# tachyon-beep/keisei

Measured on AMD Instinct MI355X. Metric: PPO samples/sec, se_resnet 40x256 on 50x9x9, higher is better.
Workload: dtype bf16; 1 GPU; se_resnet 40x256 KataGo-PPO minibatch step (gather+fwd+loss+bwd+clip+Adam), minibatch 4096/GPU from a 16384-sample device-resident epoch dataset, obs 50x9x9; per_gpu_batch=4096, global_batch=4096, parallelism=dp1

## Files before the change

### include/keisei_amd.h

```cpp
#ifndef KEISEI_AMD_H
#define KEISEI_AMD_H

#ifdef __cplusplus
extern "C" {
#endif

#define KA_OK 0
#define KA_ERR_ARG (-1)
#define KA_ERR_HIP (-2)
#define KA_ERR_UNSUPPORTED (-3)
#define KA_DTYPE_F32 0
#define KA_DTYPE_BF16 1

int ka_version(void);
const char* ka_target_arch(void);
const char* ka_last_error(void);
int ka_options_reload(void);

int ka_conv3x3_fwd(const void* in, const void* wpack, void* out, const float* in_scale, const float* in_shift,
                   const float* in_bias, int relu, float* bsum, float* sqpart, int B, int Cin, int Cout, int dtype,
                   void* stream);
int ka_conv3x3_fwd_keep_supported(int B, int Cin, int Cout, int dtype);
int ka_conv3x3_fwd_keep(const void* in, const void* wpack, void* out, const float* in_scale, const float* in_shift,
                        const float* in_bias, int relu, float* bsum, float* sqpart, void* x_out, int B, int Cin, int Cout, int dtype,
                        void* stream);
int ka_conv3x3_sqpart_rows(int B);
int ka_conv_route_counts(long long* out, int n);
int ka_conv3x3_dgrad_fused(const void* in, const void* in2, const float* k, void* dy_out, const void* wpack, void* out,
                           float* bsum, const void* ep_y, const float* ep_scale, const float* ep_shift,
                           const float* ep_mean, const float* ep_invstd, float* ep_s1, float* ep_s2, int B, int Cin,
                           int Cout, int dtype, void* stream);
int ka_conv3x3_dgrad_gated_supported(int B, int Cin, int Cout, int dtype, int masked);
int ka_conv3x3_dgrad_fused_gated(const void* du, const float* gate_add, const void* in2, const float* k,
                                 void* dy_out, const void* wpack, void* out, float* bsum, const void* ep_y,
                                 const float* ep_scale, const float* ep_shift, const float* ep_mean, const float* ep_invstd,
                                 float* ep_s1, float* ep_s2, int B, int Cin, int Cout, int dtype, void* stream);
int ka_pack_conv3x3(const float* w, void* dst, int Co, int Ci, int Nout, int Kin, int mode, int dtype, void* stream);
int ka_pack_conv3x3_multi(const long long* table, int n, long long max_pieces, int dtype, void* stream);
int ka_conv3x3_wgrad(const void* dy, const void* x, const float* in_scale, const float* in_shift, const float* in_bias,
                     int relu, float* slab, float* dw, int B, int Cin, int Cin_real, int Cout, int accumulate,
                     int target_wgs, int dtype, void* stream);
int ka_wgrad_splits(int B, int Cin, int Cout, int target_wgs);
int ka_debug_conv_stamps(unsigned long long* stamps);

int ka_obs_to_nhwc(const float* obs, const long long* idx, void* out, int B, int Cobs, int Cpad, int dtype, void* stream);
int ka_nhwc_to_nchw(const void* in, float* out, int B, int C, int dtype, void* stream);

int ka_reduce_workspace_doubles(int C);
int ka_bn_reduce(const float* bsum, int B, const float* sqpart, int R, int C, double* sums, double* part, void* stream);
int ka_bn_coeffs(const double* sums, double count, const double* count_dev, const float* gamma, const float* beta,
                 float* running_mean, float* running_var, long long* num_batches_tracked, float momentum, float eps,
                 float* scale, float* shift, float* mean, float* invstd, int C, void* stream);
int ka_bn_eval_coeffs(const float* gamma, const float* beta, const float* running_mean, const float* running_var,
                      float eps, float* scale, float* shift, int C, void* stream);
int ka_bn_eval_coeffs_multi(const long long* table, int n, int max_c, void* stream);
int ka_pair_reduce(const float* p1, const float* p2, int B, int C, double* sums, double* part, void* stream);
int ka_bn_bwd_coeffs(const double* sums_local, const double* sums_global, double count, const double* count_dev,
                     const float* gamma, const float* mean, const float* invstd, float* dgamma, float* dbeta, float* k,
                     int C, int train, void* stream);
int ka_sync_reduce(const float* p1, int rows1, const float* p2, int rows2, int C, double count, double* sums,
                   double* local_copy, double* part, void* stream);
int ka_bn_coeffs_parts(const double* part, double count, const float* gamma, const float* beta, float* running_mean,
                       float* running_var, long long* num_batches_tracked, float momentum, float eps, float* scale,
                       float* shift, float* mean, float* invstd, int C, void* stream);
int ka_bn_bwd_coeffs_parts(const double* part, double count, const float* gamma, const float* mean, const float* invstd,
                           float* dgamma, float* dbeta, float* k, int C, int train, void* stream);
int ka_bn_reduce_coeffs(const float* bsum, int B, const float* sqpart, int R, int C, double* part, int* counters, double count,
                        const float* gamma, const float* beta, float* running_mean, float* running_var,
                        long long* num_batches_tracked, float momentum, float eps, float* scale, float* shift, float* mean,
                        float* invstd, void* stream);
int ka_pair_reduce_bwd_coeffs(const float* p1, const float* p2, int rows, int C, double* part, int* counters, double count,
                              const float* gamma, const float* mean, const float* invstd, float* dgamma, float* dbeta, float* k,
                              int train, void* stream);
int ka_bn_bwd_apply(const void* dz, const void* y, const float* k, void* dy, int B, int C, int dtype, void* stream);
int ka_affine_rows(const float* in, const float* a, const float* s, float mul, float* out, int B, int C, void* stream);

int ka_block_tail_fwd(const void* y, const float* scale, const float* shift, const float* se, const void* res, void* out,
                      float* pool, int B, int C, int dtype, void* stream);
int ka_block_tail_fwd_se_supported(int C, int H, int dtype);
int ka_block_tail_fwd_se(const void* y, const float* scale, const float* shift, const float* bsum, const float* W1, const float* b1,
                         const float* W2, const float* b2, const void* res, void* out, float* pool, float* sqz_out, float* se1_out,
                         float* se_out, int B, int C, int H, int dtype, void* stream);
int ka_pool_fwd(const void* x, float* pool, int B, int C, int dtype, void* stream);
int ka_tail_bwd_reduce(const void* dout, const void* out, const void* y, const float* scale, const float* shift,
                       const float* se, float* dse, int B, int C, int dtype, void* stream);
int ka_tail_bwd_dz(const void* dout, const void* out, const void* y, const float* se, const float* dsq, const float* mean,
                   const float* invstd, void* dz, float* s1p, float* s2p, int B, int C, int dtype, void* stream);
int ka_tail_bwd_fused_supported(int C, int H, int dtype);
int ka_tail_bwd_fused(const void* dout, const void* out, const void* y, const float* scale, const float* shift,
                      const float* se, const float* se1, const float* W2, const float* W1, const float* mean,
                      const float* invstd, void* dz, float* dse, float* dh, float* s1p, float* s2p, int B, int C, int H,
                      int dtype, void* stream);
int ka_relu_bn_bwd_reduce(const void* dh, const void* y, const float* scale, const float* shift, const float* mean,
                          const float* invstd, void* da, float* s1p, float* s2p, int B, int C, int dtype, void* stream);
int ka_block_dx(const void* dxc, const void* dout, const void* out, const void* x, const float* xpool, const float* dpool,
                void* dx, int B, int C, int dtype, void* stream);
int ka_block_dx_tail_bwd_supported(int C, int H, int dtype);
int ka_block_dx_tail_bwd(const void* dxc, const void* dout_up, const void* out_up, const void* x, const float* xpool,
                         const float* dpool, void* dx, const void* y, const float* scale, const float* shift, const float* se,
                         const float* se1, const float* W2, const float* W1, const float* mean, const float* invstd, void* dz,
                         float* dse, float* dh, float* s1p, float* s2p, int B, int C, int H, int dtype, void* stream);
int ka_block_dx_tail_bwd_du(const void* dxc, const void* du_up, const void* x, const float* xpool, const float* dpool,
                            void* du_out, const void* y, const float* scale, const float* shift, const float* se,
                            const float* se1, const float* W2, const float* W1, const float* mean, const float* invstd, void* dz,
                            float* dse, float* dh, float* s1p, float* s2p, int B, int C, int H, int dtype, void* stream);
int ka_block_dx_tail_bwd_du_gate(const void* dxc, const void* du_up, const void* x, const float* xpool, const float* dpool,
                                 void* du_out, const void* y, const float* scale, const float* shift, const float* se,
                                 const float* se1, const float* W2, const float* W1, const float* mean, const float* invstd,
                                 float* gate_out, float* add_out, float* dse, float* dh, float* s1p, float* s2p, int B, int C,
                                 int H, int dtype, void* stream);

int ka_gemm(const void* A, const void* B, void* C, const float* bias, int M, int N, int K, int lda, int ldb, int ldc,
            int transA, int transB, int a_bf16, int b_bf16, int c_bf16, int relu, int accumulate, int nsplit, void* stream);
int ka_gemm_grouped_wgrad(const long long* table, int njobs, int total_wgs, void* stream);
int ka_fc_chain_supported(int K1, int ldx, int H, int N2);
int ka_fc_chain(const float* x, const float* in_scale, const float* in_shift, float in_alpha, const float* W1,
                const float* b1, const float* W2, const float* b2, float* x_out, float* hidden_out, float* y, int M, int K1,
                int ldx, int H, int N2, void* stream);
int ka_fc_chain_bwd(const float* dy, const float* hidden, const float* W2T, const float* W1T, float* dhidden_out, float* dx,
                    int M, int N2, int H, int K1, void* stream);
int ka_transpose_multi(const void* table, int n, int max_tiles, void* stream);
int ka_reduce_slabs(const float* slab, float* out, int nsplit, long long n, int accumulate, void* stream);
int ka_reduce_slabs2(const float* slab_a, float* out_a, long long na, const float* slab_b, float* out_b, long long nb, int nsplit,
                     void* stream);
int ka_colsum(const float* A, const float* Bm, float* part, float* part2, int M, int N, int nsplit, void* stream);
int ka_relu_mask(float* g, const float* h, long long n, void* stream);
int ka_rows_affine_relu(const float* in, const float* scale, const float* shift, float* out, long long M, int N, void* stream);
int ka_rows_sq_sums(const float* A, float* part, float* part2, int M, int N, int nsplit, void* stream);
int ka_rows_bn_sums(const float* da, const float* in, const float* mean, const float* invstd, float* part, float* part2,
                    int M, int N, int nsplit, void* stream);
int ka_rows_bn_bwd(float* dr, const float* in, const float* p0, const float* p1, long long M, int N, int mode, void* stream);

int ka_policy_loss(const float* logits, const void* legal, const long long* actions, const float* old_lp, const float* adv,
                   const long long* idx, float* dlogits, float* new_lp, float* rowloss, float* rowent, int* flags,
                   const float* gscale, float clip_eps, float w_policy, float w_entropy, int B, int A, int legal_words,
                   void* stream);
int ka_masked_softmax(const float* logits, const void* legal, float* probs, int* nlegal, int* flags, int B, int A,
                      int legal_words, void* stream);
int ka_policy_sample(const void* logits, int logits_bf16, const void* legal, int legal_words, long long seed,
                     const float* vlogits, const float* score, float alpha, long long* actions, float* logp, float* values,
                     int* nlegal, int* flags, int B, int A, void* stream);
int ka_policy_sample_play(const void* logits, int logits_bf16, const void* legal, int legal_words, const long long* seed_dev,
                          const int* model_of, int K, long long* actions, float* logp, int* nlegal, int* flags, int B, int A,
                          void* stream);
int ka_policy_ce(const float* logits, const long long* targets, const long long* idx, float* dlogits, float* rowloss,
                 int* flags, const float* gscale, float w_policy, int B, int A, void* stream);
int ka_value_loss(const float* vlogits, const float* score, const long long* cats, const float* targets,
                  const long long* idx, const float* rowloss, const float* rowent, float* dvlogits, float* dscore,
                  float* out, float* acc, const float* gscale, float lambda_policy, float lambda_value, float lambda_score,
                  float entropy_coeff, int combined_value_metric, int B, void* stream);
int ka_scalar_value(const float* vlogits, const float* score, float alpha, float* out, int B, void* stream);

int ka_adam_chunk(void);
int ka_clip_adam_step(const void* tab, const int* blk_tensor, const long long* blk_off, int nblocks, double* partial,
                      float* ctl, float* step_state, float* scaler, const int* guard_flags, float* acc_gnorm,
                      float max_norm, float lr, float beta1, float beta2, float eps, void* stream);

int ka_gae(const void* rewards, const void* values, const float* term, const void* next_value, const void* override_,
           const long long* lengths, void* adv, int T, int N, double gamma, double lam, int f64, void* stream);
int ka_normalize_advantages(const float* x, float* out, long long n, void* stream);

int ka_mask_words(int A);
int ka_rollout_append(const float* obs, const void* legal, const long long* actions, const float* log_probs,
                      const float* values, const float* rewards, const void* dones, const void* terminated,
                      const long long* cats, const float* score, const long long* env_ids, const float* override_,
                      float* d_obs, void* d_bits, long long* d_actions, float* d_log_probs, float* d_values, float* d_rewards,
                      void* d_dones, void* d_terminated, long long* d_cats, float* d_score, long long* d_env_ids,
                      float* d_override, int* flags, int n, int obs_elems, int A, void* stream);
int ka_rollout_append_packed(const float* obs, const void* legal_bits, const long long* actions, const float* log_probs,
                             const float* values, const float* rewards, const void* dones, const void* terminated,
                             const long long* cats, const float* score, const long long* env_ids, const float* override_,
                             float* d_obs, void* d_bits, long long* d_actions, float* d_log_probs, float* d_values, float* d_rewards,
                             void* d_dones, void* d_terminated, long long* d_cats, float* d_score, long long* d_env_ids,
                             float* d_override, int* flags, int n, int obs_elems, int A, void* stream);
int ka_unpack_mask_bits(const void* bits, const long long* idx, void* out, int rows, int A, void* stream);
int ka_pack_mask_bits(const void* legal, void* bits, int rows, int A, void* stream);

int ka_pending_open(float* obs, void* bits, long long* actions, float* log_probs, float* values, float* rewards, float* score,
                    void* valid, const void* env_mask, const float* s_obs, const void* s_legal, const void* s_bits,
                    const long long* s_actions, const float* s_log_probs, const float* s_values, const float* s_rewards,
                    const float* s_score, int* flags, int n, int obs_elems, int A, void* stream);
int ka_pending_accumulate(float* rewards, const void* valid, const float* add_rewards, int n, void* stream);
int ka_pending_settle(float* obs, void* bits, long long* actions, float* log_probs, float* values, float* rewards, float* score,
                      const void* valid, void* valid_out, const void* fin_mask, const void* dones, const void* terminated,
                      int flags_are_f32, const float* add_rewards, float* o_obs, void* o_bits, long long* o_actions,
                      float* o_log_probs, float* o_values, float* o_rewards, float* o_dones, float* o_terminated, float* o_score,
                      long long* o_env_ids, long long* o_cats, int* flags, int n, int obs_elems, int A, void* stream);

int ka_tower_eval_supported(int C, int G, int R, int dtype);
int ka_tower_eval(const void* x_in, const float* pool_in, void* x_out, float* pool_out, const void* blocks, int nblocks, int B,
                  int C, int G, int R, int dtype, void* stream);
int ka_tower_eval_grouped_supported(int C, int G, int R, int dtype);
int ka_stem_eval_grouped(const float* obs, const int* model_of, const void* stems, int K, void* x_out, float* pool_out, int B,
                         int cin, int C, int dtype, void* stream);
int ka_tower_eval_grouped(const void* x_in, const float* pool_in, void* x_out, float* pool_out, const int* model_of,
                          const void* tables, int K, int nblocks, int B, int C, int G, int R, int dtype, void* stream);
int ka_heads_eval_grouped(const void* x, const float* pool, const int* model_of, const void* heads, int K, float* logits,
                          float* value, float* score, int B, int C, int P, int V, int S, int dtype, void* stream);

int ka_shogi_env_state_bytes(void);
int ka_shogi_env_action_space(int action_mode);
int ka_shogi_env_reset(void* state, void* keys, void* checks, int n, int max_ply, int obs_mode, int action_mode, float* obs,
                       void* mask, void* mask_bits, void* current_players, int refresh, void* stream);
int ka_shogi_env_step(void* state, void* keys, void* checks, const long long* actions, int n, int max_ply, int obs_mode,
                      int action_mode, const void* prev_mask, const void* prev_mask_bits, int* err, float* obs, void* mask, void* mask_bits,
                      float* rewards, void* terminated, void* truncated, float* terminal_obs, void* current_players,
                      void* captured, void* term_reason, void* ply_count, int* material, void* stats, void* stream);

int ka_arena_state_words(int slots);
int ka_arena_referee(int* state, int slots, int envs_per_slot, const float* rewards, const void* terminated,
                     const void* truncated, const void* players, const int* nlegal, const long long* refusal, int* model_of,
                     void* pre_player, void* stream);
int ka_arena_assign(int* state, const int* jobs, int njobs, int envs_per_slot, const void* players, int* model_of,
                    void* pre_player, void* stream);
int ka_arena_cursor_words(int slots);
int ka_arena_record_pre(const int* state, const int* side_bits, int slots, int envs_per_slot, const float* obs,
                        const void* mask_bits, const long long* actions, const void* pre_player, const int* nlegal,
                        int* cursors, int* row_of, float* st_obs, void* st_mask_bits, long long* st_actions,
                        void* st_perspective, int cap, int obs_elems, int mask_words, void* stream);
int ka_arena_record_post(int* cursors, const int* row_of, int slots, int envs_per_slot, const float* rewards,
                         const void* terminated, const void* truncated, float* st_rewards, float* st_dones, int cap,
                         void* stream);
int ka_arena_feature_words(int which);
int ka_arena_features_step(const int* state, int slots, int envs_per_slot, const long long* actions, const void* pre_player,
                           const int* nlegal, const void* captured, const void* reason, const void* ply, const float* rewards,
                           const void* terminated, const void* truncated, int* acc, int* records, int* fcursors, int cap,
                           void* stream);
int ka_arena_features_seat(const int* jobs, int njobs, int slots, int envs_per_slot, int* acc, void* stream);
int ka_dynamic_targets(const float* rewards, const float* dones, long long* cats, float* adv, long long n, void* stream);

int ka_league_state_words(int opponents);
int ka_league_layout(int which);
int ka_league_step(int* state, int envs, int opponents, int flush, const float* obs, const void* mask_bits,
                   const long long* actions, const float* logp, const float* vlogits, const float* score_lead, float alpha,
                   const int* nlegal, const void* pre_player, const float* rewards, const void* terminated,
                   const void* truncated, const void* players, const int* material, float score_norm, const float* term_obs,
                   const long long* refusal, void* side, int* opp, int* games, const void* cum, int color_rand,
                   int* model_of, void* stall, float* values, float* p_obs, void* p_bits, int* p_scal, float* t_obs,
                   int* t_list, const long long* desc, int* plan, int obs_elems, int mask_words, void* stream);

int ka_tf_gemm_nt(const void* A, const void* B, void* C, const float* bias, const void* residual, int M, int N, int K,
                  int lda, int ldb, int ldc, int c_bf16, int relu, int nsplit, float drop_p, unsigned long long seed,
                  void* stream);
int ka_tf_gemm_nt_slabs(int K, int nsplit);
int ka_tf_gemm_nt_masked(const void* A, const void* B, void* C, const void* relu_act, int M, int N, int K, int lda, int ldb,
                         int ldc, float drop_p, unsigned long long seed, void* stream);
int ka_tf_gemm_tn(const void* A, const void* B, float* C, int M, int N, int K, int lda, int ldb, int ldc, int nsplit, void* stream);
int ka_tf_gemm_tn_bias(const void* A, const void* B, float* C, float* colsum, int M, int N, int K, int lda, int ldb, int ldc,
                       int nsplit, void* stream);
int ka_tf_gemm_tn_slabs(int M, int nsplit);
int ka_tf_transpose_pad(const void* in, void* out, int M, int N, int ldi, int ldo, int dtype, void* stream);
int ka_tf_cast_pad(const void* in, void* out, long long M, int N, int ldi, int ldo, int dtype, void* stream);
int ka_tf_weights16_multi(const void* table, int n, int total_tiles, void* stream);
int ka_tf_add_pos(void* x, const float* row_embed, const float* col_embed, int B, int d, int dtype, void* stream);
int ka_tf_pos_grad(const void* dx, float* scratch, float* drow, float* dcol, int B, int d, int dtype, void* stream);
int ka_tf_layernorm_fwd(const void* x, const float* gamma, const float* beta, void* y, float* mean, float* rstd, long long M,
                        int d, float eps, int dtype, void* stream);
int ka_tf_layernorm_parts(long long M);
int ka_tf_route_counts(long long* out, int n);
int ka_tf_layernorm_bwd(const void* dy, const void* x, const float* gamma, const float* mean, const float* rstd,
                        const void* dres, void* dx, float* part, float* dgamma, float* dbeta, long long M, int d, int dtype,
                        void* stream);
int ka_tf_layernorm_bwd_drop(const void* dy, const void* x, const float* gamma, const float* mean, const float* rstd,
                             const void* dres, void* dx, void* dx_drop, float drop_p, unsigned long long seed, float* part,
                             float* dgamma, float* dbeta, long long M, int d, int dtype, void* stream);
int ka_tf_drop_apply(const void* g_in, const void* act, const void* res, void* g_out, long long n, float drop_p,
                     unsigned long long seed, int dtype, void* stream);
int ka_tf_colsum(const void* a, float* part, float* out, long long M, int N, int nsplit, int dtype, void* stream);
int ka_tf_mean_pool(const void* x, float* pooled, int B, int d, int dtype, void* stream);
int ka_tf_head_grad(const float* dpooled, const void* dflat, void* dx, int B, int d, int dtype, void* stream);
int ka_tf_tanh(float* v, long long n, void* stream);
int ka_tf_tanh_bwd(const float* dy, const float* y, float* dx, long long n, void* stream);
int ka_tf_attention_fwd(const void* qkv, void* out, float* lse, int B, int H, int dh, float drop_p, unsigned long long seed,
                        int dtype, void* stream);
int ka_tf_attention_bwd(const void* qkv, const void* dout, const float* lse, void* dqkv, int B, int H, int dh, float drop_p,
                        unsigned long long seed, int dtype, void* stream);
int ka_tf_attention_bwd_o(const void* qkv, const void* out, const void* dout, const float* lse, void* dqkv, int B, int H, int dh,
                          float drop_p, unsigned long long seed, int dtype, void* stream);

#ifdef __cplusplus
}
#endif
#endif
```

### keisei_amd/_lib.py

```python
from __future__ import annotations

import ctypes
import os
from pathlib import Path
from typing import Optional

import torch

_LIB_PATH = Path(os.environ.get("KEISEI_AMD_LIB") or Path(__file__).resolve().parent / "libkeisei_amd.so")

_SIGS = {
    "ka_conv3x3_fwd": "pppppp i pp iii i p",
    "ka_conv3x3_fwd_keep_supported": "iiii",
    "ka_conv3x3_fwd_keep": "pppppp i pp p iii i p",
    "ka_conv3x3_dgrad_fused": "ppppp pp ppppp pp iii i p",
    "ka_conv3x3_dgrad_gated_supported": "iiiii",
    "ka_conv3x3_dgrad_fused_gated": "pppppp pp ppppp pp iii i p",
    "ka_conv3x3_sqpart_rows": "i",
    "ka_conv_route_counts": "p i",
    "ka_debug_conv_stamps": "p",
    "ka_pack_conv3x3": "pp iiii i i p",
    "ka_pack_conv3x3_multi": "p i q i p",
    "ka_wgrad_splits": "iiii",
    "ka_conv3x3_wgrad": "ppppp i pp iiii i i i p",
    "ka_obs_to_nhwc": "ppp iii i p",
    "ka_nhwc_to_nchw": "pp ii i p",
    "ka_bn_reduce": "p i p i i pp p",
    "ka_reduce_workspace_doubles": "i",
    "ka_pair_reduce": "pp ii pp p",
    "ka_sync_reduce": "p i p i i d ppp p",
    "ka_bn_coeffs": "p d p pppp p ff pppp i p",
    "ka_bn_coeffs_parts": "p d pppp p ff pppp i p",
    "ka_bn_bwd_coeffs_parts": "p d ppp ppp i i p",
    "ka_bn_reduce_coeffs": "p i p i i pp d pppp p ff pppp p",
    "ka_pair_reduce_bwd_coeffs": "pp i i pp d ppp ppp i p",
    "ka_bn_eval_coeffs": "pppp f pp i p",
    "ka_bn_bwd_coeffs": "pp d p ppp ppp i i p",
    "ka_affine_rows": "ppp f p ii p",
    "ka_bn_bwd_apply": "pppp ii i p",
    "ka_block_tail_fwd": "ppppp pp ii i p",
    "ka_block_tail_fwd_se_supported": "iii",
    "ka_block_tail_fwd_se": "pppppppp ppp ppp iii i p",
    "ka_pool_fwd": "pp ii i p",
    "ka_tail_bwd_reduce": "pppppp p ii i p",
    "ka_tail_bwd_dz": "ppppppp ppp ii i p",
    "ka_tail_bwd_fused_supported": "iii",
    "ka_tail_bwd_fused": "ppppp pppppp p pppp iii i p",
    "ka_relu_bn_bwd_reduce": "pppppp ppp ii i p",
    "ka_block_dx": "pppppp p ii i p",
    "ka_block_dx_tail_bwd_supported": "iii",
    "ka_block_dx_tail_bwd": "pppppp p ppppppppp p pppp iii i p",
    "ka_block_dx_tail_bwd_du": "ppppp p ppppppppp p pppp iii i p",
    "ka_block_dx_tail_bwd_du_gate": "ppppp p ppppppppp pp pppp iii i p",
    "ka_gemm": "pppp iii iii ii iii i i i p",
    "ka_reduce_slabs": "pp i q i p",
    "ka_reduce_slabs2": "pp q pp q i p",
    "ka_colsum": "pppp ii i p",
    "ka_relu_mask": "pp q p",
    "ka_rows_affine_relu": "pppp q i p",
    "ka_rows_bn_bwd": "pppp q i i p",
    "ka_rows_bn_sums": "pppp pp ii i p",
    "ka_rows_sq_sums": "ppp ii i p",
    "ka_policy_loss": "pppppp pppp pp fff iii p",
    "ka_masked_softmax": "ppppp iii p",
    "ka_policy_sample": "pi pi q pp f ppp pp ii p",
    "ka_policy_sample_play": "pi pi pp i pp pp ii p",
    "ka_policy_ce": "ppp ppp p f ii p",
    "ka_value_loss": "ppppp pp pp pp p ffff i i p",
    "ka_scalar_value": "pp f p i p",
    "ka_adam_chunk": "",
    "ka_clip_adam_step": "ppp i ppp ppp fffff p",
    "ka_gae": "ppppp pp ii dd i p",
    "ka_normalize_advantages": "pp q p",
    "ka_bn_eval_coeffs_multi": "p ii p",
    "ka_gemm_grouped_wgrad": "p ii p",
    "ka_fc_chain_supported": "iiii",
    "ka_fc_chain": "ppp f pppp ppp iiiii p",
    "ka_fc_chain_bwd": "pppppp iiii p",
    "ka_transpose_multi": "p ii p",
    "ka_mask_words": "i",
    "ka_rollout_append": "pppppppppppp pppppppppppp p iii p",
    "ka_rollout_append_packed": "pppppppppppp pppppppppppp p iii p",
    "ka_unpack_mask_bits": "ppp ii p",
    "ka_pack_mask_bits": "pp ii p",
    "ka_pending_open": "pppppppp ppppppppp p iii p",
    "ka_pending_accumulate": "ppp i p",
    "ka_pending_settle": "ppppppppp ppp i p ppppppppppp p iii p",
    "ka_tower_eval_supported": "iiii",
    "ka_tower_eval": "ppppp iiiii i p",
    "ka_tower_eval_grouped_supported": "iiii",
    "ka_stem_eval_grouped": "ppp i pp iiii p",
    "ka_tower_eval_grouped": "pppppp iiiiiii p",
    "ka_heads_eval_grouped": "pppp i ppp iiiii i p",
    "ka_shogi_env_state_bytes": "",
    "ka_shogi_env_action_space": "i",
    "ka_shogi_env_reset": "ppp ii ii pppp i p",
    "ka_shogi_env_step": "pppp ii ii ppp ppp ppp pp ppp pp p",
    "ka_arena_state_words": "i",
    "ka_arena_referee": "p ii ppppp p pp p",
    "ka_arena_assign": "pp ii ppp p",
    "ka_arena_cursor_words": "i",
    "ka_arena_record_pre": "pp ii ppppp pp pppp iii p",
    "ka_arena_record_post": "pp ii ppp pp i p",
    "ka_arena_feature_words": "i",
    "ka_arena_features_step": "p ii ppp ppp ppp ppp i p",
    "ka_arena_features_seat": "p iii p p",
    "ka_dynamic_targets": "pppp q p",
    "ka_league_state_words": "i",
    "ka_league_layout": "i",
    "ka_league_step": "p iii pppppp f ppppppp f pp pppp i ppp ppp pp pp ii p",
    "ka_tf_gemm_nt": "ppppp iii iii iii f q p",
    "ka_tf_gemm_nt_slabs": "ii",
    "ka_tf_gemm_nt_masked": "pppp iii iii f q p",
    "ka_tf_gemm_tn": "ppp iii iii i p",
    "ka_tf_gemm_tn_bias": "pppp iii iii i p",
    "ka_tf_gemm_tn_slabs": "ii",
    "ka_tf_transpose_pad": "pp iiii i p",
    "ka_tf_cast_pad": "pp q iii i p",
    "ka_tf_weights16_multi": "p ii p",
    "ka_tf_add_pos": "ppp ii i p",
    "ka_tf_pos_grad": "pppp ii i p",
    "ka_tf_layernorm_fwd": "pppppp q i f i p",
    "ka_tf_layernorm_parts": "q",
    "ka_tf_route_counts": "p i",
    "ka_tf_layernorm_bwd": "pppppp pppp q i i p",
    "ka_tf_layernorm_bwd_drop": "pppppp pp f q ppp q i i p",
    "ka_tf_drop_apply": "pppp q f q i p",
    "ka_tf_colsum": "ppp q ii i p",
    "ka_tf_mean_pool": "pp ii i p",
    "ka_tf_head_grad": "ppp ii i p",
    "ka_tf_tanh": "p q p",
    "ka_tf_tanh_bwd": "ppp q p",
    "ka_tf_attention_fwd": "ppp iii f q i p",
    "ka_tf_attention_bwd": "pppp iii f q i p",
    "ka_tf_attention_bwd_o": "ppppp iii f q i p",
    "ka_version": "",
    "ka_options_reload": "",
}
_CT = {"p": ctypes.c_void_p, "i": ctypes.c_int, "f": ctypes.c_float, "d": ctypes.c_double, "q": ctypes.c_longlong}

_lib: Optional[ctypes.CDLL] = None
_load_error: Optional[str] = None


class KeiseiHipError(RuntimeError):
    """Raised when a libkeisei_amd.so entry point reports failure (or the library is absent)."""


def _load() -> ctypes.CDLL:
    global _lib, _load_error
    if _lib is not None:
        return _lib
    if _load_error is not None:
        raise KeiseiHipError(_load_error)
    if not _LIB_PATH.exists():
        _load_error = (f"{_LIB_PATH} is missing: build it with `python -m keisei_amd.build` "
                       "(hipcc --offload-arch=gfx950). There is no fallback for GPU tensors.")
        raise KeiseiHipError(_load_error)
    try:
        lib = ctypes.CDLL(str(_LIB_PATH))
    except OSError as e:
        _load_error = f"cannot load {_LIB_PATH}: {e}"
        raise KeiseiHipError(_load_error) from e
    for name, sig in _SIGS.items():
        fn = getattr(lib, name)
        fn.argtypes = [_CT[c] for c in sig.replace(" ", "")]
        fn.restype = ctypes.c_int
    lib.ka_last_error.restype = ctypes.c_char_p
    lib.ka_last_error.argtypes = []
    lib.ka_target_arch.restype = ctypes.c_char_p
    lib.ka_target_arch.argtypes = []
    _lib = lib
    return lib


def reload_options() -> int:
    _QUERIES.clear()
    return int(_load().ka_options_reload())


def library_path() -> Path:
    return _LIB_PATH


def exported_symbols() -> list:
    return sorted(list(_SIGS) + ["ka_last_error", "ka_target_arch"])


def available() -> bool:
    try:
        _load()
        return True
    except KeiseiHipError:
        return False


_CHECK = os.environ.get("KA_CHECK_ARGS", "0") == "1"


def _check_tensors(name: str, args) -> None:
    dev = None
    for i, a in enumerate(args):
        if not isinstance(a, torch.Tensor):
            continue
        if not a.is_cuda:
            raise KeiseiHipError(f"{name}: argument {i} is a {a.device} tensor (the C ABI takes device pointers)")
        if not a.is_contiguous():
            raise KeiseiHipError(f"{name}: argument {i} is not contiguous (shape {tuple(a.shape)}, strides {a.stride()})")
        if dev is None:
            dev = a.device
        elif a.device != dev:
            raise KeiseiHipError(f"{name}: tensors on different devices ({dev} and {a.device})")
    if dev is not None and dev.index != torch.cuda.current_device():
        raise KeiseiHipError(f"{name}: tensors live on {dev} but the current device is cuda:{torch.cuda.current_device()} "
                             "(wrap the call in torch.cuda.device(tensor.device))")


def _ptr(x):
    if x is None:
        return None
    if isinstance(x, torch.Tensor):
        return x.data_ptr()
    return int(x)


def stream_ptr(device=None) -> int:
    return torch.cuda.current_stream(device).cuda_stream


_PLANS: dict = {}
_Tensor = torch.Tensor
_cur_dev = torch.cuda.current_device


def _plan(name: str):
    lib = _load()
    sig = _SIGS[name].replace(" ", "")
    ent = (getattr(lib, name), tuple(i for i, c in enumerate(sig) if c == "p"), len(sig))
    _PLANS[name] = ent
    return ent


def call(name: str, *args) -> None:
    ent = _PLANS.get(name)
    if ent is None:
        ent = _plan(name)
    fn, ptr_idx, n = ent
    if len(args) != n:
        raise TypeError(f"{name}: expected {n} arguments, got {len(args)}")
    conv = list(args)
    dev = None
    for i in ptr_idx:
        a = conv[i]
        if a is None:
            continue
        if type(a) is _Tensor or isinstance(a, _Tensor):
            if dev is None and a.is_cuda:
                dev = a.device.index
            conv[i] = a.data_ptr()
        else:
            conv[i] = int(a)
    if dev is not None and dev != _cur_dev():
        with torch.cuda.device(dev):
            if _CHECK:
                _check_tensors(name, args)
            rc = fn(*conv)
    else:
        if _CHECK:
            _check_tensors(name, args)
        rc = fn(*conv)
    if rc != 0:
        raise KeiseiHipError(f"{name} failed ({rc}): {_load().ka_last_error().decode()}")


_QUERIES: dict = {}


def query(name: str, *args) -> int:
    key = (name, args)
    v = _QUERIES.get(key)
    if v is None:
        v = _QUERIES[key] = int(getattr(_load(), name)(*args))
    return v


DTYPE_F32, DTYPE_BF16 = 0, 1


def dtype_code(dt: torch.dtype) -> int:
    if dt == torch.float32:
        return DTYPE_F32
    if dt == torch.bfloat16:
        return DTYPE_BF16
    raise KeiseiHipError(f"unsupported activation dtype {dt} (float32 or bfloat16)")
```

### keisei_amd/csrc/common.h

```cpp
#pragma once
#include <hip/hip_runtime.h>
#include <stdint.h>

#define KA_OK 0
#define KA_ERR_ARG (-1)
#define KA_ERR_HIP (-2)
#define KA_ERR_UNSUPPORTED (-3)

#define KA_DTYPE_F32 0
#define KA_DTYPE_BF16 1

#define KA_BOARD 81
#define KA_PADBOARD 121

typedef __attribute__((ext_vector_type(8))) __bf16 bf16x8;
typedef __attribute__((ext_vector_type(4))) __bf16 bf16x4;
typedef __attribute__((ext_vector_type(4))) float f32x4;
typedef __attribute__((ext_vector_type(2))) float f32x2;

struct bf16_t { uint16_t v; };

void ka_set_error(const char* fmt, ...);
int ka_check_launch(const char* what);
#define KA_REQUIRE(cond, ...) do { if (!(cond)) { ka_set_error(__VA_ARGS__); return KA_ERR_ARG; } } while (0)

#include <atomic>
inline int ka_big_lds_once(const void* func, std::atomic<unsigned long long>& done, const char* what) {
    int dev = 0;
    if (hipGetDevice(&dev) != hipSuccess) { ka_set_error("%s: hipGetDevice failed", what); return KA_ERR_HIP; }
    const unsigned long long bit = 1ull << (dev & 63);
    if (done.load(std::memory_order_acquire) & bit) return KA_OK;
    if (hipFuncSetAttribute(func, hipFuncAttributeMaxDynamicSharedMemorySize, 160 * 1024) != hipSuccess) {
        ka_set_error("%s: hipFuncSetAttribute failed on device %d", what, dev);
        return KA_ERR_HIP;
    }
    done.fetch_or(bit, std::memory_order_release);
    return KA_OK;
}

#include <stdlib.h>
inline const char* ka_diag_env(const char* name) {
#ifdef KA_DIAG
    return getenv(name);
#else
    (void)name;
    return nullptr;
#endif
}

#define KA_OPTIONS(X)                                                                                                      \
    X(CONV_P) X(CONV_MT) X(CONV_PC2) X(CONV_PC2_SKIP) X(CONV_PC2_STAG) X(CONV_CORNER_IN) X(CONV_P_STAG) X(CONV_P_PRIO) X(CONV_P_WGS) X(CONV_P_NPW) X(CONV_WM) X(CONV_KC)       \
    X(CONV_NTW) X(CONV_STAGGER) X(CONV_PRIO) X(WGRAD_TN) X(WGRAD_WGS) X(WGRAD_STAG) X(WGRAD_LEAN) X(BOARD_PAIRS) X(TF_LDS_EPI) X(TF_K256) X(TF_BIG)    \
    X(TF_MAP2D) X(TF_ATTN_LDS) X(TF_ATTN_ONE) X(TAIL_FWD_KB) X(TAIL_GATE_P4)
enum KaOpt {
#define KA_OPT_ENUM(n) KA_OPT_##n,
    KA_OPTIONS(KA_OPT_ENUM)
#undef KA_OPT_ENUM
    KA_OPT_COUNT
};
struct KaOptVal { int set, val; };
const KaOptVal* ka_opts();
inline bool ka_opt_set(KaOpt o) { return ka_opts()[o].set != 0; }
inline int ka_opt(KaOpt o, int dflt) { const KaOptVal v = ka_opts()[o]; return v.set ? v.val : dflt; }

std::atomic<unsigned long long*>& ka_debug_stamps();

enum KaConvRoute {
    KA_RT_CONV,
    KA_RT_PC,
    KA_RT_PC2,
    KA_RT_PC2_CORNER_IN,
    KA_RT_PC2_CORNER_OUT,
    KA_RT_CORNER,
    KA_RT_WGRAD_LEAN,
    KA_RT_WGRAD_TILED,
    KA_RT_COUNT
};
void ka_conv_route(int r);

__device__ __forceinline__ float bf2f(uint16_t h) { return __uint_as_float(((uint32_t)h) << 16); }
__device__ __forceinline__ uint16_t f2bf(float f) {
    __bf16 b = (__bf16)f;
    return __builtin_bit_cast(uint16_t, b);
}

template <typename T> struct Elem;
template <> struct Elem<float> {
    static constexpr int kSize = 4;
    static constexpr int kPer16 = 4;
    static constexpr int kDtype = KA_DTYPE_F32;
    typedef f32x4 vec16;
    static __device__ __forceinline__ float ld(const float* p) { return *p; }
    static __device__ __forceinline__ void st(float* p, float v) { *p = v; }
    static __device__ __forceinline__ void unpack(const vec16& v, float* f) {
        f[0] = v[0]; f[1] = v[1]; f[2] = v[2]; f[3] = v[3];
    }
    static __device__ __forceinline__ vec16 pack(const float* f) { vec16 v = {f[0], f[1], f[2], f[3]}; return v; }
};
template <> struct Elem<bf16_t> {
    static constexpr int kSize = 2;
    static constexpr int kPer16 = 8;
    static constexpr int kDtype = KA_DTYPE_BF16;
    typedef bf16x8 vec16;
    static __device__ __forceinline__ float ld(const bf16_t* p) { return bf2f(p->v); }
    static __device__ __forceinline__ void st(bf16_t* p, float v) { p->v = f2bf(v); }
    static __device__ __forceinline__ void unpack(const vec16& v, float* f) {
#pragma unroll
        for (int i = 0; i < 8; ++i) f[i] = (float)v[i];
    }
    static __device__ __forceinline__ vec16 pack(const float* f) {
        vec16 v;
#pragma unroll
        for (int i = 0; i < 8; ++i) v[i] = (__bf16)f[i];
        return v;
    }
};

template <typename T> __device__ __forceinline__ f32x2 ld2(const T* p);
template <> __device__ __forceinline__ f32x2 ld2<float>(const float* p) { return *reinterpret_cast<const f32x2*>(p); }
template <> __device__ __forceinline__ f32x2 ld2<bf16_t>(const bf16_t* p) {
    uint32_t u = *reinterpret_cast<const uint32_t*>(p);
    f32x2 r = {__uint_as_float(u << 16), __uint_as_float(u & 0xffff0000u)};
    return r;
}
template <typename T> __device__ __forceinline__ void st2(T* p, f32x2 v);
template <> __device__ __forceinline__ void st2<float>(float* p, f32x2 v) { *reinterpret_cast<f32x2*>(p) = v; }
template <> __device__ __forceinline__ void st2<bf16_t>(bf16_t* p, f32x2 v) {
    uint32_t u = (uint32_t)f2bf(v[0]) | ((uint32_t)f2bf(v[1]) << 16);
    *reinterpret_cast<uint32_t*>(p) = u;
}
template <typename T> __device__ __forceinline__ float rnd(float v);
template <> __device__ __forceinline__ float rnd<float>(float v) { return v; }
template <> __device__ __forceinline__ float rnd<bf16_t>(float v) { return bf2f(f2bf(v)); }

__device__ __forceinline__ int pad_index(int p) { return (p / 9 + 1) * 11 + (p % 9) + 1; }

__device__ __forceinline__ float wave_sum(float v) {
#pragma unroll
    for (int o = 32; o > 0; o >>= 1) v += __shfl_xor(v, o);
    return v;
}
__device__ __forceinline__ double wave_sum_d(double v) {
#pragma unroll
    for (int o = 32; o > 0; o >>= 1) v += __shfl_xor(v, o);
    return v;
}
#define KA_LDS_BARRIER() asm volatile("s_waitcnt lgkmcnt(0)\n\ts_barrier" ::: "memory")

__device__ __forceinline__ float sigmoidf_(float x) { return 1.0f / (1.0f + expf(-x)); }

__device__ __forceinline__ int ka_tile_rank(bool want, int running, int* wsum, int* rank) {
    const int lane = threadIdx.x & 63, wave = threadIdx.x >> 6;
    const unsigned long long b = __ballot(want);
    __syncthreads();
    if (lane == 0) wsum[wave] = __popcll(b);
    __syncthreads();
    int off = running, tot = 0;
    for (int w = 0; w < 4; ++w) {
        if (w < wave) off += wsum[w];
        tot += wsum[w];
    }
    *rank = want ? off + __popcll(b & ((1ull << lane) - 1ull)) : -1;
    return tot;
}
```

### keisei_amd/csrc/conv3x3.hip

```cpp
#include <stdlib.h>
#include <utility>
#include "common.h"

static std::atomic<long long> g_conv_routes[KA_RT_COUNT];
void ka_conv_route(int r) { g_conv_routes[r].fetch_add(1, std::memory_order_relaxed); }

namespace {

constexpr int kNB = 2;
constexpr int kPW = 17;
constexpr int kBoardStride = 193;
constexpr int kLdsSquares = kBoardStride + 11 * kPW;
constexpr int kImgSquares1 = 10 * kPW + 11;
constexpr int kZeroSquares = 2 * (kPW + 1) + 1;
__device__ __forceinline__ int lds_square(int b, int p) { return b * kBoardStride + (p / 9 + 1) * kPW + (p % 9) + 1; }
constexpr int kMTW = 6;

__host__ __device__ __forceinline__ int chan_of(int nt, int s, int NT) {
    return ((nt | 1) < NT) ? (nt >> 1) * 32 + (s >> 2) * 8 + (nt & 1) * 4 + (s & 3) : nt * 16 + s;
}

__device__ __forceinline__ float row_sum16(float v) {
    v += __int_as_float(__builtin_amdgcn_update_dpp(0, __float_as_int(v), 0xB1, 0xF, 0xF, true));
    v += __int_as_float(__builtin_amdgcn_update_dpp(0, __float_as_int(v), 0x4E, 0xF, 0xF, true));
// ... 748 lines not shown
#pragma unroll
                for (int e = 0; e < 4; ++e) {
                    esc[e] = a.ep_scale[cbl + 4 * j + e]; esh[e] = a.ep_shift[cbl + 4 * j + e];
                    emu[e] = a.ep_mean[cbl + 4 * j + e]; eis[e] = a.ep_invstd[cbl + 4 * j + e];
                    t1[e] = 0.f; t2[e] = 0.f;
                }
#pragma unroll
                for (int mt = 0; mt < MT; ++mt) {
                    const int p = mt * 16 + rl;
                    const bool in = p < KA_BOARD;
                    bf16x4 yv = bf16x4{};
                    if (in) yv = *reinterpret_cast<const bf16x4*>(smem + kPcLds + p * kPcYStride + (cb0 + 4 * j) * 2);
                    bf16x4 o;
#pragma unroll
                    for (int e = 0; e < 4; ++e) {
                        const float y = (float)yv[e];
                        const __bf16 db = (__bf16)acc[mt][j][e];
                        const float d = (in && y * esc[e] + esh[e] > 0.f) ? (float)db : 0.f;
                        t1[e] += d; t2[e] += d * ((y - emu[e]) * eis[e]);
                        o[e] = (__bf16)d;
                    }
                    if (j == 0) o0[mt] = o;
                    else if (in) {
                        bf16x8 o8;
#pragma unroll
                        for (int e = 0; e < 4; ++e) { o8[e] = o0[mt][e]; o8[4 + e] = o[e]; }
                        *reinterpret_cast<bf16x8*>(static_cast<char*>(a.out) + ((size_t)(bb * KA_BOARD + p) * a.Cout + cb0) * 2) = o8;
                    }
                }
#pragma unroll
                for (int e = 0; e < 4; ++e) { t1[e] = row_sum16(t1[e]); t2[e] = row_sum16(t2[e]); }
                if (rl == 0) {
                    *reinterpret_cast<f32x4*>(a.ep_s1 + (size_t)bb * a.Cout + cb0 + 4 * j) = f32x4{t1[0], t1[1], t1[2], t1[3]};
                    *reinterpret_cast<f32x4*>(a.ep_s2 + (size_t)bb * a.Cout + cb0 + 4 * j) = f32x4{t2[0], t2[1], t2[2], t2[3]};
                }
            }
            wfrag(0, 0, w0); wfrag(0, 1, w1); wfrag(0, 2, w2);
        }
    }
}

template <bool TWO, bool MASKED, int NPW, int MT, bool STAG = false>
static int launch_conv_pc_form(const ConvArgs& a, int grid, size_t lds, hipStream_t st, const char* what) {
    static std::atomic<unsigned long long> done{0};
    if (int rc = ka_big_lds_once(reinterpret_cast<const void*>(&conv3x3_pc_kernel<TWO, MASKED, NPW, MT, STAG>), done, what)) return rc;
    hipLaunchKernelGGL((conv3x3_pc_kernel<TWO, MASKED, NPW, MT, STAG>), dim3(grid), dim3(512 + 64 * NPW), lds, st, a);
    return ka_check_launch(what);
}
static int launch_conv_pc(ConvArgs a, hipStream_t st) {
    a.tune_stagger = 0; a.tune_prio = 0;
    if (const char* e = ka_diag_env("KA_CONV_P_ABL")) a.tune_stagger = atoi(e);
    a.tune_prio = ka_opt(KA_OPT_CONV_P_PRIO, 0);
    ka_conv_route(KA_RT_PC);
    int grid = 256;
    if (const int v = ka_opt(KA_OPT_CONV_P_WGS, 0); v > 0) grid = v;
    if (grid > a.B) grid = a.B;
    const int stag = ka_opt(KA_OPT_CONV_P_STAG, 0);
#define KA_PC_FORM(TWO_, MASKED_, NPW_, LDS_, WHAT_)                                                         \
    (a.mt5 ? ((stag && !MASKED_) ? launch_conv_pc_form<TWO_, false, NPW_, 5, true>(a, grid, LDS_, st, WHAT_ ", 5 row tiles, staggered") \
                                 : launch_conv_pc_form<TWO_, MASKED_, NPW_, 5>(a, grid, LDS_, st, WHAT_ ", 5 row tiles"))            \
           : launch_conv_pc_form<TWO_, MASKED_, NPW_, kMTW>(a, grid, LDS_, st, WHAT_))
    if (a.in2 && a.ep_y) return KA_PC_FORM(true, true, 4, kPcLdsMasked, "conv3x3 (pc, masked)");
    if (a.in2) return KA_PC_FORM(true, false, 4, kPcLds, "conv3x3 (pc, two-tensor)");
    if (ka_opt_set(KA_OPT_CONV_P_NPW) ? ka_opt(KA_OPT_CONV_P_NPW, 4) == 2 : (a.in_scale || a.relu || a.in_bias))
        return KA_PC_FORM(false, false, 2, kPcLds, "conv3x3 (pc, 2 staging waves)");
    return KA_PC_FORM(false, false, 4, kPcLds, "conv3x3 (pc)");
#undef KA_PC_FORM
}

typedef __attribute__((ext_vector_type(2))) unsigned u32x2;
template <int C, int MT>
__device__ __forceinline__ void conv_epilogue_masked_pair(const ConvArgs& a, f32x4 (&acc)[2 * MT][2], int b0, bool has_b1, int nt0, int r, int q) {
    constexpr int ROWB = C * 2, NT = C / 16;
    const int cb[2] = {chan_of(nt0, 4 * q, NT), chan_of(nt0 + 1, 4 * q, NT)};
    const char* yb = static_cast<const char*>(a.ep_y) + (size_t)b0 * (KA_BOARD * ROWB);
    char* ob = static_cast<char*>(a.out) + (size_t)b0 * (KA_BOARD * ROWB);
    const int lo[2] = {r * ROWB + cb[0] * 2, r * ROWB + cb[1] * 2};
    auto live = [&](int mt) { return MT == 5 || mt < 5 || r == 0; };
    u32x2 yA[MT], yB[MT];
    auto yload = [&](int b, int j, u32x2 (&y)[MT]) {
#pragma unroll
        for (int mt = 0; mt < MT; ++mt) y[mt] = live(mt) ? *reinterpret_cast<const u32x2*>(yb + b * (KA_BOARD * ROWB) + lo[j] + mt * 16 * ROWB) : u32x2{0u, 0u};
    };
    f32x4 cA[2], cB[2];
    yload(0, 0, yA);
    cA[0] = *reinterpret_cast<const f32x4*>(a.ep_scale + cb[0]); cA[1] = *reinterpret_cast<const f32x4*>(a.ep_shift + cb[0]);
    if (a.bsum) {
#pragma unroll
        for (int b = 0; b < 2; ++b)
#pragma unroll
            for (int j = 0; j < 2; ++j) {
                float s0[4] = {0.f, 0.f, 0.f, 0.f};
#pragma unroll
                for (int mt = 0; mt < MT; ++mt)
#pragma unroll
                    for (int i = 0; i < 4; ++i) s0[i] += live(mt) ? acc[MT * b + mt][j][i] : 0.f;
#pragma unroll
                for (int i = 0; i < 4; ++i) s0[i] = row_sum16(s0[i]);
                if (r == 0 && (b == 0 || has_b1)) *reinterpret_cast<f32x4*>(a.bsum + (b0 + b) * C + cb[j]) = f32x4{s0[0], s0[1], s0[2], s0[3]};
            }
    }
    yload(0, 1, yB);
    cB[0] = *reinterpret_cast<const f32x4*>(a.ep_scale + cb[1]); cB[1] = *reinterpret_cast<const f32x4*>(a.ep_shift + cb[1]);
    auto process = [&](int b, int j, const u32x2 (&y)[MT], const f32x4 (&c)[2]) {
        const f32x4 emu = *reinterpret_cast<const f32x4*>(a.ep_mean + cb[j]), eis = *reinterpret_cast<const f32x4*>(a.ep_invstd + cb[j]);
        float t1[4] = {0.f, 0.f, 0.f, 0.f}, t2[4] = {0.f, 0.f, 0.f, 0.f};
#pragma unroll
        for (int mt = 0; mt < MT; ++mt) {
            u32x2 o;
#pragma unroll
            for (int h = 0; h < 2; ++h) {
                const unsigned yw = y[mt][h];
                const float y0 = __uint_as_float(yw << 16), y1 = __uint_as_float(yw & 0xffff0000u);
                typedef __attribute__((ext_vector_type(2))) __bf16 bf16x2;
                const bf16x2 dbp = {(__bf16)acc[MT * b + mt][j][2 * h], (__bf16)acc[MT * b + mt][j][2 * h + 1]};
                const unsigned dw = __builtin_bit_cast(unsigned, dbp);
                const float d0 = (live(mt) && y0 * c[0][2 * h] + c[1][2 * h] > 0.f) ? __uint_as_float(dw << 16) : 0.f;
                const float d1 = (live(mt) && y1 * c[0][2 * h + 1] + c[1][2 * h + 1] > 0.f) ? __uint_as_float(dw & 0xffff0000u) : 0.f;
                t1[2 * h] += d0; t1[2 * h + 1] += d1;
                t2[2 * h] = fmaf(d0, y0, t2[2 * h]); t2[2 * h + 1] = fmaf(d1, y1, t2[2 * h + 1]);
                o[h] = (__float_as_uint(d0) >> 16) | __float_as_uint(d1);
            }
            if (live(mt)) *reinterpret_cast<u32x2*>(ob + b * (KA_BOARD * ROWB) + lo[j] + mt * 16 * ROWB) = o;
        }
#pragma unroll
        for (int e = 0; e < 4; ++e) {
            t1[e] = row_sum16(t1[e]);
            t2[e] = (row_sum16(t2[e]) - emu[e] * t1[e]) * eis[e];
        }
        if (r == 0) {
            *reinterpret_cast<f32x4*>(a.ep_s1 + (b0 + b) * C + cb[j]) = f32x4{t1[0], t1[1], t1[2], t1[3]};
            *reinterpret_cast<f32x4*>(a.ep_s2 + (b0 + b) * C + cb[j]) = f32x4{t2[0], t2[1], t2[2], t2[3]};
        }
    };
    process(0, 0, yA, cA);
    if (has_b1) yload(1, 0, yA);
    process(0, 1, yB, cB);
    if (has_b1) {
        yload(1, 1, yB);
        process(1, 0, yA, cA);
        process(1, 1, yB, cB);
    }
}

__device__ __forceinline__ void ld4x8_l2(const float* const (&p)[8], f32x4 (&v)[8]) {
    asm volatile("global_load_dwordx4 %0, %8, off sc1\n\t"
                 "global_load_dwordx4 %1, %9, off sc1\n\t"
                 "global_load_dwordx4 %2, %10, off sc1\n\t"
                 "global_load_dwordx4 %3, %11, off sc1\n\t"
                 "global_load_dwordx4 %4, %12, off sc1\n\t"
                 "global_load_dwordx4 %5, %13, off sc1\n\t"
                 "global_load_dwordx4 %6, %14, off sc1\n\t"
                 "global_load_dwordx4 %7, %15, off sc1\n\t"
                 "s_waitcnt vmcnt(0)"
                 : "=&v"(v[0]), "=&v"(v[1]), "=&v"(v[2]), "=&v"(v[3]), "=&v"(v[4]), "=&v"(v[5]), "=&v"(v[6]), "=&v"(v[7])
                 : "v"(p[0]), "v"(p[1]), "v"(p[2]), "v"(p[3]), "v"(p[4]), "v"(p[5]), "v"(p[6]), "v"(p[7])
                 : "memory");
}
__device__ __forceinline__ void corner_tile_epilogue(const ConvArgs& a, const f32x4 (&acc)[2], int bb, bool live, int nt0, int q) {
    if (!live) return;
    int cb[2];
    f32x4 pbs[2], psq[2], ps1[2], ps2[2];
    {
        const float* any = a.bsum ? a.bsum : reinterpret_cast<const float*>(a.wpack);
        const float* src[8];
#pragma unroll
        for (int j = 0; j < 2; ++j) {
            cb[j] = chan_of(nt0 + j, 4 * q, 16);
            const size_t srow = (size_t)bb * 256 + cb[j];
            src[j] = a.bsum ? a.bsum + srow : any;
            src[2 + j] = a.sqpart ? a.sqpart + srow : any;
            src[4 + j] = a.ep_y ? a.ep_s1 + srow : any;
            src[6 + j] = a.ep_y ? a.ep_s2 + srow : any;
        }
        f32x4 got[8];
        ld4x8_l2(src, got);
#pragma unroll
        for (int j = 0; j < 2; ++j) { pbs[j] = got[j]; psq[j] = got[2 + j]; ps1[j] = got[4 + j]; ps2[j] = got[6 + j]; }
    }
#pragma unroll
    for (int j = 0; j < 2; ++j) {
        const f32x4 v = acc[j];
        const size_t orow = ((size_t)bb * KA_BOARD + 80) * 256 + cb[j], srow = (size_t)bb * 256 + cb[j];
        if (a.bsum) *reinterpret_cast<f32x4*>(a.bsum + srow) = pbs[j] + v;
        if (a.sqpart) *reinterpret_cast<f32x4*>(a.sqpart + srow) = psq[j] + f32x4{v[0] * v[0], v[1] * v[1], v[2] * v[2], v[3] * v[3]};
        bf16x4 o;
        if (!a.ep_y) {
#pragma unroll
            for (int e = 0; e < 4; ++e) o[e] = (__bf16)v[e];
        } else {
            const f32x4 esc = *reinterpret_cast<const f32x4*>(a.ep_scale + cb[j]), esh = *reinterpret_cast<const f32x4*>(a.ep_shift + cb[j]);
            const f32x4 emu = *reinterpret_cast<const f32x4*>(a.ep_mean + cb[j]), eis = *reinterpret_cast<const f32x4*>(a.ep_invstd + cb[j]);
            const bf16x4 yv = *reinterpret_cast<const bf16x4*>(static_cast<const char*>(a.ep_y) + orow * 2);
            f32x4 t1, t2;
#pragma unroll
            for (int e = 0; e < 4; ++e) {
                const float y = (float)yv[e];
                const __bf16 db = (__bf16)v[e];
                const float d = (y * esc[e] + esh[e] > 0.f) ? (float)db : 0.f;
                t1[e] = d; t2[e] = d * ((y - emu[e]) * eis[e]);
                o[e] = (__bf16)d;
            }
            *reinterpret_cast<f32x4*>(a.ep_s1 + srow) = ps1[j] + t1;
            *reinterpret_cast<f32x4*>(a.ep_s2 + srow) = ps2[j] + t2;
        }
        *reinterpret_cast<bf16x4*>(static_cast<char*>(a.out) + orow * 2) = o;
    }
}

constexpr int kP2Stride = 64 * 2 + 32;
constexpr int kP2Img = kImgSquares1 * kP2Stride;
constexpr int kP2Lds = 4 * kP2Img;
constexpr int kP2SideRow = 4 * 512 + 16;
constexpr int kP2SideSlots = 9;
constexpr int kP2Side = kP2Lds, kP2Dump = kP2Side + 2 * kP2SideSlots * kP2SideRow, kP2LdsCorner = kP2Dump + 16;
constexpr int kP2Base = (kPW + 1) * kP2Stride;

struct P2Perm { unsigned char sq[10][16]; };
constexpr P2Perm make_p2perm() {
    P2Perm P{};
    const int E[8] = {0, 1, 2, 3, 12, 13, 14, 15}, O[8] = {4, 5, 6, 7, 8, 9, 10, 11};
    for (int k = 0; k < 8; ++k) {
        const int edge[4] = {k, 9 * k + 8, 9 * (k + 1), k < 7 ? 72 + (k + 1) : 40};
        for (int t = 0; t < 4; ++t) { P.sq[t][E[k]] = (unsigned char)edge[t]; P.sq[t][O[k]] = (unsigned char)edge[t]; }
    }
    int byres[8][6] = {}, cnt[8] = {};
    for (int y = 1; y <= 7; ++y)
        for (int x = 1; x <= 7; ++x) {
            if (y == 4 && x == 4) continue;
            const int rho = (x + y) & 7;
            byres[rho][cnt[rho]++] = 9 * y + x;
        }
    for (int b = 0; b < 2; ++b)
        for (int tt = 0; tt < 3; ++tt)
            for (int k = 0; k < 8; ++k) {
                P.sq[4 + 3 * b + tt][E[k]] = (unsigned char)byres[k][2 * tt];
                P.sq[4 + 3 * b + tt][O[k]] = (unsigned char)byres[k][2 * tt + 1];
            }
    return P;
}
__device__ const P2Perm kP2Perm = make_p2perm();
__host__ __device__ constexpr bool p2_skip(int t, int tap) {
    return (t == 0 && tap / 3 == 0) || (t == 1 && tap % 3 == 2) || (t == 2 && tap % 3 == 0);
}

template <typename F, int... I>
__device__ __forceinline__ void static_for_impl(F&& f, std::integer_sequence<int, I...>) { (f(std::integral_constant<int, I>{}), ...); }
template <int N, typename F>
__device__ __forceinline__ void static_for(F&& f) { static_for_impl(f, std::make_integer_sequence<int, N>{}); }

struct P2Seq { unsigned char s[216], t[216]; int n; };
constexpr P2Seq make_p2seq(bool skip, int ntiles) {
    P2Seq Q{};
    Q.n = 0;
    for (int s = 0; s < 18; ++s)
        for (int t = 0; t < ntiles; ++t)
            if (!(skip && p2_skip(t, s >> 1))) { Q.s[Q.n] = (unsigned char)s; Q.t[Q.n] = (unsigned char)t; ++Q.n; }
    return Q;
}

__device__ __forceinline__ void conv_epilogue_pair(const ConvArgs& a, f32x4 (&acc)[10][2], const unsigned (&sqp)[3], int b0, bool has_b1,
                                                   int nt0, int r, int q) {
    const int cb[2] = {chan_of(nt0, 4 * q, 16), chan_of(nt0 + 1, 4 * q, 16)};
    const bool isO = r >= 4 && r < 12;
    if (a.bsum || a.sqpart) {
#pragma unroll
        for (int j = 0; j < 2; ++j) {
#pragma unroll
            for (int b = 0; b < 2; ++b) {
                float s[4] = {0.f, 0.f, 0.f, 0.f}, ss[4] = {0.f, 0.f, 0.f, 0.f};
#pragma unroll
                for (int t = 0; t < 10; ++t) {
                    if (t >= 4 && (t >= 7) != (b == 1)) continue;
#pragma unroll
                    for (int i = 0; i < 4; ++i) {
                        float v = acc[t][j][i];
                        if (t < 4) v = (isO == (b == 1)) ? v : 0.f;
                        s[i] += v; ss[i] += v * v;
                    }
                }
#pragma unroll
                for (int i = 0; i < 4; ++i) { s[i] = row_sum16(s[i]); ss[i] = row_sum16(ss[i]); }
                if (r == 0 && (b == 0 || has_b1)) {
                    if (a.bsum) *reinterpret_cast<f32x4*>(a.bsum + (size_t)(b0 + b) * 256 + cb[j]) = f32x4{s[0], s[1], s[2], s[3]};
                    if (a.sqpart) *reinterpret_cast<f32x4*>(a.sqpart + (size_t)(b0 + b) * 256 + cb[j]) = f32x4{ss[0], ss[1], ss[2], ss[3]};
                }
                __builtin_amdgcn_sched_barrier(0);
            }
        }
    }
#pragma unroll
    for (int t = 0; t < 10; ++t) {
        const int bd = t < 4 ? (isO ? 1 : 0) : (t < 7 ? 0 : 1);
        if (bd && !has_b1) continue;
        bf16x8 o;
#pragma unroll
        for (int i = 0; i < 4; ++i) { o[i] = (__bf16)acc[t][0][i]; o[4 + i] = (__bf16)acc[t][1][i]; }
        const int sq = (int)((sqp[t >> 2] >> (8 * (t & 3))) & 0xffu);
        *reinterpret_cast<bf16x8*>(static_cast<char*>(a.out) + (size_t)b0 * (KA_BOARD * 512) + ((bd * KA_BOARD + sq) * 256 + cb[0]) * 2) = o;
        __builtin_amdgcn_sched_barrier(0);
    }
}

template <int C, int MT, bool TWO, bool MASKED, int NPW, bool SKIP = false, bool STAG = false, bool GATED = false>
__global__ __launch_bounds__((C / 32 + NPW) * 64) void conv3x3_pc2_kernel(ConvArgs a) {
    static_assert(!GATED || (TWO && MASKED && !SKIP && !STAG), "the gated input is conv2's data gradient: two-tensor, masked");
    static_assert(!(SKIP && MASKED), "the border-tile layout is built for the register-only epilogue");
    static_assert((C == 256 && MT == 5) || (C == 128 && MT == 6 && !SKIP), "shapes this kernel is built for");
    constexpr int NMW = C / 32, NCH = C / 64, NTILE = C / 16, KSG = C / 32, ROWB = C * 2, NTL = 2 * MT;
    constexpr int NT_ = (NMW + NPW) * 64, NP = 64 * NPW;
    constexpr int kHalf = KA_BOARD * 8, kPieces = 2 * kHalf;
    constexpr int KP = (kPieces + NP - 1) / NP;
    extern __shared__ __attribute__((aligned(16))) char smem[];
    const int tid = threadIdx.x, lane = tid & 63, wave = tid >> 6, r = lane & 15, q = lane >> 4;
    const int nwg = gridDim.x, npairs_all = (a.B + 1) >> 1;
    if ((int)blockIdx.x >= npairs_all) return;
    for (int i = tid; i < kP2Lds / 16; i += NT_) reinterpret_cast<uint4*>(smem)[i] = uint4{0, 0, 0, 0};
    const int npairs = (npairs_all - (int)blockIdx.x + nwg - 1) / nwg, nunits = NCH * npairs;
    if (!MASKED) a.ep_y = nullptr;
    __syncthreads();

    if (wave >= NMW) {
        const int pt = tid - NMW * 64, pc = pt & 7, swave = __builtin_amdgcn_readfirstlane(wave) - NMW;
        const bool has_aff = GATED || a.in_scale != nullptr;
        auto pair_rsrc = [&](const void* p, int b0, bool sized) {
            const unsigned nb = sized ? (unsigned)min(2, a.B - b0) * (KA_BOARD * ROWB) : 0u;
            return __builtin_amdgcn_make_buffer_rsrc(const_cast<char*>(static_cast<const char*>(p)) + (size_t)b0 * (KA_BOARD * ROWB), 0, nb,
                                                     0x00020000);
        };
        const int voff0 = (pt >> 3) * ROWB + pc * 16;
        int ldso[KP];
#pragma unroll
        for (int k = 0; k < KP; ++k) {
            const int row = min((pt + NP * k) >> 3, 2 * KA_BOARD - 1), j = row >= KA_BOARD ? 1 : 0;
            ldso[k] = j * kP2Img + lds_square(0, row - j * KA_BOARD) * kP2Stride + pc * 16;
        }
        auto live = [&](int k) { return (swave * 64 + NP * k) < kPieces; };
        const bool corner_in = C == 256 && MT == 5 && !MASKED && a.mt5 == 2;
        int cso[KP];
#pragma unroll
        for (int k = 0; k < KP; ++k) {
            const int row = min((pt + NP * k) >> 3, 2 * KA_BOARD - 1), j = row >= KA_BOARD ? 1 : 0, sq = row - j * KA_BOARD;
            const int ps = sq == 70 ? 0 : sq == 71 ? 1 : sq == 79 ? 2 : sq == 80 ? 3 : -1;
            cso[k] = (corner_in && ps >= 0 && pt + NP * k < kPieces) ? j * kP2SideRow + ps * 512 + pc * 16 : -1;
        }
        int chas = 0;
#pragma unroll
        for (int k = 0; k < KP; ++k) chas |= (__builtin_amdgcn_readfirstlane((int)(__ballot(cso[k] >= 0) != 0ull)) & 1) << k;
        bf16x8 pv[KP], pw[TWO ? KP : 1];
        auto stage_load = [&](int u) {
            const int b0 = __builtin_amdgcn_readfirstlane(2 * ((int)blockIdx.x + (u / NCH) * nwg)), c4 = u % NCH;
            const int soff = __builtin_amdgcn_readfirstlane(c4 * 128);
            const __amdgpu_buffer_rsrc_t r_in = pair_rsrc(a.in, b0, true), r_in2 = pair_rsrc(TWO ? a.in2 : a.in, b0, true);
#pragma unroll
            for (int k = 0; k < KP; ++k) {
                if (!live(k)) continue;
                const int vo = pt + NP * k < kPieces ? voff0 + k * (NP / 8) * ROWB : (int)0x7fffffff;
                pv[k] = __builtin_bit_cast(bf16x8, __builtin_amdgcn_raw_buffer_load_b128(r_in, vo, soff, 2));
                if (TWO) pw[TWO ? k : 0] = __builtin_bit_cast(bf16x8, __builtin_amdgcn_raw_buffer_load_b128(r_in2, vo, soff, 2));
            }
        };
        auto stage_write = [&](int u) __attribute__((always_inline)) {
            const int b0 = __builtin_amdgcn_readfirstlane(2 * ((int)blockIdx.x + (u / NCH) * nwg)), c4 = u % NCH, ch0 = c4 * 64 + pc * 8;
            const int soff = __builtin_amdgcn_readfirstlane(c4 * 128);
            const __amdgpu_buffer_rsrc_t r_out = pair_rsrc(a.in_out ? a.in_out : a.in, b0, a.in_out != nullptr);
            char* img = smem + (u & 1) * (2 * kP2Img);
            float sc[8], sh[8], k3[8], pb[2][8];
            {
                const f32x4 z = {0.f, 0.f, 0.f, 0.f}, o = {1.f, 1.f, 1.f, 1.f};
                const float* shp = GATED ? a.in_scale + C : a.in_shift;
                const float* k3p = GATED ? a.in_scale + 2 * C : a.in_k3;
                const f32x4 s0 = has_aff ? *reinterpret_cast<const f32x4*>(a.in_scale + ch0) : o, s1 = has_aff ? *reinterpret_cast<const f32x4*>(a.in_scale + ch0 + 4) : o;
                const f32x4 t0 = has_aff ? *reinterpret_cast<const f32x4*>(shp + ch0) : z, t1 = has_aff ? *reinterpret_cast<const f32x4*>(shp + ch0 + 4) : z;
                const f32x4 u0 = TWO ? *reinterpret_cast<const f32x4*>(k3p + ch0) : z, u1 = TWO ? *reinterpret_cast<const f32x4*>(k3p + ch0 + 4) : z;
                const bool bias = !TWO && a.in_bias;
                const f32x4 p00 = bias ? *reinterpret_cast<const f32x4*>(a.in_bias + (size_t)b0 * C + ch0) : z;
                const f32x4 p01 = bias ? *reinterpret_cast<const f32x4*>(a.in_bias + (size_t)b0 * C + ch0 + 4) : z;
                const bool b1 = bias && b0 + 1 < a.B;
                const f32x4 p10 = b1 ? *reinterpret_cast<const f32x4*>(a.in_bias + (size_t)(b0 + 1) * C + ch0) : z;
                const f32x4 p11 = b1 ? *reinterpret_cast<const f32x4*>(a.in_bias + (size_t)(b0 + 1) * C + ch0 + 4) : z;
#pragma unroll
                for (int e = 0; e < 4; ++e) {
                    sc[e] = s0[e]; sc[4 + e] = s1[e]; sh[e] = t0[e]; sh[4 + e] = t1[e]; k3[e] = u0[e]; k3[4 + e] = u1[e];
                    pb[0][e] = p00[e]; pb[0][4 + e] = p01[e]; pb[1][e] = p10[e]; pb[1][4 + e] = p11[e];
                }
            }
            float gsc0[8], gsh0[8], gsc1[8], gsh1[8];
            if constexpr (GATED) {
                const f32x4 z = {0.f, 0.f, 0.f, 0.f};
                const float* gp = a.in_bias + (size_t)b0 * C + ch0;
                const float* ap = gp + (size_t)a.B * C;
                const bool b1 = b0 + 1 < a.B;
                const f32x4 g00 = *reinterpret_cast<const f32x4*>(gp), g01 = *reinterpret_cast<const f32x4*>(gp + 4);
                const f32x4 a00 = *reinterpret_cast<const f32x4*>(ap), a01 = *reinterpret_cast<const f32x4*>(ap + 4);
                const f32x4 g10 = b1 ? *reinterpret_cast<const f32x4*>(gp + C) : z, g11 = b1 ? *reinterpret_cast<const f32x4*>(gp + C + 4) : z;
                const f32x4 a10 = b1 ? *reinterpret_cast<const f32x4*>(ap + C) : z, a11 = b1 ? *reinterpret_cast<const f32x4*>(ap + C + 4) : z;
#pragma unroll
                for (int e = 0; e < 4; ++e) {
                    gsc0[e] = g00[e] * sc[e]; gsc0[4 + e] = g01[e] * sc[4 + e];
                    gsh0[e] = fmaf(a00[e], sc[e], sh[e]); gsh0[4 + e] = fmaf(a01[e], sc[4 + e], sh[4 + e]);
                    gsc1[e] = g10[e] * sc[e]; gsc1[4 + e] = g11[e] * sc[4 + e];
                    gsh1[e] = fmaf(a10[e], sc[e], sh[e]); gsh1[4 + e] = fmaf(a11[e], sc[4 + e], sh[4 + e]);
                }
            }
#pragma unroll
            for (int k = 0; k < KP; ++k) {
                if (!live(k)) continue;
                const int i = pt + NP * k;
                if (i >= kPieces) continue;
                const int j = i >= kHalf ? 1 : 0;
                bf16x8 v = pv[k];
                if (TWO) {
                    const bool jlo = NP * (k + 1) <= kHalf, jhi = NP * k >= kHalf;
#pragma unroll
                    for (int e = 0; e < 8; ++e) {
                        float se_ = sc[e], he_ = sh[e];
                        if constexpr (GATED) {
                            const float c0 = gsc0[e], c1 = gsc1[e], h0 = gsh0[e], h1 = gsh1[e];
                            se_ = jlo ? c0 : jhi ? c1 : (j ? c1 : c0);
                            he_ = jlo ? h0 : jhi ? h1 : (j ? h1 : h0);
                        }
                        v[e] = (__bf16)fmaf((float)pw[TWO ? k : 0][e], k3[e], fmaf((float)v[e], se_, he_));
                    }
                    if (b0 + j >= a.B) v = bf16x8{};
                    __builtin_amdgcn_raw_buffer_store_b128(__builtin_bit_cast(__attribute__((ext_vector_type(4))) unsigned, v), r_out,
                                                           voff0 + k * (NP / 8) * ROWB, soff, 0);
                } else if (has_aff || a.relu || a.in_bias) {
#pragma unroll
                    for (int e = 0; e < 8; e += 2) {
                        f32x2 f = {(float)v[e], (float)v[e + 1]};
                        if (has_aff) f = __builtin_elementwise_fma(f, f32x2{sc[e], sc[e + 1]}, f32x2{sh[e], sh[e + 1]});
                        if (a.relu) f = __builtin_elementwise_max(f, f32x2{0.f, 0.f});
                        if (a.in_bias) f += j ? f32x2{pb[1][e], pb[1][e + 1]} : f32x2{pb[0][e], pb[0][e + 1]};
                        v[e] = (__bf16)f[0]; v[e + 1] = (__bf16)f[1];
                    }
                    if (b0 + j >= a.B) v = bf16x8{};
                    if constexpr (C == 256) __builtin_amdgcn_raw_buffer_store_b128(__builtin_bit_cast(__attribute__((ext_vector_type(4))) unsigned, v), r_out,
                                                           voff0 + k * (NP / 8) * ROWB, soff, 0);
                }
                *reinterpret_cast<bf16x8*>(img + ldso[k]) = v;
            }
        };
        auto side_write = [&](int u) {
            if constexpr (C == 256 && MT == 5) {
                if (!corner_in) return;
                const char* img = smem + (u & 1) * (2 * kP2Img);
                const int side0 = kP2Side + 2 * ((u / NCH) % kP2SideSlots) * kP2SideRow + (u % NCH) * 128;
#pragma unroll
                for (int k = 0; k < KP; ++k) {
                    if (!live(k) || !((chas >> k) & 1)) continue;
                    const bf16x8 t = *reinterpret_cast<const bf16x8*>(img + ldso[k]);
                    *reinterpret_cast<bf16x8*>(smem + (cso[k] >= 0 ? side0 + cso[k] : kP2Dump)) = t;
                }
            }
        };
        auto stage = [&](int u) __attribute__((always_inline)) { stage_load(u); stage_write(u); side_write(u); };
        stage(0);
        KA_LDS_BARRIER();
        if constexpr (STAG) {
            for (int v = 1; v < nunits; ++v) {
                stage_load(v);
                KA_LDS_BARRIER();
                stage_write(v);
                side_write(v);
                KA_LDS_BARRIER();
            }
            KA_LDS_BARRIER();
            KA_LDS_BARRIER();
            return;
        }
        for (int u = 0; u < nunits; ++u) {
            if (u + 1 < nunits) stage(u + 1);
            KA_LDS_BARRIER();
        }
        return;
    }

    const __amdgpu_buffer_rsrc_t wrsrc = __builtin_amdgcn_make_buffer_rsrc(const_cast<void*>(a.wpack), 0, 9 * KSG * NTILE * 1024, 0x00020000);
    const int wlane = __builtin_amdgcn_readfirstlane(wave) * 2048 + lane * 16;
    auto wfrag = [&](int c4, int s, bf16x8 (&f)[2]) {
        if (s >= 18) { s -= 18; c4 = (c4 + 1) % NCH; }
        const int tap = s >> 1, ks = c4 * 2 + (s & 1);
        const int so = __builtin_amdgcn_readfirstlane(((tap * KSG + ks) * NTILE) * 1024);
        f[0] = __builtin_bit_cast(bf16x8, __builtin_amdgcn_raw_buffer_load_b128(wrsrc, wlane, so, 0));
        f[1] = __builtin_bit_cast(bf16x8, __builtin_amdgcn_raw_buffer_load_b128(wrsrc, wlane + 1024, so, 0));
    };
    constexpr int NRB = SKIP ? 10 : MT;
    int rowbase[NRB];
    unsigned sqp[3] = {0u, 0u, 0u};
#pragma unroll
    for (int t = 0; t < NRB; ++t) {
        if (SKIP) {
            const int sq = kP2Perm.sq[t][r];
            sqp[t >> 2] |= (unsigned)sq << (8 * (t & 3));
            const int bd = t < 4 ? ((r >= 4 && r < 12) ? 1 : 0) : (t < 7 ? 0 : 1);
            rowbase[t] = bd * kP2Img + lds_square(0, sq) * kP2Stride + q * 16 - kP2Base;
        } else {
            const int p = t * 16 + r;
            rowbase[t] = (p < KA_BOARD ? lds_square(0, p) : kPW + 13) * kP2Stride + q * 16 - kP2Base;
        }
    }
    auto frag_off = [&](int t) { return SKIP ? rowbase[SKIP ? t : 0] : rowbase[t % MT] + (t / MT) * kP2Img; };
    bf16x8 wr[3][2];
    wfrag(0, 0, wr[0]); wfrag(0, 1, wr[1]);
    f32x4 acc[NTL][2];
    KA_LDS_BARRIER();
    if (a.stamps && tid == 0) {
        a.stamps[blockIdx.x * 8 + 0] = __builtin_amdgcn_s_memtime();
        a.stamps[blockIdx.x * 8 + 3] = __builtin_amdgcn_s_memrealtime();
    }
    const bool late = STAG && __builtin_amdgcn_readfirstlane(wave) >= NMW / 2;
    if (late) KA_LDS_BARRIER();
    for (int u = 0; u < nunits; ++u) {
        const int c4 = u % NCH;
        if (!c4) {
#pragma unroll
            for (int t = 0; t < NTL; ++t) { acc[t][0] = f32x4{0.f, 0.f, 0.f, 0.f}; acc[t][1] = f32x4{0.f, 0.f, 0.f, 0.f}; }
        }
        const char* img = smem;
        constexpr P2Seq Q = make_p2seq(SKIP, NTL);
        constexpr int R = MASKED ? 5 : 8;
        bf16x8 fa[R];
        auto frag_at = [&](auto n_) {
            constexpr int n = decltype(n_)::value, s = Q.s[n], t = Q.t[n], tap = s >> 1;
            constexpr int toff = kP2Base + ((tap / 3 - 1) * kPW + (tap % 3 - 1)) * kP2Stride + (s & 1) * 64;
            fa[n % R] = *reinterpret_cast<const bf16x8*>(img + frag_off(t) + toff);
        };
        static_for<R>(frag_at);
        static_for<Q.n>([&](auto n_) {
            constexpr int n = decltype(n_)::value, s = Q.s[n], t = Q.t[n];
            if constexpr (n == 0 || Q.s[n > 0 ? n - 1 : 0] != s) {
                __builtin_amdgcn_sched_barrier(0);
                if constexpr (STAG && s == 9) KA_LDS_BARRIER();
                if (!(MASKED && c4 == NCH - 1 && s >= 16)) wfrag(c4, s + 2, wr[(s + 2) % 3]);
                __builtin_amdgcn_sched_barrier(0);
            }
            acc[t][0] = __builtin_amdgcn_mfma_f32_16x16x32_bf16(wr[s % 3][0], fa[n % R], acc[t][0], 0, 0, 0);
            acc[t][1] = __builtin_amdgcn_mfma_f32_16x16x32_bf16(wr[s % 3][1], fa[n % R], acc[t][1], 0, 0, 0);
            __builtin_amdgcn_sched_group_barrier(0x008, 2, 0);
            if constexpr (n + R < Q.n) {
                frag_at(std::integral_constant<int, n + R>{});
                __builtin_amdgcn_sched_group_barrier(0x100, 1, 0);
            }
        });
        __builtin_amdgcn_sched_barrier(0);
        if (c4 == NCH - 1) {
            const int b0 = 2 * ((int)blockIdx.x + (u / NCH) * nwg);
            if constexpr (MASKED) {
                int rl = r, ql = q;
                asm volatile("" : "+v"(rl), "+v"(ql));
                conv_epilogue_masked_pair<C, MT>(a, acc, b0, b0 + 1 < a.B, wave * 2, rl, ql);
                wfrag(0, 0, wr[0]); wfrag(0, 1, wr[1]);
            } else if constexpr (SKIP) {
                if constexpr (SKIP) conv_epilogue_pair(a, acc, sqp, b0, b0 + 1 < a.B, wave * 2, r, q);
            } else {
                conv_epilogue<bf16_t, 2, MT>(a, reinterpret_cast<f32x4 (&)[MT][2]>(acc[0]), b0, wave * 2, NTILE, r, q);
                if (b0 + 1 < a.B) conv_epilogue<bf16_t, 2, MT>(a, reinterpret_cast<f32x4 (&)[MT][2]>(acc[MT]), b0 + 1, wave * 2, NTILE, r, q);
            }
            if constexpr (C == 256 && MT == 5 && !SKIP && !STAG && !MASKED) {
                const int pidx = u / NCH;
                if (a.mt5 == 2 && ((pidx & 7) == 7 || pidx == npairs - 1)) {
                    const int g0 = pidx & ~7;
                    const int pr = g0 + (r >> 1), prc = min(pr, pidx);
                    const char* arow = smem + kP2Side + (2 * (prc % kP2SideSlots) + (r & 1)) * kP2SideRow + q * 16;
                    auto cw = [&](int step, bf16x8 (&f)[2]) {
                        const int ps = (step >> 2) & 3, tap = ps < 2 ? ps : ps + 1, ks = (step >> 4) * 4 + (step & 3);
                        const int so = __builtin_amdgcn_readfirstlane(((tap * KSG + ks) * NTILE) * 1024);
                        f[0] = __builtin_bit_cast(bf16x8, __builtin_amdgcn_raw_buffer_load_b128(wrsrc, wlane, so, 0));
                        f[1] = __builtin_bit_cast(bf16x8, __builtin_amdgcn_raw_buffer_load_b128(wrsrc, wlane + 1024, so, 0));
                    };
                    constexpr int kAh = 8;
                    bf16x8 wq[kAh][2];
#pragma unroll
                    for (int s2 = 0; s2 < kAh; ++s2) cw(s2, wq[s2]);
                    f32x4 cacc[2] = {f32x4{0.f, 0.f, 0.f, 0.f}, f32x4{0.f, 0.f, 0.f, 0.f}};
#pragma unroll
                    for (int step = 0; step < 32; ++step) {
                        const bf16x8 w0 = wq[step % kAh][0], w1 = wq[step % kAh][1];
                        if (step + kAh < 32) cw(step + kAh, wq[step % kAh]);
                        const int ps = (step >> 2) & 3, ks = (step >> 4) * 4 + (step & 3);
                        const bf16x8 af = *reinterpret_cast<const bf16x8*>(arow + ps * 512 + ks * 64);
                        cacc[0] = __builtin_amdgcn_mfma_f32_16x16x32_bf16(w0, af, cacc[0], 0, 0, 0);
                        cacc[1] = __builtin_amdgcn_mfma_f32_16x16x32_bf16(w1, af, cacc[1], 0, 0, 0);
                    }
                    const int bb = 2 * ((int)blockIdx.x + pr * nwg) + (r & 1);
                    asm volatile("s_waitcnt vmcnt(0)" ::: "memory");
                    corner_tile_epilogue(a, cacc, bb, pr <= pidx && bb < a.B, wave * 2, q);
                }
            }
        }
#pragma unroll
        for (int t = 0; t < NRB; ++t) rowbase[t] += (u & 1) ? -2 * kP2Img : 2 * kP2Img;
        if (!(late && u == nunits - 1)) KA_LDS_BARRIER();
    }
    if (a.stamps && tid == 0) {
        a.stamps[blockIdx.x * 8 + 7] = __builtin_amdgcn_s_memtime();
        a.stamps[blockIdx.x * 8 + 4] = __builtin_amdgcn_s_memrealtime();
    }
}

template <int C, int MT, bool TWO, bool MASKED, int NPW, bool SKIP = false, bool STAG = false, bool GATED = false>
static int launch_conv_pc2_form(const ConvArgs& a, hipStream_t st, const char* what) {
    static std::atomic<unsigned long long> done{0};
    if (int rc = ka_big_lds_once(reinterpret_cast<const void*>(&conv3x3_pc2_kernel<C, MT, TWO, MASKED, NPW, SKIP, STAG, GATED>), done, what)) return rc;
    const int pairs = (a.B + 1) / 2, grid = pairs < 256 ? pairs : 256;
    hipLaunchKernelGGL((conv3x3_pc2_kernel<C, MT, TWO, MASKED, NPW, SKIP, STAG, GATED>), dim3(grid), dim3((C / 32 + NPW) * 64),
                       C == 256 ? kP2LdsCorner : kP2Lds, st, a);
    return ka_check_launch(what);
}
static int launch_conv_pc2(const ConvArgs& a, hipStream_t st) {
    ka_conv_route(a.Cin == 128 ? KA_RT_PC2 : (a.mt5 == 2 ? KA_RT_PC2_CORNER_IN : KA_RT_PC2_CORNER_OUT));
    if (a.in2 && a.in_bias) {
        KA_REQUIRE(a.in2 && a.ep_y, "conv3x3: the gated input comes with the two-tensor transform and the masked epilogue");
        if (a.Cin == 128) return launch_conv_pc2_form<128, 6, true, true, 4, false, false, true>(a, st, "conv3x3 (two boards per unit, 128 channels, gated two-tensor, masked)");
        return launch_conv_pc2_form<256, 5, true, true, 4, false, false, true>(a, st, "conv3x3 (two boards per unit, gated two-tensor, masked)");
    }
    if (a.Cin == 128) {
        if (a.in2 && a.ep_y) return launch_conv_pc2_form<128, 6, true, true, 4>(a, st, "conv3x3 (two boards per unit, 128 channels, two-tensor, masked)");
        if (a.in2) return launch_conv_pc2_form<128, 6, true, false, 4>(a, st, "conv3x3 (two boards per unit, 128 channels, two-tensor)");
        return launch_conv_pc2_form<128, 6, false, false, 4>(a, st, "conv3x3 (two boards per unit, 128 channels)");
    }
    const bool skip = ka_opt(KA_OPT_CONV_PC2_SKIP, 0) != 0;
    const bool stag = ka_opt(KA_OPT_CONV_PC2_STAG, 0) != 0;
    if (stag && !skip) {
        if (a.in2 && a.ep_y) return launch_conv_pc2_form<256, 5, true, true, 4, false, true>(a, st, "conv3x3 (two boards per unit, two-tensor, masked, staggered)");
        if (a.in2) return launch_conv_pc2_form<256, 5, true, false, 4, false, true>(a, st, "conv3x3 (two boards per unit, two-tensor, staggered)");
        return launch_conv_pc2_form<256, 5, false, false, 4, false, true>(a, st, "conv3x3 (two boards per unit, staggered)");
    }
    if (a.in2 && a.ep_y) return launch_conv_pc2_form<256, 5, true, true, 4>(a, st, "conv3x3 (two boards per unit, two-tensor, masked)");
    if (a.in2) return skip ? launch_conv_pc2_form<256, 5, true, false, 4, true>(a, st, "conv3x3 (two boards per unit, two-tensor, border tiles)")
                           : launch_conv_pc2_form<256, 5, true, false, 4>(a, st, "conv3x3 (two boards per unit, two-tensor)");
    return skip ? launch_conv_pc2_form<256, 5, false, false, 4, true>(a, st, "conv3x3 (two boards per unit, border tiles)")
                : launch_conv_pc2_form<256, 5, false, false, 4>(a, st, "conv3x3 (two boards per unit)");
}

constexpr int kCornerBoards = 32, kCornerStride = 4 * 512 + 16;
constexpr int kCornerLds = kCornerBoards * kCornerStride;

__global__ __launch_bounds__(512) void conv3x3_corner_kernel(ConvArgs a) {
    extern __shared__ __attribute__((aligned(16))) char cs[];
    const int tid = threadIdx.x, lane = tid & 63, wave = tid >> 6, r = lane & 15, q = lane >> 4;
    const int b0 = blockIdx.x * kCornerBoards;
    const int rt = wave & 1, nt0 = blockIdx.y * 8 + (wave >> 1) * 2;
    const char* wl = static_cast<const char*>(a.wpack) + (size_t)nt0 * 1024 + lane * 16;
    auto wfrag = [&](int step, int j) {
        const int kc = step >> 4, ps = (step >> 2) & 3, ks = kc * 4 + (step & 3), tap = ps < 2 ? ps : ps + 1;
        return *reinterpret_cast<const bf16x8*>(wl + (size_t)((tap * 8 + ks) * 16 + j) * 1024);
    };
    constexpr int kAhead = 12;
    bf16x8 wq[kAhead][2];
#pragma unroll
    for (int s2 = 0; s2 < kAhead; ++s2) { wq[s2][0] = wfrag(s2, 0); wq[s2][1] = wfrag(s2, 1); }
    const bool has_aff = a.in_scale != nullptr;
    const int pc = tid & 31, ch0 = pc * 8;
    {
        bf16x8 pv[8], pw[8];
#pragma unroll
        for (int k = 0; k < 8; ++k) {
            const int i = tid + 512 * k, bl = i >> 7, ps = (i >> 5) & 3, bb = min(b0 + bl, a.B - 1);
            const int p = ps == 0 ? 70 : ps == 1 ? 71 : ps == 2 ? 79 : 80;
            const size_t off = (((size_t)bb * KA_BOARD + p) * 256 + ch0) * 2;
            pv[k] = *reinterpret_cast<const bf16x8*>(static_cast<const char*>(a.in) + off);
            pw[k] = a.in2 ? *reinterpret_cast<const bf16x8*>(static_cast<const char*>(a.in2) + off) : bf16x8{};
        }
        float sc[8], sh[8], k3[8];
#pragma unroll
        for (int e = 0; e < 8; ++e) { sc[e] = 1.f; sh[e] = 0.f; k3[e] = 0.f; }
        if (has_aff) {
            const f32x4 s0 = *reinterpret_cast<const f32x4*>(a.in_scale + ch0), s1 = *reinterpret_cast<const f32x4*>(a.in_scale + ch0 + 4);
            const f32x4 t0 = *reinterpret_cast<const f32x4*>(a.in_shift + ch0), t1 = *reinterpret_cast<const f32x4*>(a.in_shift + ch0 + 4);
#pragma unroll
            for (int e = 0; e < 4; ++e) { sc[e] = s0[e]; sc[4 + e] = s1[e]; sh[e] = t0[e]; sh[4 + e] = t1[e]; }
        }
        if (a.in2) {
            const f32x4 u0 = *reinterpret_cast<const f32x4*>(a.in_k3 + ch0), u1 = *reinterpret_cast<const f32x4*>(a.in_k3 + ch0 + 4);
#pragma unroll
            for (int e = 0; e < 4; ++e) { k3[e] = u0[e]; k3[4 + e] = u1[e]; }
        }
#pragma unroll
        for (int k = 0; k < 8; ++k) {
            const int i = tid + 512 * k, bl = i >> 7, ps = (i >> 5) & 3;
            bf16x8 v = pv[k];
            if (a.in2 && a.in_bias) {
                const size_t go = (size_t)min(b0 + bl, a.B - 1) * 256 + ch0;
                const float* addp = a.in_bias + (size_t)a.B * 256;
                const f32x4 g0 = *reinterpret_cast<const f32x4*>(a.in_bias + go), g1 = *reinterpret_cast<const f32x4*>(a.in_bias + go + 4);
                const f32x4 a0 = *reinterpret_cast<const f32x4*>(addp + go), a1 = *reinterpret_cast<const f32x4*>(addp + go + 4);
#pragma unroll
                for (int e = 0; e < 8; ++e) {
                    const float ge = e < 4 ? g0[e & 3] : g1[e & 3], ae = e < 4 ? a0[e & 3] : a1[e & 3];
                    v[e] = (__bf16)fmaf((float)pw[k][e], k3[e], fmaf((float)v[e], ge * sc[e], fmaf(ae, sc[e], sh[e])));
                }
            } else if (a.in2) {
#pragma unroll
                for (int e = 0; e < 8; ++e) v[e] = (__bf16)fmaf((float)pw[k][e], k3[e], fmaf((float)v[e], sc[e], sh[e]));
            } else if (has_aff || a.relu || a.in_bias) {
                f32x4 pb0 = {0.f, 0.f, 0.f, 0.f}, pb1 = pb0;
                if (a.in_bias) {
                    const size_t bo = (size_t)min(b0 + bl, a.B - 1) * 256 + ch0;
                    pb0 = *reinterpret_cast<const f32x4*>(a.in_bias + bo); pb1 = *reinterpret_cast<const f32x4*>(a.in_bias + bo + 4);
                }
#pragma unroll
                for (int e = 0; e < 8; ++e) {
                    float f = (float)v[e];
                    if (has_aff) f = fmaf(f, sc[e], sh[e]);
                    if (a.relu) f = fmaxf(f, 0.f);
                    if (a.in_bias) f += e < 4 ? pb0[e & 3] : pb1[e & 3];
                    v[e] = (__bf16)f;
                }
            }
            if (b0 + bl >= a.B) v = bf16x8{};
            *reinterpret_cast<bf16x8*>(cs + bl * kCornerStride + ps * 512 + pc * 16) = v;
        }
    }
    __syncthreads();
    const int bb = b0 + 16 * rt + r;
    const bool live = bb < a.B;
    const int bbc = min(bb, a.B - 1);
    int cb[2];
    f32x4 pbs[2], psq[2], ps1[2], ps2[2], esc[2], esh[2], emu[2], eis[2];
    bf16x4 yv[2];
#pragma unroll
    for (int j = 0; j < 2; ++j) {
        cb[j] = chan_of(nt0 + j, 4 * q, 16);
        const size_t srow = (size_t)bbc * 256 + cb[j];
        pbs[j] = psq[j] = ps1[j] = ps2[j] = esc[j] = esh[j] = emu[j] = eis[j] = f32x4{0.f, 0.f, 0.f, 0.f};
        yv[j] = bf16x4{};
        if (a.bsum) pbs[j] = *reinterpret_cast<const f32x4*>(a.bsum + srow);
        if (a.sqpart) psq[j] = *reinterpret_cast<const f32x4*>(a.sqpart + srow);
        if (a.ep_y) {
            ps1[j] = *reinterpret_cast<const f32x4*>(a.ep_s1 + srow); ps2[j] = *reinterpret_cast<const f32x4*>(a.ep_s2 + srow);
            esc[j] = *reinterpret_cast<const f32x4*>(a.ep_scale + cb[j]); esh[j] = *reinterpret_cast<const f32x4*>(a.ep_shift + cb[j]);
            emu[j] = *reinterpret_cast<const f32x4*>(a.ep_mean + cb[j]); eis[j] = *reinterpret_cast<const f32x4*>(a.ep_invstd + cb[j]);
            yv[j] = *reinterpret_cast<const bf16x4*>(static_cast<const char*>(a.ep_y) + (((size_t)bbc * KA_BOARD + 80) * 256 + cb[j]) * 2);
        }
    }
    f32x4 acc[2] = {f32x4{0.f, 0.f, 0.f, 0.f}, f32x4{0.f, 0.f, 0.f, 0.f}};
    const char* arow = cs + (16 * rt + r) * kCornerStride + q * 16;
#pragma unroll
    for (int step = 0; step < 32; ++step) {
        const bf16x8 w0 = wq[step % kAhead][0], w1 = wq[step % kAhead][1];
        if (step + kAhead < 32) { wq[step % kAhead][0] = wfrag(step + kAhead, 0); wq[step % kAhead][1] = wfrag(step + kAhead, 1); }
        const int ps = (step >> 2) & 3, ks = (step >> 4) * 4 + (step & 3);
        const bf16x8 af = *reinterpret_cast<const bf16x8*>(arow + ps * 512 + ks * 64);
        acc[0] = __builtin_amdgcn_mfma_f32_16x16x32_bf16(w0, af, acc[0], 0, 0, 0);
        acc[1] = __builtin_amdgcn_mfma_f32_16x16x32_bf16(w1, af, acc[1], 0, 0, 0);
    }
    if (!live) return;
#pragma unroll
    for (int j = 0; j < 2; ++j) {
        const f32x4 v = acc[j];
        const size_t orow = ((size_t)bb * KA_BOARD + 80) * 256 + cb[j], srow = (size_t)bb * 256 + cb[j];
        if (a.bsum) *reinterpret_cast<f32x4*>(a.bsum + srow) = pbs[j] + v;
        if (a.sqpart) *reinterpret_cast<f32x4*>(a.sqpart + srow) = psq[j] + f32x4{v[0] * v[0], v[1] * v[1], v[2] * v[2], v[3] * v[3]};
        bf16x4 o;
        if (!a.ep_y) {
#pragma unroll
            for (int e = 0; e < 4; ++e) o[e] = (__bf16)v[e];
        } else {
            f32x4 t1, t2;
#pragma unroll
            for (int e = 0; e < 4; ++e) {
                const float y = (float)yv[j][e];
                const __bf16 db = (__bf16)v[e];
                const float d = (y * esc[j][e] + esh[j][e] > 0.f) ? (float)db : 0.f;
                t1[e] = d; t2[e] = d * ((y - emu[j][e]) * eis[j][e]);
                o[e] = (__bf16)d;
            }
            *reinterpret_cast<f32x4*>(a.ep_s1 + srow) = ps1[j] + t1;
            *reinterpret_cast<f32x4*>(a.ep_s2 + srow) = ps2[j] + t2;
        }
        *reinterpret_cast<bf16x4*>(static_cast<char*>(a.out) + orow * 2) = o;
    }
}
static int launch_conv_corner(const ConvArgs& a, hipStream_t st) {
    static std::atomic<unsigned long long> done{0};
    ka_conv_route(KA_RT_CORNER);
    if (int rc = ka_big_lds_once(reinterpret_cast<const void*>(&conv3x3_corner_kernel), done, "conv3x3 (corner)")) return rc;
    hipLaunchKernelGGL(conv3x3_corner_kernel, dim3((a.B + kCornerBoards - 1) / kCornerBoards, 2), dim3(512), kCornerLds, st, a);
    return ka_check_launch("conv3x3 (corner)");
}

template <typename T>
int conv_dispatch(ConvArgs a, hipStream_t st) {
    typedef Elem<T> E;
    constexpr int CPK = 4 * E::kPer16;
    KA_REQUIRE(a.B > 0 && a.Cin % CPK == 0 && a.Cout % 16 == 0,
               "conv3x3: need Cin %% %d == 0 and Cout %% 16 == 0 (got Cin=%d Cout=%d)", CPK, a.Cin, a.Cout);
    bool want5 = false;
    if constexpr (sizeof(T) == 2) {
        const int pv = ka_opt(KA_OPT_CONV_P, 1);
        want5 = a.Cin == 256 && a.Cout == 256 && a.B >= 512 && ka_opt(KA_OPT_CONV_MT, 5) != 6;
        const int p2 = ka_opt(KA_OPT_CONV_PC2, 3);
        if (p2 != 0 && want5 && pv != 0 && (!a.in2 || (p2 >= 2 && !a.ep_y) || p2 >= 3)) {
            const bool corner_in = ka_opt(KA_OPT_CONV_CORNER_IN, 1) != 0 && !a.ep_y && ka_opt(KA_OPT_CONV_PC2_SKIP, 0) == 0 &&
                                   ka_opt(KA_OPT_CONV_PC2_STAG, 0) == 0;
            a.mt5 = corner_in ? 2 : 1;
            if (int rc = launch_conv_pc2(a, st)) return rc;
            return corner_in ? KA_OK : launch_conv_corner(a, st);
        }
        if (p2 != 0 && pv != 0 && a.Cin == 128 && a.Cout == 128 && a.B >= 512 && (!a.in2 || (p2 >= 2 && !a.ep_y) || p2 >= 3))
            return launch_conv_pc2(a, st);
        KA_REQUIRE(!(a.in2 && a.in_bias), "conv3x3: the gated two-tensor input exists in the two-board kernel only (ka_conv3x3_dgrad_gated_supported)");
        if (pv != 0 && a.Cin == 256 && a.Cout == 256 && a.B >= 512 &&
            (!a.in2 || (pv >= 2 && !a.ep_y) || pv >= 3)) {
            a.mt5 = want5;
            if (int rc = launch_conv_pc(a, st)) return rc;
            return want5 ? launch_conv_corner(a, st) : KA_OK;
        }
    }
    int wm = 1;
    if (const int v = ka_opt(KA_OPT_CONV_WM, 0); v == 1 || v == 2) wm = v;
    const int img_squares = wm == 2 ? kLdsSquares : kImgSquares1;
    int kc = 0;
    for (int steps = a.Cin / CPK; steps >= 1; --steps) {
        const int cand = steps * CPK;
        if (a.Cin % cand != 0 || 256 % (cand * E::kSize / 16) != 0) continue;
        if ((size_t)(img_squares + kZeroSquares) * (cand * E::kSize + 32) > 150 * 1024) continue;
        kc = cand;
        break;
    }
    KA_REQUIRE(kc > 0, "conv3x3: cannot chunk Cin=%d", a.Cin);
    if (E::kSize == 2 && kc > 128 && a.Cin % 128 == 0) kc = 128;
    int ntw = a.Cout > 128 ? 4 : (a.Cout > 64 ? 2 : 1);
    while (ntw > 1 && (long long)((a.B + wm - 1) / wm) * ((a.Cout + 64 * ntw - 1) / (64 * ntw)) < 256) ntw >>= 1;
    a.tune_prio = 1;
    if (const int v = ka_opt(KA_OPT_CONV_KC, 0); v > 0 && a.Cin % v == 0 && v % CPK == 0 && v <= kc) kc = v;
    if (const int v = ka_opt(KA_OPT_CONV_NTW, 0); v == 1 || v == 2 || v == 4) ntw = v;
    a.tune_stagger = ka_opt(KA_OPT_CONV_STAGGER, a.tune_stagger);
    a.tune_prio = ka_opt(KA_OPT_CONV_PRIO, a.tune_prio);
    KA_REQUIRE(256 % (kc * E::kSize / 16) == 0, "conv3x3: chunk of %d channels does not tile the workgroup", kc);
    a.KC = kc;
    if (wm == 1) {
        if (ntw == 4) {
            if constexpr (sizeof(T) == 2) {
                if (want5) {
                    a.mt5 = 1;
                    if (int rc = launch_conv<T, 4, 1>(a, st)) return rc;
                    return launch_conv_corner(a, st);
                }
            }
            return launch_conv<T, 4, 1>(a, st);
        }
        if (ntw == 2) return launch_conv<T, 2, 1>(a, st);
        return launch_conv<T, 1, 1>(a, st);
    }
    if (ntw == 4) return launch_conv<T, 4, 2>(a, st);
    if (ntw == 2) return launch_conv<T, 2, 2>(a, st);
    return launch_conv<T, 1, 2>(a, st);
}

}

extern "C" int ka_conv3x3_fwd(const void* in, const void* wpack, void* out, const float* in_scale,
                              const float* in_shift, const float* in_bias, int relu, float* bsum, float* sqpart,
                              int B, int Cin, int Cout, int dtype, void* stream) {
    ConvArgs a{in, wpack, out, in_scale, in_shift, in_bias, bsum, sqpart, B, Cin, Cout, 0, relu,
               nullptr, nullptr, nullptr, nullptr, nullptr, nullptr, nullptr, nullptr, nullptr, nullptr, 0, 0, g_stamps.load()};
    KA_REQUIRE(in && wpack && out, "conv3x3: null tensor");
    KA_REQUIRE((in_scale == nullptr) == (in_shift == nullptr), "conv3x3: scale/shift must come together");
    hipStream_t st = static_cast<hipStream_t>(stream);
    if (dtype == KA_DTYPE_BF16) return conv_dispatch<bf16_t>(a, st);
    if (dtype == KA_DTYPE_F32) return conv_dispatch<float>(a, st);
    ka_set_error("conv3x3: unknown dtype %d", dtype);
    return KA_ERR_ARG;
}

extern "C" int ka_conv3x3_fwd_keep_supported(int B, int Cin, int Cout, int dtype) {
    if (dtype != KA_DTYPE_BF16 || Cin != Cout || B < 512) return 0;
    if (ka_opt(KA_OPT_CONV_P, 1) == 0 || ka_opt(KA_OPT_CONV_PC2, 3) == 0) return 0;
    return Cin == 256 && ka_opt(KA_OPT_CONV_MT, 5) != 6;
}
extern "C" int ka_conv3x3_fwd_keep(const void* in, const void* wpack, void* out, const float* in_scale, const float* in_shift,
                                   const float* in_bias, int relu, float* bsum, float* sqpart, void* x_out, int B, int Cin, int Cout,
                                   int dtype, void* stream) {
    KA_REQUIRE(in && wpack && out, "conv3x3: null tensor");
    KA_REQUIRE((in_scale == nullptr) == (in_shift == nullptr), "conv3x3: scale/shift must come together");
    KA_REQUIRE(!x_out || ((in_scale || in_bias || relu) && ka_conv3x3_fwd_keep_supported(B, Cin, Cout, dtype)),
               "conv3x3_fwd_keep: x_out needs an input transform and a shape the two-board kernel takes (B=%d Cin=%d Cout=%d)", B, Cin, Cout);
    ConvArgs a{in, wpack, out, in_scale, in_shift, in_bias, bsum, sqpart, B, Cin, Cout, 0, relu,
               nullptr, nullptr, x_out, nullptr, nullptr, nullptr, nullptr, nullptr, nullptr, nullptr, 0, 0, g_stamps.load()};
    hipStream_t st = static_cast<hipStream_t>(stream);
    if (dtype == KA_DTYPE_BF16) return conv_dispatch<bf16_t>(a, st);
    if (dtype == KA_DTYPE_F32) return conv_dispatch<float>(a, st);
    ka_set_error("conv3x3: unknown dtype %d", dtype);
    return KA_ERR_ARG;
}

extern "C" int ka_conv3x3_dgrad_fused(const void* in, const void* in2, const float* k, void* dy_out, const void* wpack,
                                      void* out, float* bsum, const void* ep_y, const float* ep_scale,
                                      const float* ep_shift, const float* ep_mean, const float* ep_invstd, float* ep_s1,
                                      float* ep_s2, int B, int Cin, int Cout, int dtype, void* stream) {
    KA_REQUIRE(in && in2 && k && wpack && out, "conv3x3_dgrad_fused: null tensor");
    KA_REQUIRE(dtype == KA_DTYPE_BF16, "conv3x3_dgrad_fused: bf16 only");
    KA_REQUIRE(!ep_y || (ep_scale && ep_shift && ep_mean && ep_invstd && ep_s1 && ep_s2), "conv3x3_dgrad_fused: epilogue tensors");
    ConvArgs a{in, wpack, out, k, k + Cin, nullptr, bsum, nullptr, B, Cin, Cout, 0, 0,
               in2, k + 2 * Cin, dy_out, ep_y, ep_scale, ep_shift, ep_mean, ep_invstd, ep_s1, ep_s2, 0, 0, g_stamps.load()};
    return conv_dispatch<bf16_t>(a, static_cast<hipStream_t>(stream));
}

extern "C" int ka_conv3x3_dgrad_gated_supported(int B, int Cin, int Cout, int dtype, int masked) {
    if (dtype != KA_DTYPE_BF16 || B < 512 || Cin != Cout || (Cin != 256 && Cin != 128)) return 0;
    const int pv = ka_opt(KA_OPT_CONV_P, 1), p2 = ka_opt(KA_OPT_CONV_PC2, 3);
    if (pv == 0 || p2 < 3 || !masked) return 0;
    if (Cin == 256 && ka_opt(KA_OPT_CONV_MT, 5) == 6) return 0;
    return 1;
}

extern "C" int ka_conv3x3_dgrad_fused_gated(const void* du, const float* gate_add, const void* in2, const float* k,
                                            void* dy_out, const void* wpack, void* out, float* bsum, const void* ep_y,
                                            const float* ep_scale, const float* ep_shift, const float* ep_mean,
                                            const float* ep_invstd, float* ep_s1, float* ep_s2, int B, int Cin, int Cout,
                                            int dtype, void* stream) {
    KA_REQUIRE(du && gate_add && in2 && k && wpack && out, "conv3x3_dgrad_fused_gated: null tensor");
    KA_REQUIRE(dtype == KA_DTYPE_BF16, "conv3x3_dgrad_fused_gated: bf16 only");
    KA_REQUIRE(!ep_y || (ep_scale && ep_shift && ep_mean && ep_invstd && ep_s1 && ep_s2), "conv3x3_dgrad_fused_gated: epilogue tensors");
    KA_REQUIRE(ka_conv3x3_dgrad_gated_supported(B, Cin, Cout, dtype, ep_y != nullptr),
               "conv3x3_dgrad_fused_gated: shape B=%d C=%d/%d %s is not taken by the two-board kernel's masked form", B, Cin, Cout,
               ep_y ? "masked" : "plain");
    ConvArgs a{du, wpack, out, k, k + Cin, gate_add, bsum, nullptr, B, Cin, Cout, 0, 0,
               in2, k + 2 * Cin, dy_out, ep_y, ep_scale, ep_shift, ep_mean, ep_invstd, ep_s1, ep_s2, 0, 0, g_stamps.load()};
    return conv_dispatch<bf16_t>(a, static_cast<hipStream_t>(stream));
}

extern "C" int ka_debug_conv_stamps(unsigned long long* stamps) { g_stamps.store(stamps); return KA_OK; }

extern "C" int ka_conv3x3_sqpart_rows(int B) { return B; }

extern "C" int ka_conv_route_counts(long long* out, int n) {
    KA_REQUIRE(out && n >= 0, "conv_route_counts: bad arguments");
    for (int i = 0; i < n && i < KA_RT_COUNT; ++i) out[i] = g_conv_routes[i].load(std::memory_order_relaxed);
    return KA_OK;
}

extern "C" int ka_pack_conv3x3(const float* w, void* dst, int Co, int Ci, int Nout, int Kin, int mode, int dtype,
                               void* stream) {
    KA_REQUIRE(w && dst && (mode == 0 || mode == 1), "pack_conv3x3: bad arguments");
    KA_REQUIRE(Nout % 16 == 0, "pack_conv3x3: Nout %% 16 != 0");
    hipStream_t st = static_cast<hipStream_t>(stream);
    const int cpk = dtype == KA_DTYPE_BF16 ? 32 : 16;
    KA_REQUIRE(Kin % cpk == 0, "pack_conv3x3: Kin %% %d != 0", cpk);
    const size_t total = (size_t)9 * (Kin / cpk) * (Nout / 16) * 64;
    const int blocks = (int)((total + 255) / 256 < 2048 ? (total + 255) / 256 : 2048);
    if (dtype == KA_DTYPE_BF16)
        hipLaunchKernelGGL(pack_conv3x3_kernel<bf16_t>, dim3(blocks), dim3(256), 0, st, w, dst, Co, Ci, Nout, Kin, mode);
    else if (dtype == KA_DTYPE_F32)
        hipLaunchKernelGGL(pack_conv3x3_kernel<float>, dim3(blocks), dim3(256), 0, st, w, dst, Co, Ci, Nout, Kin, mode);
    else { ka_set_error("pack_conv3x3: unknown dtype %d", dtype); return KA_ERR_ARG; }
    return ka_check_launch("pack_conv3x3");
}

extern "C" int ka_pack_conv3x3_multi(const long long* table, int n, long long max_pieces, int dtype, void* stream) {
    KA_REQUIRE(table && n > 0 && max_pieces > 0, "pack_conv3x3_multi: bad arguments");
    hipStream_t st = static_cast<hipStream_t>(stream);
    const int bx = (int)((max_pieces + 255) / 256 < 64 ? (max_pieces + 255) / 256 : 64);
    if (dtype == KA_DTYPE_BF16)
        hipLaunchKernelGGL(pack_conv3x3_multi_kernel<bf16_t>, dim3(bx, n), dim3(256), 0, st, table);
    else if (dtype == KA_DTYPE_F32)
        hipLaunchKernelGGL(pack_conv3x3_multi_kernel<float>, dim3(bx, n), dim3(256), 0, st, table);
    else { ka_set_error("pack_conv3x3_multi: unknown dtype %d", dtype); return KA_ERR_ARG; }
    return ka_check_launch("pack_conv3x3_multi");
}
```

### keisei_amd/csrc/gemm.hip

```cpp
#include "common.h"

namespace {

struct GemmArgs {
    const void* A; const void* B; void* C; const float* bias;
    int M, N, K, lda, ldb, ldc;
    int transA, transB;
    int a_bf16, b_bf16, c_bf16, relu, ksplit_len, accumulate;
    int a_vec, b_vec;
};

#define KA_GLOBAL __attribute__((address_space(1)))
__device__ __forceinline__ float ldx(const void* p, size_t i, int bf16) {
    return bf16 ? bf2f(((const KA_GLOBAL uint16_t*)p)[i]) : ((const KA_GLOBAL float*)p)[i];
}

__device__ __forceinline__ f32x4 ld4(const void* base, size_t i, int bf16, int vec, int valid) {
    f32x4 v = {0.f, 0.f, 0.f, 0.f};
    if (valid <= 0) return v;
    if (vec && valid >= 4) {
        if (bf16) {
            const uint32_t ux = ((const KA_GLOBAL uint32_t*)((const KA_GLOBAL uint16_t*)base + i))[0];
            const uint32_t uy = ((const KA_GLOBAL uint32_t*)((const KA_GLOBAL uint16_t*)base + i))[1];
            const uint2 u = {ux, uy};
            v[0] = __uint_as_float(u.x << 16); v[1] = __uint_as_float(u.x & 0xffff0000u);
            v[2] = __uint_as_float(u.y << 16); v[3] = __uint_as_float(u.y & 0xffff0000u);
        } else {
            v = *(const KA_GLOBAL f32x4*)((const KA_GLOBAL float*)base + i);
        }
    } else {
#pragma unroll
        for (int e = 0; e < 4; ++e)
            if (e < valid) v[e] = ldx(base, i + e, bf16);
    }
    return v;
}

template <bool TA, bool TB, int NW, bool ONES>
__device__ __forceinline__ void gemm_tile(const GemmArgs& g, int bx, int by, int bz, float* colsum_out) {
    constexpr int BK = 32;
    __shared__ __attribute__((aligned(16))) float As[BK][64 + 16];
    __shared__ __attribute__((aligned(16))) float Bs[BK][64 + 16];
    const int tid = threadIdx.x;
    const int m0 = by * 64, n0 = bx * 64;
    const int kbeg = bz * g.ksplit_len, kend = min(g.K, kbeg + g.ksplit_len);
    const int Neff = g.N + ((ONES && colsum_out) ? 1 : 0);
    f32x4 ra[2], rb[2];
    const bool loader = NW == 4 || tid < 256;
    auto load_tile = [&](int k0) {
        if (!loader) return;
#pragma unroll
        for (int h = 0; h < 2; ++h) {
            if (!TA) {
                const int m = min(m0 + (tid >> 3) + 32 * h, g.M - 1), k = k0 + (tid & 7) * 4;
                ra[h] = ld4(g.A, (size_t)m * g.lda + k, g.a_bf16, g.a_vec, kend - k);
            } else {
                const int k = k0 + (tid >> 4) + 16 * h, m = m0 + (tid & 15) * 4;
                ra[h] = ld4(g.A, (size_t)k * g.lda + m, g.a_bf16, g.a_vec, k < kend ? g.M - m : 0);
            }
            if (TB) {
                const int n = min(n0 + (tid >> 3) + 32 * h, g.N - 1), k = k0 + (tid & 7) * 4;
                rb[h] = ld4(g.B, (size_t)n * g.ldb + k, g.b_bf16, g.b_vec, kend - k);
            } else {
                const int k = k0 + (tid >> 4) + 16 * h, n = n0 + (tid & 15) * 4;
                rb[h] = ld4(g.B, (size_t)k * g.ldb + n, g.b_bf16, g.b_vec, k < kend ? g.N - n : 0);
                if (ONES && Neff > g.N && k < kend && g.N >= n && g.N < n + 4) rb[h][g.N - n] = 1.f;
            }
        }
    };
    auto store_tile = [&]() {
        if (!loader) return;
#pragma unroll
        for (int h = 0; h < 2; ++h) {
            if (!TA) {
                const int m = (tid >> 3) + 32 * h, k = (tid & 7) * 4;
#pragma unroll
                for (int e = 0; e < 4; ++e) As[k + e][m] = ra[h][e];
            } else {
                *reinterpret_cast<f32x4*>(&As[(tid >> 4) + 16 * h][(tid & 15) * 4]) = ra[h];
            }
            if (TB) {
                const int n = (tid >> 3) + 32 * h, k = (tid & 7) * 4;
#pragma unroll
                for (int e = 0; e < 4; ++e) Bs[k + e][n] = rb[h][e];
            } else {
                *reinterpret_cast<f32x4*>(&Bs[(tid >> 4) + 16 * h][(tid & 15) * 4]) = rb[h];
            }
        }
    };
    const int lane = tid & 63, wave = tid >> 6, r = lane & 15, q = lane >> 4;
    const int wm = wave & 3, wn = wave >> 2;
    constexpr int NJ = NW == 4 ? 4 : 1;
    f32x4 acc[NJ];
#pragma unroll
    for (int j = 0; j < NJ; ++j) acc[j] = f32x4{0.f, 0.f, 0.f, 0.f};
    const bool rows_live = m0 + wm * 16 < g.M;
    load_tile(kbeg);
    for (int k0 = kbeg; k0 < kend; k0 += BK) {
        __syncthreads();
        store_tile();
        __syncthreads();
        if (k0 + BK < kend) load_tile(k0 + BK);
        if (!rows_live) continue;
#pragma unroll
        for (int j = 0; j < NJ; ++j) {
            const int nt = (NW == 4 ? j : wn) * 16;
            if (n0 + nt >= Neff) continue;
#pragma unroll
            for (int kk = 0; kk < BK; kk += 4)
                acc[j] = __builtin_amdgcn_mfma_f32_16x16x4f32(As[kk + q][wm * 16 + r], Bs[kk + q][nt + r], acc[j], 0, 0, 0);
        }
    }
    const size_t slab = (size_t)bz * g.M * g.ldc;
    KA_GLOBAL float* C = (KA_GLOBAL float*)g.C;
    if (!rows_live) return;
#pragma unroll
    for (int j = 0; j < NJ; ++j) {
        const int n = n0 + (NW == 4 ? j : wn) * 16 + r;
        if (n >= Neff) continue;
        if (ONES && n == g.N) {
#pragma unroll
            for (int i = 0; i < 4; ++i) {
                const int m = m0 + wm * 16 + 4 * q + i;
                if (m < g.M) ((KA_GLOBAL float*)colsum_out)[m] = acc[j][i];
            }
            continue;
        }
        const float bv = g.bias ? ((const KA_GLOBAL float*)g.bias)[n] : 0.f;
#pragma unroll
        for (int i = 0; i < 4; ++i) {
            const int m = m0 + wm * 16 + 4 * q + i;
            if (m >= g.M) continue;
            float v = acc[j][i] + bv;
            if (g.relu) v = fmaxf(v, 0.f);
            const size_t o = slab + (size_t)m * g.ldc + n;
            if (g.c_bf16) ((KA_GLOBAL uint16_t*)g.C)[o] = f2bf(v);
            else C[o] = g.accumulate ? C[o] + v : v;
        }
    }
}

template <bool TA, bool TB, int NW>
__global__ __launch_bounds__(64 * NW) void gemm_f32_fast_kernel(GemmArgs g) {
    gemm_tile<TA, TB, NW, false>(g, blockIdx.x, blockIdx.y, blockIdx.z, nullptr);
}

__global__ __launch_bounds__(256) void gemm_grouped_wgrad_kernel(const long long* __restrict__ table, int njobs) {
    int lo = 0, hi = njobs - 1;
    while (lo < hi) {
        const int mid = (lo + hi + 1) >> 1;
        if ((int)table[(size_t)mid * 10 + 9] <= (int)blockIdx.x) lo = mid; else hi = mid - 1;
    }
    const long long* t = table + (size_t)lo * 10;
    const int M = (int)t[4], N = (int)t[5], K = (int)t[6], ldx = (int)t[7];
    float* db = reinterpret_cast<float*>(t[3]);
    GemmArgs g{reinterpret_cast<const void*>(t[0]), reinterpret_cast<const void*>(t[1]), reinterpret_cast<void*>(t[2]), nullptr,
               N, K, M, N, ldx, K, 1, 0, 0, (int)t[8], 0, 0, (M + 31) / 32 * 32, 0, 0, 0};
    g.a_vec = (N % 4 == 0) && ((t[0] & 15) == 0);
    g.b_vec = (ldx % 4 == 0) && ((t[1] & (g.b_bf16 ? 7 : 15)) == 0);
    const int tiles_x = (K + (db ? 1 : 0) + 63) / 64;
    const int local = (int)blockIdx.x - (int)t[9];
    gemm_tile<true, false, 4, true>(g, local % tiles_x, local / tiles_x, 0, db);
}

struct ChainArgs {
    const float* x; const float* in_scale; const float* in_shift; float in_alpha;
    const float* W1; const float* b1; const float* W2; const float* b2;
    float* x_out;
    float* hidden_out;
    float* y;
    int M, K1, ldx, H, N2;
    const float* hmask;
    unsigned long long* stamps;
};

constexpr int kFcBatch = 12;
__global__ __launch_bounds__(512) void fc_chain_kernel(ChainArgs a) {
    extern __shared__ __attribute__((aligned(16))) float lds[];
    const int xs_ld = a.K1 + 4, hs_ld = a.H + 4;
    float* xs = lds;
    float* hs = xs + 16 * xs_ld;
    float* part = hs + 16 * hs_ld;
    const int tid = threadIdx.x, lane = tid & 63, wave = tid >> 6, r = lane & 15, q = lane >> 4;
    const int m0 = blockIdx.x * 16;
#ifdef KA_DIAG_FC_TL
#define KA_FTL(ph) do { if (a.stamps && blockIdx.x % 100 == 0 && blockIdx.x < 300 && lane == 0) \
        a.stamps[((blockIdx.x / 100) * 8 + wave) * 8 + (ph)] = __builtin_amdgcn_s_memtime(); } while (0)
#else
#define KA_FTL(ph) do {} while (0)
#endif
    KA_FTL(0);
    float touch = 0.f;
    {
        const size_t w2_pieces = ((size_t)a.N2 * a.H * sizeof(float) + 63) / 64;
        for (size_t i = tid; i < w2_pieces; i += 512) touch += a.W2[i * 16];
    }
    const int k4n = a.K1 >> 2;
    for (int i = tid; i < 16 * k4n; i += 512) {
        const int row = i / k4n, c4 = (i - row * k4n) * 4;
        const int m = min(m0 + row, a.M - 1);
        f32x4 v = *reinterpret_cast<const f32x4*>(a.x + (size_t)m * a.ldx + c4);
        if (a.in_scale) {
            const f32x4 sc = *reinterpret_cast<const f32x4*>(a.in_scale + c4);
            const f32x4 sh = *reinterpret_cast<const f32x4*>(a.in_shift + c4);
#pragma unroll
            for (int e = 0; e < 4; ++e) v[e] = sc[e] * (v[e] * a.in_alpha) + sh[e];
            if (a.x_out && m0 + row < a.M) *reinterpret_cast<f32x4*>(a.x_out + (size_t)m * a.K1 + c4) = v;
        }
        *reinterpret_cast<f32x4*>(xs + row * xs_ld + c4) = v;
    }
    KA_FTL(1);
    __syncthreads();
    KA_FTL(2);
    const int T1 = a.H >> 4;
    const int ksplit = T1 >= 8 ? 1 : 8 / T1;
    {
        const int klen = a.K1 / ksplit;
        for (int unit = wave; unit < T1 * ksplit; unit += 8) {
            const int tile = unit % T1, kp = unit / T1;
            const float* wrow = a.W1 + (size_t)(tile * 16 + r) * a.K1 + 4 * q;
            const float* xrow = xs + r * xs_ld + 4 * q;
            f32x4 acc = {0.f, 0.f, 0.f, 0.f};
            const int kbeg = kp * klen, kend = kbeg + klen;
            for (int k0 = kbeg; k0 < kend; k0 += 16 * kFcBatch) {
                f32x4 bv[kFcBatch];
#pragma unroll
                for (int u = 0; u < kFcBatch; ++u)
                    if (k0 + 16 * u < kend) bv[u] = *reinterpret_cast<const f32x4*>(wrow + k0 + 16 * u);
#pragma unroll
                for (int u = 0; u < kFcBatch; ++u) {
                    if (k0 + 16 * u >= kend) break;
                    const f32x4 av = *reinterpret_cast<const f32x4*>(xrow + k0 + 16 * u);
#pragma unroll
                    for (int i = 0; i < 4; ++i) acc = __builtin_amdgcn_mfma_f32_16x16x4f32(av[i], bv[u][i], acc, 0, 0, 0);
                }
            }
            if (ksplit == 1) {
                const float bias = a.b1 ? a.b1[tile * 16 + r] : 0.f;
#pragma unroll
                for (int i = 0; i < 4; ++i) {
                    float hv = fmaxf(acc[i] + bias, 0.f);
                    if (a.hmask) hv = a.hmask[(size_t)min(m0 + 4 * q + i, a.M - 1) * a.H + tile * 16 + r] > 0.f ? acc[i] : 0.f;
                    hs[(4 * q + i) * hs_ld + tile * 16 + r] = hv;
                }
            } else {
#pragma unroll
                for (int i = 0; i < 4; ++i) part[(kp * 16 + 4 * q + i) * a.H + tile * 16 + r] = acc[i];
            }
        }
    }
    KA_FTL(3);
    __syncthreads();
    KA_FTL(4);
    if (ksplit > 1) {
        for (int i = tid; i < 16 * a.H; i += 512) {
            const int row = i / a.H, n = i - row * a.H;
            float v = a.b1 ? a.b1[n] : 0.f;
            for (int kp = 0; kp < ksplit; ++kp) v += part[(kp * 16 + row) * a.H + n];
            if (a.hmask) hs[row * hs_ld + n] = a.hmask[(size_t)min(m0 + row, a.M - 1) * a.H + n] > 0.f ? v : 0.f;
            else hs[row * hs_ld + n] = fmaxf(v, 0.f);
        }
        __syncthreads();
    }
    if (a.hidden_out)
        for (int i = tid; i < 16 * a.H; i += 512) {
            const int row = i / a.H, n = i - row * a.H;
            if (m0 + row < a.M) a.hidden_out[(size_t)(m0 + row) * a.H + n] = hs[row * hs_ld + n];
        }
    KA_FTL(5);
    const int T2 = (a.N2 + 15) >> 4;
    for (int tile = wave; tile < T2; tile += 8) {
        const int n = min(tile * 16 + r, a.N2 - 1);
        const float* wrow = a.W2 + (size_t)n * a.H + 4 * q;
        const float* hrow = hs + r * hs_ld + 4 * q;
        f32x4 acc = {0.f, 0.f, 0.f, 0.f};
        for (int k0 = 0; k0 < a.H; k0 += 16 * kFcBatch) {
            f32x4 bv[kFcBatch];
#pragma unroll
            for (int u = 0; u < kFcBatch; ++u)
                if (k0 + 16 * u < a.H) bv[u] = *reinterpret_cast<const f32x4*>(wrow + k0 + 16 * u);
#pragma unroll
            for (int u = 0; u < kFcBatch; ++u) {
                if (k0 + 16 * u >= a.H) break;
                const f32x4 av = *reinterpret_cast<const f32x4*>(hrow + k0 + 16 * u);
#pragma unroll
                for (int i = 0; i < 4; ++i) acc = __builtin_amdgcn_mfma_f32_16x16x4f32(av[i], bv[u][i], acc, 0, 0, 0);
            }
        }
        if (tile * 16 + r < a.N2) {
            const float bias = a.b2 ? a.b2[n] : 0.f;
#pragma unroll
            for (int i = 0; i < 4; ++i) {
                const int m = m0 + 4 * q + i;
                if (m < a.M) a.y[(size_t)m * a.N2 + n] = acc[i] + bias;
            }
        }
    }
    KA_FTL(6);
#undef KA_FTL
    if (touch == 1.2345678e38f && a.hidden_out) a.hidden_out[0] = touch;
}

__global__ void reduce_slabs_kernel(const float* __restrict__ slab, float* __restrict__ out, int nsplit, size_t n,
                                    int accumulate) {
    for (size_t i = blockIdx.x * (size_t)blockDim.x + threadIdx.x; i < n; i += (size_t)gridDim.x * blockDim.x) {
        float s = 0.f;
        int k = 0;
        for (; k + 8 <= nsplit; k += 8) {
            float v[8];
#pragma unroll
            for (int u = 0; u < 8; ++u) v[u] = slab[(size_t)(k + u) * n + i];
#pragma unroll
            for (int u = 0; u < 8; ++u) s += v[u];
        }
        for (; k < nsplit; ++k) s += slab[(size_t)k * n + i];
        out[i] = accumulate ? out[i] + s : s;
    }
}

__global__ __launch_bounds__(256) void colsum_kernel(const float* __restrict__ A, const float* __restrict__ Bm,
                                                     float* __restrict__ part, float* __restrict__ part2, int M,
                                                     int N, int rows_per) {
    __shared__ float red[2][4][64];
    const int n = blockIdx.x * 64 + (threadIdx.x & 63), sl = threadIdx.x >> 6;
    const int mbeg = blockIdx.y * rows_per, mend = min(M, mbeg + rows_per);
    float s = 0.f, s2 = 0.f;
    if (n < N) {
        int m = mbeg + sl;
        for (; m + 28 < mend; m += 32) {
            float a[8], b[8];
#pragma unroll
            for (int u = 0; u < 8; ++u) {
                a[u] = A[(size_t)(m + 4 * u) * N + n];
                b[u] = Bm ? Bm[(size_t)(m + 4 * u) * N + n] : 0.f;
            }
#pragma unroll
            for (int u = 0; u < 8; ++u) { s += a[u]; s2 += a[u] * b[u]; }
        }
        for (; m < mend; m += 4) {
            const float a = A[(size_t)m * N + n];
            s += a;
            if (Bm) s2 += a * Bm[(size_t)m * N + n];
        }
    }
    red[0][sl][threadIdx.x & 63] = s; red[1][sl][threadIdx.x & 63] = s2;
    __syncthreads();
    if (sl == 0 && n < N) {
        const int l = threadIdx.x;
        part[(size_t)blockIdx.y * N + n] = red[0][0][l] + red[0][1][l] + red[0][2][l] + red[0][3][l];
        if (part2) part2[(size_t)blockIdx.y * N + n] = red[1][0][l] + red[1][1][l] + red[1][2][l] + red[1][3][l];
    }
}

__global__ void relu_mask_kernel(float* __restrict__ g, const float* __restrict__ h, size_t n) {
    for (size_t i = blockIdx.x * (size_t)blockDim.x + threadIdx.x; i < n; i += (size_t)gridDim.x * blockDim.x)
        if (!(h[i] > 0.f)) g[i] = 0.f;
}

__global__ void rows_affine_relu_kernel(const float* __restrict__ in, const float* __restrict__ scale,
                                        const float* __restrict__ shift, float* __restrict__ out, size_t total, int N) {
    for (size_t i = blockIdx.x * (size_t)blockDim.x + threadIdx.x; i < total; i += (size_t)gridDim.x * blockDim.x) {
        const int n = i % N;
        out[i] = fmaxf(in[i] * scale[n] + shift[n], 0.f);
    }
}
__global__ void rows_bn_bwd_kernel(float* __restrict__ dr, const float* __restrict__ in, const float* __restrict__ p0,
                                   const float* __restrict__ p1, size_t total, int N, int mode) {
    for (size_t i = blockIdx.x * (size_t)blockDim.x + threadIdx.x; i < total; i += (size_t)gridDim.x * blockDim.x) {
        const int n = i % N;
        if (mode == 0) { if (!(in[i] * p0[n] + p1[n] > 0.f)) dr[i] = 0.f; }
        else dr[i] = p0[n] * dr[i] + p0[N + n] + p0[2 * N + n] * in[i];
    }
}
__global__ __launch_bounds__(256) void rows_bn_sums_kernel(const float* __restrict__ da, const float* __restrict__ in,
                                                           const float* __restrict__ mean, const float* __restrict__ invstd,
                                                           float* __restrict__ part, float* __restrict__ part2, int M,
                                                           int N, int rows_per) {
    __shared__ float red[2][4][64];
    const int n = blockIdx.x * 64 + (threadIdx.x & 63), sl = threadIdx.x >> 6;
    const int mbeg = blockIdx.y * rows_per, mend = min(M, mbeg + rows_per);
    float s = 0.f, s2 = 0.f;
    if (n < N) {
        const float mu = mean[n], is = invstd[n];
        int m = mbeg + sl;
        for (; m + 28 < mend; m += 32) {
            float a[8], b[8];
#pragma unroll
            for (int u = 0; u < 8; ++u) { a[u] = da[(size_t)(m + 4 * u) * N + n]; b[u] = in[(size_t)(m + 4 * u) * N + n]; }
#pragma unroll
            for (int u = 0; u < 8; ++u) { s += a[u]; s2 += a[u] * ((b[u] - mu) * is); }
        }
        for (; m < mend; m += 4) {
            const float a = da[(size_t)m * N + n];
            s += a; s2 += a * ((in[(size_t)m * N + n] - mu) * is);
        }
    }
    red[0][sl][threadIdx.x & 63] = s; red[1][sl][threadIdx.x & 63] = s2;
    __syncthreads();
    if (sl == 0 && n < N) {
        const int l = threadIdx.x;
        part[(size_t)blockIdx.y * N + n] = red[0][0][l] + red[0][1][l] + red[0][2][l] + red[0][3][l];
        part2[(size_t)blockIdx.y * N + n] = red[1][0][l] + red[1][1][l] + red[1][2][l] + red[1][3][l];
    }
}
__global__ __launch_bounds__(256) void rows_sq_sums_kernel(const float* __restrict__ A, float* __restrict__ part,
                                                           float* __restrict__ part2, int M, int N, int rows_per) {
    __shared__ float red[2][4][64];
    const int n = blockIdx.x * 64 + (threadIdx.x & 63), sl = threadIdx.x >> 6;
    const int mbeg = blockIdx.y * rows_per, mend = min(M, mbeg + rows_per);
    float s = 0.f, s2 = 0.f;
    if (n < N) {
        int m = mbeg + sl;
        for (; m + 28 < mend; m += 32) {
            float a[8];
#pragma unroll
            for (int u = 0; u < 8; ++u) a[u] = A[(size_t)(m + 4 * u) * N + n];
#pragma unroll
            for (int u = 0; u < 8; ++u) { s += a[u]; s2 += a[u] * a[u]; }
        }
        for (; m < mend; m += 4) { const float a = A[(size_t)m * N + n]; s += a; s2 += a * a; }
    }
    red[0][sl][threadIdx.x & 63] = s; red[1][sl][threadIdx.x & 63] = s2;
    __syncthreads();
    if (sl == 0 && n < N) {
        const int l = threadIdx.x;
        part[(size_t)blockIdx.y * N + n] = red[0][0][l] + red[0][1][l] + red[0][2][l] + red[0][3][l];
        part2[(size_t)blockIdx.y * N + n] = red[1][0][l] + red[1][1][l] + red[1][2][l] + red[1][3][l];
    }
}

inline int grid1d(size_t n, int cap) { size_t b = (n + 255) / 256; return (int)(b < (size_t)cap ? (b ? b : 1) : cap); }

}

extern "C" int ka_gemm(const void* A, const void* B, void* C, const float* bias, int M, int N, int K, int lda, int ldb,
                       int ldc, int transA, int transB, int a_bf16, int b_bf16, int c_bf16, int relu, int accumulate,
                       int nsplit, void* stream) {
    KA_REQUIRE(A && B && C && M > 0 && N > 0 && K > 0 && nsplit >= 1, "gemm: bad arguments");
    KA_REQUIRE(nsplit == 1 || (!bias && !relu && !c_bf16 && !accumulate), "gemm: split-K output must be raw fp32 slabs");
    KA_REQUIRE(!(accumulate && c_bf16), "gemm: accumulate needs an fp32 output");
    int len = (K + nsplit - 1) / nsplit;
    len = (len + 31) / 32 * 32;
    GemmArgs g{A, B, C, bias, M, N, K, lda, ldb, ldc, transA, transB, a_bf16, b_bf16, c_bf16, relu, len, accumulate};
    dim3 grid((N + 63) / 64, (M + 63) / 64, nsplit);
    KA_REQUIRE(grid.y <= 65535, "gemm: M too large for grid.y (%d rows)", M);
    hipStream_t st = static_cast<hipStream_t>(stream);
    auto rows_aligned = [](const void* p, int ld, int bf16) {
        return ld % 4 == 0 && (reinterpret_cast<uintptr_t>(p) & (bf16 ? 7 : 15)) == 0;
    };
    g.a_vec = rows_aligned(A, lda, a_bf16);
    g.b_vec = rows_aligned(B, ldb, b_bf16);
    const bool wide = (long long)grid.x * grid.y * grid.z < 128;
#define KA_GEMM_LAUNCH(TA_, TB_) \
    do { if (wide) hipLaunchKernelGGL((gemm_f32_fast_kernel<TA_, TB_, 16>), grid, dim3(1024), 0, st, g); \
         else hipLaunchKernelGGL((gemm_f32_fast_kernel<TA_, TB_, 4>), grid, dim3(256), 0, st, g); } while (0)
    if (transA && transB) KA_GEMM_LAUNCH(true, true);
    else if (transA) KA_GEMM_LAUNCH(true, false);
    else if (transB) KA_GEMM_LAUNCH(false, true);
    else KA_GEMM_LAUNCH(false, false);
#undef KA_GEMM_LAUNCH
    return ka_check_launch("gemm");
}

extern "C" int ka_gemm_grouped_wgrad(const long long* table, int njobs, int total_wgs, void* stream) {
    KA_REQUIRE(table && njobs > 0 && total_wgs > 0, "gemm_grouped_wgrad: bad arguments");
    hipLaunchKernelGGL(gemm_grouped_wgrad_kernel, dim3(total_wgs), dim3(256), 0, static_cast<hipStream_t>(stream), table, njobs);
    return ka_check_launch("gemm_grouped_wgrad");
}

extern "C" int ka_fc_chain_supported(int K1, int ldx, int H, int N2) {
    const int T1 = H / 16;
    const int ksplit = T1 >= 8 ? 1 : (T1 > 0 ? 8 / T1 : 0);
    return K1 >= 16 && K1 % 16 == 0 && K1 <= 2048 && ldx % 4 == 0 && ldx >= K1 && H >= 16 && H % 16 == 0 && H <= 512 &&
           (T1 >= 8 || T1 == 1 || T1 == 2 || T1 == 4) && (K1 / ksplit) % 16 == 0 && N2 >= 1;
}

extern "C" int ka_fc_chain(const float* x, const float* in_scale, const float* in_shift, float in_alpha, const float* W1,
                           const float* b1, const float* W2, const float* b2, float* x_out, float* hidden_out, float* y,
                           int M, int K1, int ldx, int H, int N2, void* stream) {
    KA_REQUIRE(x && W1 && W2 && y && M > 0, "fc_chain: null tensor");
    KA_REQUIRE(ka_fc_chain_supported(K1, ldx, H, N2), "fc_chain: unsupported shape (K1=%d ldx=%d H=%d N2=%d)", K1, ldx, H, N2);
    KA_REQUIRE((in_scale == nullptr) == (in_shift == nullptr), "fc_chain: in_scale / in_shift come together");
    KA_REQUIRE(!x_out || in_scale, "fc_chain: x_out is the transformed input; without a transform pass x itself");
    KA_REQUIRE((reinterpret_cast<uintptr_t>(x) & 15) == 0 && (reinterpret_cast<uintptr_t>(W1) & 15) == 0 &&
               (reinterpret_cast<uintptr_t>(W2) & 15) == 0, "fc_chain: operands must be 16-byte aligned");
    const int T1 = H / 16, ksplit = T1 >= 8 ? 1 : 8 / T1;
    const size_t lds = (size_t)(16 * (K1 + 4) + 16 * (H + 4) + (ksplit > 1 ? ksplit * 16 * H : 0)) * sizeof(float);
    KA_REQUIRE(lds <= 160 * 1024, "fc_chain: LDS %zu B", lds);
    static std::atomic<unsigned long long> attr_done{0};
    if (int rc = ka_big_lds_once(reinterpret_cast<const void*>(&fc_chain_kernel), attr_done, "fc_chain")) return rc;
    ChainArgs a{x, in_scale, in_shift, in_alpha, W1, b1, W2, b2, x_out, hidden_out, y, M, K1, ldx, H, N2, nullptr, ka_debug_stamps().load()};
    hipLaunchKernelGGL(fc_chain_kernel, dim3((M + 15) / 16), dim3(512), lds, static_cast<hipStream_t>(stream), a);
    return ka_check_launch("fc_chain");
}

extern "C" int ka_fc_chain_bwd(const float* dy, const float* hidden, const float* W2T, const float* W1T, float* dhidden_out,
                               float* dx, int M, int N2, int H, int K1, void* stream) {
    KA_REQUIRE(dy && hidden && W2T && W1T && dhidden_out && dx && M > 0, "fc_chain_bwd: null tensor");
    KA_REQUIRE(ka_fc_chain_supported(N2, N2, H, K1), "fc_chain_bwd: unsupported shape (N2=%d H=%d K1=%d)", N2, H, K1);
    KA_REQUIRE((reinterpret_cast<uintptr_t>(dy) & 15) == 0 && (reinterpret_cast<uintptr_t>(W2T) & 15) == 0 &&
               (reinterpret_cast<uintptr_t>(W1T) & 15) == 0, "fc_chain_bwd: operands must be 16-byte aligned");
    const int T1 = H / 16, ksplit = T1 >= 8 ? 1 : 8 / T1;
    const size_t lds = (size_t)(16 * (N2 + 4) + 16 * (H + 4) + (ksplit > 1 ? ksplit * 16 * H : 0)) * sizeof(float);
    KA_REQUIRE(lds <= 160 * 1024, "fc_chain_bwd: LDS %zu B", lds);
    static std::atomic<unsigned long long> attr_done{0};
    if (int rc = ka_big_lds_once(reinterpret_cast<const void*>(&fc_chain_kernel), attr_done, "fc_chain_bwd")) return rc;
    ChainArgs a{dy, nullptr, nullptr, 1.f, W2T, nullptr, W1T, nullptr, nullptr, dhidden_out, dx, M, N2, N2, H, K1, hidden, ka_debug_stamps().load()};
    hipLaunchKernelGGL(fc_chain_kernel, dim3((M + 15) / 16), dim3(512), lds, static_cast<hipStream_t>(stream), a);
    return ka_check_launch("fc_chain_bwd");
}

namespace {
__global__ __launch_bounds__(256) void transpose_multi_kernel(const long long* __restrict__ table) {
    __shared__ float tile[32][33];
    const long long* t = table + (size_t)blockIdx.y * 4;
    const KA_GLOBAL float* src = (const KA_GLOBAL float*)t[0];
    KA_GLOBAL float* dst = (KA_GLOBAL float*)t[1];
    const int R = (int)t[2], Cc = (int)t[3];
    const int tiles_c = (Cc + 31) / 32, ntiles = ((R + 31) / 32) * tiles_c;
    const int tx = threadIdx.x & 31, ty = threadIdx.x >> 5;
    for (int tl = blockIdx.x; tl < ntiles; tl += gridDim.x) {
        const int r0 = (tl / tiles_c) * 32, c0 = (tl % tiles_c) * 32;
        __syncthreads();
#pragma unroll
        for (int k = 0; k < 32; k += 8) {
            const int rr = r0 + ty + k, cc = c0 + tx;
            tile[ty + k][tx] = (rr < R && cc < Cc) ? src[(size_t)rr * Cc + cc] : 0.f;
        }
        __syncthreads();
#pragma unroll
        for (int k = 0; k < 32; k += 8) {
            const int cc = c0 + ty + k, rr = r0 + tx;
            if (cc < Cc && rr < R) dst[(size_t)cc * R + rr] = tile[tx][ty + k];
        }
    }
}
}

extern "C" int ka_transpose_multi(const void* table, int n, int max_tiles, void* stream) {
    KA_REQUIRE(table && n > 0 && max_tiles > 0, "transpose_multi: bad arguments");
    hipLaunchKernelGGL(transpose_multi_kernel, dim3(max_tiles < 64 ? max_tiles : 64, n), dim3(256), 0, static_cast<hipStream_t>(stream),
                       static_cast<const long long*>(table));
    return ka_check_launch("transpose_multi");
}

extern "C" int ka_reduce_slabs(const float* slab, float* out, int nsplit, long long n, int accumulate, void* stream) {
    KA_REQUIRE(slab && out && nsplit >= 1 && n > 0, "reduce_slabs: bad arguments");
    hipLaunchKernelGGL(reduce_slabs_kernel, dim3(grid1d((size_t)n, 2048)), dim3(256), 0,
                       static_cast<hipStream_t>(stream), slab, out, nsplit, (size_t)n, accumulate);
    return ka_check_launch("reduce_slabs");
}

__global__ void reduce_slabs2_kernel(const float* __restrict__ sa, float* __restrict__ oa, size_t na, const float* __restrict__ sb,
                                     float* __restrict__ ob, size_t nb, int nsplit) {
    for (size_t i = blockIdx.x * (size_t)blockDim.x + threadIdx.x; i < na + nb; i += (size_t)gridDim.x * blockDim.x) {
        const bool first = i < na;
        const float* __restrict__ sl = first ? sa : sb;
        const size_t n = first ? na : nb, j = first ? i : i - na;
        float s = 0.f;
        int k = 0;
        for (; k + 8 <= nsplit; k += 8) {
            float v[8];
#pragma unroll
            for (int u = 0; u < 8; ++u) v[u] = sl[(size_t)(k + u) * n + j];
#pragma unroll
            for (int u = 0; u < 8; ++u) s += v[u];
        }
        for (; k < nsplit; ++k) s += sl[(size_t)k * n + j];
        (first ? oa : ob)[j] = s;
    }
}
extern "C" int ka_reduce_slabs2(const float* slab_a, float* out_a, long long na, const float* slab_b, float* out_b, long long nb,
                                int nsplit, void* stream) {
    KA_REQUIRE(slab_a && out_a && slab_b && out_b && nsplit >= 1 && na > 0 && nb > 0, "reduce_slabs2: bad arguments");
    hipLaunchKernelGGL(reduce_slabs2_kernel, dim3(grid1d((size_t)(na + nb), 2048)), dim3(256), 0, static_cast<hipStream_t>(stream),
                       slab_a, out_a, (size_t)na, slab_b, out_b, (size_t)nb, nsplit);
    return ka_check_launch("reduce_slabs2");
}

extern "C" int ka_colsum(const float* A, const float* Bm, float* part, float* part2, int M, int N, int nsplit,
                         void* stream) {
    KA_REQUIRE(A && part && M > 0 && N > 0 && nsplit >= 1, "colsum: bad arguments");
    const int rows_per = (M + nsplit - 1) / nsplit;
    hipLaunchKernelGGL(colsum_kernel, dim3((N + 63) / 64, nsplit), dim3(256), 0, static_cast<hipStream_t>(stream), A, Bm,
                       part, part2, M, N, rows_per);
    return ka_check_launch("colsum");
}

extern "C" int ka_relu_mask(float* g, const float* h, long long n, void* stream) {
    KA_REQUIRE(g && h && n > 0, "relu_mask: bad arguments");
    hipLaunchKernelGGL(relu_mask_kernel, dim3(grid1d((size_t)n, 2048)), dim3(256), 0, static_cast<hipStream_t>(stream),
                       g, h, (size_t)n);
    return ka_check_launch("relu_mask");
}

extern "C" int ka_rows_affine_relu(const float* in, const float* scale, const float* shift, float* out, long long M,
                                   int N, void* stream) {
    KA_REQUIRE(in && scale && shift && out, "rows_affine_relu: null tensor");
    hipLaunchKernelGGL(rows_affine_relu_kernel, dim3(grid1d((size_t)M * N, 4096)), dim3(256), 0,
                       static_cast<hipStream_t>(stream), in, scale, shift, out, (size_t)M * N, N);
    return ka_check_launch("rows_affine_relu");
}

extern "C" int ka_rows_bn_bwd(float* dr, const float* in, const float* p0, const float* p1, long long M, int N,
                              int mode, void* stream) {
    KA_REQUIRE(dr && in && p0 && (mode == 1 || p1), "rows_bn_bwd: null tensor");
    hipLaunchKernelGGL(rows_bn_bwd_kernel, dim3(grid1d((size_t)M * N, 4096)), dim3(256), 0,
                       static_cast<hipStream_t>(stream), dr, in, p0, p1, (size_t)M * N, N, mode);
    return ka_check_launch("rows_bn_bwd");
}

extern "C" int ka_rows_bn_sums(const float* da, const float* in, const float* mean, const float* invstd, float* part,
                               float* part2, int M, int N, int nsplit, void* stream) {
    KA_REQUIRE(da && in && mean && invstd && part && part2, "rows_bn_sums: null tensor");
    const int rows_per = (M + nsplit - 1) / nsplit;
    hipLaunchKernelGGL(rows_bn_sums_kernel, dim3((N + 63) / 64, nsplit), dim3(256), 0, static_cast<hipStream_t>(stream),
                       da, in, mean, invstd, part, part2, M, N, rows_per);
    return ka_check_launch("rows_bn_sums");
}

extern "C" int ka_rows_sq_sums(const float* A, float* part, float* part2, int M, int N, int nsplit, void* stream) {
    KA_REQUIRE(A && part && part2, "rows_sq_sums: null tensor");
    const int rows_per = (M + nsplit - 1) / nsplit;
    hipLaunchKernelGGL(rows_sq_sums_kernel, dim3((N + 63) / 64, nsplit), dim3(256), 0, static_cast<hipStream_t>(stream),
                       A, part, part2, M, N, rows_per);
    return ka_check_launch("rows_sq_sums");
}
```

### keisei_amd/hip/seresnet.py

```python
from __future__ import annotations

from typing import Dict, List, Optional

import os
import threading

import torch
import torch.distributed as dist
from torch import nn

from keisei_amd import _lib

_call = _lib.call


def _round_up(x: int, m: int) -> int:
    return (x + m - 1) // m * m


class _Saved:
    __slots__ = ("B", "T", "train", "xin", "stem", "blocks", "heads", "sync")


_FC_SPLITS = int(os.environ.get("KA_FC_SPLITS", "256"))


class SEResNetEngine:
    def __init__(self, model: nn.Module) -> None:
        self.model = model
        self._pack_sets: Dict[tuple, dict] = {}
        self._scratch: Optional[torch.Tensor] = None
        self._redws: Optional[torch.Tensor] = None
        self._side = None
        self._pack_tkey = None
        self._graphs = {}
        self._graph_lock = threading.Lock()
        self._wslab: Optional[torch.Tensor] = None
        self._fc_jobs = None
        self._row_ring = None
        self._evalc = None
        self._evalc_sets = {}
        self._fc_tr_sets = {}
        self._tensor_lists = None
        self._tower_tabs = {}
        self._evalc_live = None
        self.overlap_wgrad = os.environ.get("KA_WGRAD_OVERLAP", "0") != "0"
        self.fork_fc = os.environ.get("KA_FC_FORK", "1") != "0"
        self._fc_side = None
        self._gpool_done = None
        self._redcnt = None
        self.bn_one_launch = os.environ.get("KA_BN_ONE_LAUNCH", "0") == "1"
        self._in_forward = False
        self.kernel_events = None
        self.weights_epoch = 0
        self.grad_reducer = None
        self.sync_events = None

    def _timed(self, kind: str, name: str, *args) -> None:
        ev = self.kernel_events
        if ev is None:
            _call(name, *args)
            return
        stream = torch.cuda.current_stream()
        a, b = torch.cuda.Event(enable_timing=True), torch.cuda.Event(enable_timing=True)
        a.record(stream)
        _call(name, *args)
        b.record(stream)
        ev[kind].append((a, b))
        if kind == "conv3x3" and name == "ka_conv3x3_fwd" and "conv3x3_fwd" in ev and self._in_forward:
            ev["conv3x3_fwd"].append((a, b))

    def notify_weights_updated(self) -> None:
        self.weights_epoch += 1

    def _red_ws(self, C: int, device) -> torch.Tensor:
        n = _lib.query("ka_reduce_workspace_doubles", C)
        if self._redws is None or self._redws.numel() < n or self._redws.device != device:
            self._redws = torch.empty(n, dtype=torch.float64, device=device)
        return self._redws

    def _red_counters(self, device) -> torch.Tensor:
        if self._redcnt is None or self._redcnt.device != device:
            self._redcnt = torch.zeros(64, dtype=torch.int32, device=device)
        return self._redcnt

    def _wgrad_side(self, n: int, device):
        if self._side is None or self._side.device != device:
            self._side = torch.cuda.Stream(device)
        if self._wslab is None or self._wslab.numel() < n or self._wslab.device != device:
            self._wslab = torch.empty(n, dtype=torch.float32, device=device)
        return self._side, self._wslab

    def _wgrad_launch(self, side, main, inputs, *args) -> None:
        if side is None:
            self._timed("wgrad", "ka_conv3x3_wgrad", *args, _lib.stream_ptr(main.device))
            return
        ev = torch.cuda.Event()
        ev.record(main)
        with torch.cuda.stream(side):
            side.wait_event(ev)
            self._timed("wgrad", "ka_conv3x3_wgrad", *args, _lib.stream_ptr(main.device))
        for t in inputs:
            t.record_stream(side)

    def _scratch_f32(self, n: int, device) -> torch.Tensor:
        if self._scratch is None or self._scratch.numel() < n or self._scratch.device != device:
            self._scratch = torch.empty(max(n, 1 << 20), dtype=torch.float32, device=device)
        return self._scratch

    def _conv_layers(self):
        m = self.model
        yield "input_conv", m.input_conv
        for i, blk in enumerate(m.blocks):
            yield f"blocks.{i}.conv1", blk.conv1
            yield f"blocks.{i}.conv2", blk.conv2

    def _get_packs(self, T: torch.dtype, device) -> Dict[str, tuple]:
        convs = list(self._conv_layers())
        tkey = (T, str(device), tuple(c.weight.data_ptr() for _, c in convs))
        ent = self._pack_sets.get(tkey)
        if ent is None:
            if len(self._pack_sets) >= 4:
                self._pack_sets.clear()
                self._graphs.clear()
            cpk = 32 if T == torch.bfloat16 else 16
            packs, jobs, mx = {}, [], 0
            for name, conv in convs:
                w = conv.weight
                co, ci = w.shape[0], w.shape[1]
                ci_pad = _round_up(ci, 64) if name == "input_conv" else ci
                nf = 9 * (ci_pad // cpk) * (co // 16) * 64
                fwd = torch.empty(nf * 16, dtype=torch.uint8, device=device)
                jobs.append([w.data_ptr(), fwd.data_ptr(), co, ci, co, ci_pad, 0, 0]); mx = max(mx, nf)
                dg = None
                if name != "input_conv":
                    nd = 9 * (co // cpk) * (ci // 16) * 64
                    dg = torch.empty(nd * 16, dtype=torch.uint8, device=device)
                    jobs.append([w.data_ptr(), dg.data_ptr(), co, ci, ci, co, 1, 0]); mx = max(mx, nd)
                packs[name] = (fwd, dg)
            ent = {"packs": packs, "table": torch.tensor(jobs, dtype=torch.int64).to(device), "max": mx, "key": None}
            self._pack_sets[tkey] = ent
        self._pack_tkey = tkey
        key = (self.weights_epoch, sum(c.weight._version for _, c in convs))
        if key != ent["key"]:
            _call("ka_pack_conv3x3_multi", ent["table"], ent["table"].shape[0], ent["max"], _lib.dtype_code(T),
                  _lib.stream_ptr(device))
            ent["key"] = key
        return ent["packs"]

    def _tower_table(self, T, device, packs):
        m = self.model
        if os.environ.get("KA_TOWER", "1") == "0" or self._evalc_live is None or T != torch.bfloat16:
            return None
        blk0 = m.blocks[0]
        C, G, R = m.params.channels, blk0.global_fc[0].out_features, blk0.se_fc1.out_features
        if not _lib.query("ka_tower_eval_supported", C, G, R, _lib.dtype_code(T)):
            return None
        rows = []
        for i, blk in enumerate(m.blocks):
            lins = (blk.global_fc[0], blk.global_fc[2], blk.se_fc1, blk.se_fc2)
            if (id(blk.bn1) not in self._evalc_live or id(blk.bn2) not in self._evalc_live
                    or any(l.bias is None or not l.weight.is_contiguous() or l.weight.dtype != torch.float32 for l in lins)):
                return None
            sc1, sh1 = self._evalc_live[id(blk.bn1)]
            sc2, sh2 = self._evalc_live[id(blk.bn2)]
            rows.append([packs[f"blocks.{i}.conv1"][0].data_ptr(), packs[f"blocks.{i}.conv2"][0].data_ptr(),
                         sc1.data_ptr(), sh1.data_ptr(), sc2.data_ptr(), sh2.data_ptr(),
                         lins[0].weight.data_ptr(), lins[0].bias.data_ptr(), lins[1].weight.data_ptr(), lins[1].bias.data_ptr(),
                         lins[2].weight.data_ptr(), lins[2].bias.data_ptr(), lins[3].weight.data_ptr(), lins[3].bias.data_ptr()])
        key = (str(device), tuple(map(tuple, rows)))
        ent = self._tower_tabs.get(key)
        if ent is None:
            if len(self._tower_tabs) >= 4:
                self._tower_tabs.clear()
                self._graphs.clear()
            ent = torch.tensor(rows, dtype=torch.int64).to(device)
            self._tower_tabs[key] = ent
        return ent

    def _eval_coeffs_all(self, device, st):
        import struct

        bns = [b for b in self.model.modules() if isinstance(b, nn.modules.batchnorm._BatchNorm)]
        if not bns or any(b.weight is None or b.bias is None or b.running_mean is None or b.running_var is None for b in bns):
            return None
        key = (str(device), tuple((b.weight.data_ptr(), b.bias.data_ptr(), b.running_mean.data_ptr(), b.running_var.data_ptr(),
                                   float(b.eps)) for b in bns))
        ent = self._evalc_sets.get(key)
        if ent is None:
            if len(self._evalc_sets) >= 4:
                self._evalc_sets.clear()
                self._graphs.clear()
            mx = max(b.num_features for b in bns)
            out = torch.empty(len(bns), 2, mx, device=device)
            rows, views = [], {}
            for i, b in enumerate(bns):
                C = b.num_features
                sc, sh = out[i, 0, :C], out[i, 1, :C]
                eps_bits = struct.unpack("<I", struct.pack("<f", float(b.eps)))[0]
                rows.append([b.weight.data_ptr(), b.bias.data_ptr(), b.running_mean.data_ptr(), b.running_var.data_ptr(),
                             sc.data_ptr(), sh.data_ptr(), C, eps_bits])
                views[id(b)] = (sc, sh)
            ent = (key, torch.tensor(rows, dtype=torch.int64).to(device), views, mx, out)
            self._evalc_sets[key] = ent
        self._evalc = ent
        _, table, views, mx, _ = self._evalc
        _call("ka_bn_eval_coeffs_multi", table, table.shape[0], mx, st)
        return views

    @staticmethod
    def _sync_group(bn: nn.Module):
        if isinstance(bn, nn.SyncBatchNorm) and dist.is_available() and dist.is_initialized():
            return dist.get_world_size() > 1 or os.environ.get("KA_FORCE_COLLECTIVES", "0") == "1"
        return False

    def _allreduce_async(self, t):
        return dist.all_reduce(t, async_op=True)

    def _allreduce_wait(self, work) -> None:
        if work is None:
            return
        ev = self.sync_events
        if ev is None or not torch.cuda.is_available():
            work.wait()
            return
        stream = torch.cuda.current_stream()
        a, b = torch.cuda.Event(enable_timing=True), torch.cuda.Event(enable_timing=True)
        a.record(stream)
        work.wait()
        b.record(stream)
        ev.append((a, b))

    def _bn_forward_begin(self, bn, bsum, rows_b, sq, rows_s, C, count, train, device, st):
        if not train:
            return (bn, None, None, None, C, count, train, device, st)
        sync = self._sync_group(bn)
        ws = self._red_ws(C, device)
        sums = work = None
        if sync:
            sums = torch.empty(2 * C + 1, dtype=torch.float64, device=device)
            _call("ka_sync_reduce", bsum, rows_b, sq, rows_s, C, float(count), sums, None, ws, st)
            work = self._allreduce_async(sums)
        elif self.bn_one_launch and C <= 64 * 64:
            return (bn, None, None, (ws, bsum, rows_b, sq, rows_s), C, count, train, device, st)
        else:
            _call("ka_bn_reduce", bsum, rows_b, sq, rows_s, C, None, ws, st)
        return (bn, sums, work, ws, C, count, train, device, st)

    def _bn_forward_end(self, ctx):
        bn, sums, work, ws, C, count, train, device, st = ctx
        if not train and self._evalc_live is not None and id(bn) in self._evalc_live:
            scale, shift = self._evalc_live[id(bn)]
            return scale, shift, None, None
        scale = torch.empty(C, device=device); shift = torch.empty(C, device=device)
        if not train:
            _call("ka_bn_eval_coeffs", bn.weight, bn.bias, bn.running_mean, bn.running_var, float(bn.eps), scale, shift, C, st)
            return scale, shift, None, None
        mean = torch.empty(C, device=device); invstd = torch.empty(C, device=device)
        track = bn.track_running_stats and bn.running_mean is not None
        if track and bn.momentum is None:
            momentum = 1.0 / float(int(bn.num_batches_tracked) + 1)
        else:
            momentum = float(bn.momentum if bn.momentum is not None else 0.0)
        rm, rv, nbt = (bn.running_mean, bn.running_var, bn.num_batches_tracked) if track else (None, None, None)
        if sums is not None:
            self._allreduce_wait(work)
            _call("ka_bn_coeffs", sums, float(count), sums[2 * C:], bn.weight, bn.bias, rm, rv, nbt, momentum, float(bn.eps),
                  scale, shift, mean, invstd, C, st)
        elif isinstance(ws, tuple):
            ws, bsum, rows_b, sq, rows_s = ws
            _call("ka_bn_reduce_coeffs", bsum, rows_b, sq, rows_s, C, ws, self._red_counters(device), float(count), bn.weight, bn.bias,
                  rm, rv, nbt, momentum, float(bn.eps), scale, shift, mean, invstd, st)
        else:
            _call("ka_bn_coeffs_parts", ws, float(count), bn.weight, bn.bias, rm, rv, nbt, momentum, float(bn.eps),
                  scale, shift, mean, invstd, C, st)
        return scale, shift, mean, invstd

    def _bn_forward(self, bn, bsum, rows_b, sq, rows_s, C, count, train, device, st):
        return self._bn_forward_end(self._bn_forward_begin(bn, bsum, rows_b, sq, rows_s, C, count, train, device, st))

    def _gemm(self, A, Bm, C, bias, M, N, K, lda, ldb, ldc, ta, tb, st, abf=0, bbf=0, cbf=0, relu=0, acc=0, ns=1):
        _call("ka_gemm", A, Bm, C, bias, M, N, K, lda, ldb, ldc, ta, tb, abf, bbf, cbf, relu, acc, ns, st)

    def _linear(self, x, lin: nn.Linear, relu: int, st):
        M, lda = x.shape
        N, K = lin.weight.shape
        y = torch.empty(M, N, device=x.device)
        self._gemm(x, lin.weight, y, lin.bias, M, N, K, lda, K, N, 0, 1, st, relu=relu)
        return y

    def _fc_chain(self, x, lin1: nn.Linear, lin2: nn.Linear, st, keep: bool, affine=None):
        M, ldx = x.shape
        H, K1 = lin1.weight.shape
        N2 = lin2.weight.shape[0]
        dev = x.device
        fused = (os.environ.get("KA_FC_CHAIN", "1") != "0" and lin1.weight.is_contiguous() and lin2.weight.is_contiguous()
                 and _lib.query("ka_fc_chain_supported", K1, ldx, H, N2))
        if not fused:
            xp = x
            if affine is not None:
                xp = torch.empty(M, K1, device=dev)
                _call("ka_affine_rows", x, affine[0], affine[1], float(affine[2]), xp, M, K1, st)
            hidden = self._linear(xp, lin1, 1, st)
            return (xp if affine is not None else None), hidden, self._linear(hidden, lin2, 0, st)
        y = torch.empty(M, N2, device=dev)
        hidden = torch.empty(M, H, device=dev) if keep else None
        xp = torch.empty(M, K1, device=dev) if (keep and affine is not None) else None
        sc, sh, alpha = affine if affine is not None else (None, None, 1.0)
        _call("ka_fc_chain", x, sc, sh, float(alpha), lin1.weight, lin1.bias, lin2.weight, lin2.bias, xp, hidden, y,
              M, K1, ldx, H, N2, st)
        return xp, hidden, y

    def _fc_transposed(self, device, st):
        blocks = self.model.blocks
        ptrs = tuple((b.global_fc[0].weight.data_ptr(), b.global_fc[2].weight.data_ptr()) for b in blocks)
        ent = self._fc_tr_sets.get((str(device), ptrs))
        if ent is None:
            if len(self._fc_tr_sets) >= 4:
                self._fc_tr_sets.clear()
            views, rows, mt = [], [], 1
            for b in blocks:
                w1, w2 = b.global_fc[0].weight, b.global_fc[2].weight
                w2t = torch.empty(w2.shape[1], w2.shape[0], device=device); w1t = torch.empty(w1.shape[1], w1.shape[0], device=device)
                views.append((w2t, w1t))
                for src, dst in ((w2, w2t), (w1, w1t)):
                    rows.append([src.data_ptr(), dst.data_ptr(), src.shape[0], src.shape[1]])
                    mt = max(mt, ((src.shape[0] + 31) // 32) * ((src.shape[1] + 31) // 32))
            ent = {"views": views, "table": torch.tensor(rows, dtype=torch.int64).to(device), "n": len(rows), "mt": mt, "key": None}
            self._fc_tr_sets[(str(device), ptrs)] = ent
        key = (self.weights_epoch, sum(b.global_fc[0].weight._version + b.global_fc[2].weight._version for b in blocks))
        if key != ent["key"]:
            _call("ka_transpose_multi", ent["table"], ent["n"], ent["mt"], st)
            ent["key"] = key
        return ent["views"]

    def _gpool_bwd(self, i, blk, dg, g1, bpool, grads, pre, st, tr, side=None):
        lin1, lin2 = blk.global_fc[0], blk.global_fc[2]
        B = dg.shape[0]
        if tr is not None:
            w2t, w1t = tr[i]
            dg1 = torch.empty(B, lin1.out_features, device=dg.device)
            dpool_x = torch.empty(B, lin1.in_features, device=dg.device)
            if side is not None:
                sstream, ev = side
                main = torch.cuda.current_stream(dg.device)
                with torch.cuda.stream(sstream):
                    sstream.wait_event(ev)
                    _call("ka_fc_chain_bwd", dg, g1, w2t, w1t, dg1, dpool_x, B, lin2.out_features, lin1.out_features,
                          lin1.in_features, _lib.stream_ptr(dg.device))
                    done = torch.cuda.Event(); done.record(sstream)
                for t in (dg, g1, dg1, dpool_x):
                    t.record_stream(sstream)
                self._gpool_done = done
            else:
                _call("ka_fc_chain_bwd", dg, g1, w2t, w1t, dg1, dpool_x, B, lin2.out_features, lin1.out_features, lin1.in_features, st)
            self._linear_bwd(dg, g1, lin2, grads, pre + "global_fc.2.weight", pre + "global_fc.2.bias", st, need_dx=False)
            self._linear_bwd(dg1, bpool, lin1, grads, pre + "global_fc.0.weight", pre + "global_fc.0.bias", st, need_dx=False)
            return dpool_x
        dg1 = self._linear_bwd(dg, g1, lin2, grads, pre + "global_fc.2.weight", pre + "global_fc.2.bias", st)
        _call("ka_relu_mask", dg1, g1, dg1.numel(), st)
        return self._linear_bwd(dg1, bpool, lin1, grads, pre + "global_fc.0.weight", pre + "global_fc.0.bias", st)

    def _upload_rows(self, rows, device):
        flat = torch.tensor(rows, dtype=torch.int64).reshape(-1)
        ring = self._row_ring
        if ring is None or ring["host"][0].numel() < flat.numel():
            n = max(flat.numel(), 4096)
            ring = {"host": [torch.empty(n, dtype=torch.int64).pin_memory() for _ in range(2)],
                    "dev": [torch.empty(n, dtype=torch.int64, device=device) for _ in range(2)], "evt": [None, None], "flip": 0}
            self._row_ring = ring
        i = ring["flip"]
        ring["flip"] ^= 1
        if ring["evt"][i] is not None:
            ring["evt"][i].synchronize()
        ring["host"][i][:flat.numel()].copy_(flat)
        ring["dev"][i][:flat.numel()].copy_(ring["host"][i][:flat.numel()], non_blocking=True)
        ev = torch.cuda.Event()
        ev.record(torch.cuda.current_stream(device))
        ring["evt"][i] = ev
        return ring["dev"][i]

    def _flush_fc_jobs(self, grads, device, st) -> None:
        jobs, self._fc_jobs = self._fc_jobs, None
        if not jobs:
            return None
        total = sum(N * K + (N if bname is not None else 0) for (_, _, _, _, _, N, K, _, bname, _) in jobs)
        flat = torch.empty(total, device=device)
        rows, off, wg = [], 0, 0
        for dy, x, ldx, xbf, M, N, K, wname, bname, wshape in jobs:
            dW = flat[off:off + N * K]; off += N * K
            db_ptr = 0
            if bname is not None:
                db = flat[off:off + N]; off += N
                grads[bname] = db
                db_ptr = db.data_ptr()
            grads[wname] = dW.view(wshape)
            rows.append([dy.data_ptr(), x.data_ptr(), dW.data_ptr(), db_ptr, M, N, K, ldx, xbf, wg])
            wg += ((N + 63) // 64) * ((K + (1 if bname is not None else 0) + 63) // 64)
        table = self._upload_rows(rows, device)
        _call("ka_gemm_grouped_wgrad", table, len(jobs), wg, st)
        return flat

    def _linear_bwd(self, dy, x, lin: nn.Linear, grads, wname, bname, st, need_dx=True, x_bf16=0, dx_out=None, acc_dx=0,
                    defer=True):
        M, N = dy.shape
        K = lin.weight.shape[1] if lin.weight.ndim == 2 else lin.weight.shape[1]
        dev = dy.device
        ldx = x.shape[1]
        if (defer and self._fc_jobs is not None and M <= 16384 and dy.dtype == torch.float32 and dy.is_contiguous()
                and x.is_contiguous()):
            self._fc_jobs.append((dy, x, ldx, int(x_bf16), M, N, K, wname, bname, tuple(lin.weight.shape)))
            if not need_dx:
                return None
            dx = dx_out if dx_out is not None else torch.empty(M, K, device=dev)
            self._gemm(dy, lin.weight, dx, None, M, K, N, N, K, K, 0, 0, st, acc=acc_dx)
            return dx
        ns = max(1, min(_FC_SPLITS, (M + 511) // 512))
        dW = torch.empty(N, K, device=dev)
        if ns == 1:
            self._gemm(dy, x, dW, None, N, K, M, N, ldx, K, 1, 0, st, bbf=x_bf16)
        else:
            slab = self._scratch_f32(ns * N * K, dev)
            self._gemm(dy, x, slab, None, N, K, M, N, ldx, K, 1, 0, st, bbf=x_bf16, ns=ns)
            _call("ka_reduce_slabs", slab, dW, ns, N * K, 0, st)
        grads[wname] = dW.view_as(lin.weight)
        if bname is not None:
            nsb = max(1, min(_FC_SPLITS, (M + 127) // 128))
            db = torch.empty(N, device=dev)
            if nsb == 1:
                _call("ka_colsum", dy, None, db, None, M, N, 1, st)
            else:
                part = self._scratch_f32(nsb * N, dev)
                _call("ka_colsum", dy, None, part, None, M, N, nsb, st)
                _call("ka_reduce_slabs", part, db, nsb, N, 0, st)
            grads[bname] = db
        if not need_dx:
            return None
        dx = dx_out if dx_out is not None else torch.empty(M, K, device=dev)
        self._gemm(dy, lin.weight, dx, None, M, K, N, N, K, K, 0, 0, st, acc=acc_dx)
        return dx

    def forward_eval_graphed(self, obs: torch.Tensor, T: torch.dtype):
        m = self.model
        dev = obs.device
        if obs.dtype != torch.float32 or not obs.is_contiguous():
            obs = obs.float().contiguous()
        self._get_packs(T, dev)
        from keisei_amd.training._structure import structure_fingerprint, structure_version
        tl, ver = self._tensor_lists, structure_version()
        self._tl_calls = getattr(self, "_tl_calls", 0) + 1
        if tl is not None and tl[2] == ver and self._tl_calls % 64 == 0 and structure_fingerprint(m) != tl[3]:
            tl = None
        if tl is None or tl[2] != ver:
            tl = self._tensor_lists = (list(m.buffers()), list(m.parameters()), ver, structure_fingerprint(m))
        key = (tuple(obs.shape), T, str(dev), self._pack_tkey,
               tuple(b.data_ptr() for b in tl[0]), tuple(q.data_ptr() for q in tl[1]))
        with self._graph_lock:
            ent = self._graphs.get(key)
            if ent is None:
                if len(self._graphs) >= 8:
                    self._graphs.clear()
                static_in = obs.clone()
                saved_overlap = self.fork_fc
                self.fork_fc = saved_overlap and os.environ.get("KA_EVAL_GRAPH_FORK", "1") != "0"
                try:
                    self.forward(static_in, False, False, T, None)
                    torch.cuda.synchronize(dev)
                    graph = torch.cuda.CUDAGraph()
                    with torch.cuda.graph(graph):
                        out = self.forward(static_in, False, False, T, None)[:3]
                finally:
                    self.fork_fc = saved_overlap
                ent = (graph, static_in, out)
                self._graphs[key] = ent
            graph, static_in, out = ent
            static_in.copy_(obs)
            graph.replay()
            return tuple(t.clone() for t in out)

    def forward(self, obs: torch.Tensor, train: bool, keep: bool, T: torch.dtype, idx: Optional[torch.Tensor] = None):
        self._in_forward = True
        m = self.model
        p = m.params
        dev = obs.device
        st = _lib.stream_ptr(dev)
        code = _lib.dtype_code(T)
        C = p.channels
        B = obs.shape[0] if idx is None else idx.shape[0]
        if obs.dtype != torch.float32 or not obs.is_contiguous():
            obs = obs.float().contiguous()
        packs = self._get_packs(T, dev)
        self._evalc_live = self._eval_coeffs_all(dev, st) if (not train and not keep) else None
        rows = _lib.query("ka_conv3x3_sqpart_rows", B)
        count = B * 81
        sv = _Saved()
        sv.B, sv.T, sv.train = B, T, train

        def new_act(ch):
            return torch.empty(B, 81, ch, dtype=T, device=dev)

        cin_pad = _round_up(p.obs_channels, 64)
        xin = new_act(cin_pad)
        _call("ka_obs_to_nhwc", obs, idx, xin, B, p.obs_channels, cin_pad, code, st)
        y0 = new_act(C)
        bsum = torch.empty(B, C, device=dev); sq = torch.empty(rows, C, device=dev)
        _call("ka_conv3x3_fwd", xin, packs["input_conv"][0], y0, None, None, None, 0,
              bsum if train else None, sq if train else None, B, cin_pad, C, code, st)
        sc0, sh0, mu0, is0 = self._bn_forward(m.input_bn, bsum, B, sq, rows, C, count, train, dev, st)
        x = new_act(C)
        pool = torch.empty(B, 4 * C, device=dev)
        _call("ka_block_tail_fwd", y0, sc0, sh0, None, None, x, pool, B, C, code, st)
        sv.xin = xin
        sv.stem = (y0, sc0, sh0, mu0, is0)
        sv.blocks = []

        tower_tab = self._tower_table(T, dev, packs) if (not train and not keep and len(m.blocks) > 0) else None
        if tower_tab is not None:
            blk0 = m.blocks[0]
            out = new_act(C)
            pool_out = torch.empty(B, 4 * C, device=dev)
            _call("ka_tower_eval", x, pool, out, pool_out, tower_tab, len(m.blocks), B, C, blk0.global_fc[0].out_features,
                  blk0.se_fc1.out_features, code, st)
            x, pool = out, pool_out
        fc_side = os.environ.get("KA_FC_SIDE")
        fside = self._wgrad_side(1, dev)[0] if (self.fork_fc and (fc_side == "1" or (fc_side is None and B < 512))) else None
        flate = self._wgrad_side(1, dev)[0] if (fc_side == "2" and fside is None) else None
        main_f = torch.cuda.current_stream(dev)
        keep_x2 = (T == torch.bfloat16 and os.environ.get("KA_KEEP_X2", "0") == "1"
                   and bool(_lib.query("ka_conv3x3_fwd_keep_supported", B, C, C, code)))
        se_in_tail = os.environ.get("KA_SE_IN_TAIL", "0") == "1"
        for i, blk in enumerate(m.blocks if tower_tab is None else ()):
            if fside is not None:
                ev = torch.cuda.Event(); ev.record(main_f)
                with torch.cuda.stream(fside):
                    fside.wait_event(ev)
                    sts = _lib.stream_ptr(dev)
                    _, g1, g = self._fc_chain(pool, blk.global_fc[0], blk.global_fc[2], sts, keep)
                    g_ready = torch.cuda.Event(); g_ready.record(fside)
                g.record_stream(main_f)
                if g1 is not None:
                    g1.record_stream(main_f)
            y1 = new_act(C)
            bsum1 = torch.empty(B, C, device=dev); sq1 = torch.empty(rows, C, device=dev)
            self._timed("conv3x3", "ka_conv3x3_fwd", x, packs[f"blocks.{i}.conv1"][0], y1, None, None, None, 0,
                  bsum1 if train else None, sq1 if train else None, B, C, C, code, st)
            if flate is not None:
                ev = torch.cuda.Event(); ev.record(main_f)
                with torch.cuda.stream(flate):
                    flate.wait_event(ev)
                    _, g1, g = self._fc_chain(pool, blk.global_fc[0], blk.global_fc[2], _lib.stream_ptr(dev), keep)
                    g_ready = torch.cuda.Event(); g_ready.record(flate)
                pool.record_stream(flate); g.record_stream(main_f)
                if g1 is not None:
                    g1.record_stream(main_f)
            bn1_ctx = self._bn_forward_begin(blk.bn1, bsum1, B, sq1, rows, C, count, train, dev, st)
            if flate is not None:
                pass
            elif fside is None:
                _, g1, g = self._fc_chain(pool, blk.global_fc[0], blk.global_fc[2], st, keep)
            sc1, sh1, mu1, is1 = self._bn_forward_end(bn1_ctx)
            if fside is not None or flate is not None:
                main_f.wait_event(g_ready)
            y2 = new_act(C)
            bsum2 = torch.empty(B, C, device=dev); sq2 = torch.empty(rows, C, device=dev)
            x2 = new_act(C) if (keep and keep_x2) else None
            if x2 is not None:
                self._timed("conv3x3", "ka_conv3x3_fwd_keep", y1, packs[f"blocks.{i}.conv2"][0], y2, sc1, sh1, g, 1,
                            bsum2, sq2 if train else None, x2, B, C, C, code, st)
            else:
                self._timed("conv3x3", "ka_conv3x3_fwd", y1, packs[f"blocks.{i}.conv2"][0], y2, sc1, sh1, g, 1,
                            bsum2, sq2 if train else None, B, C, C, code, st)
            sc2, sh2, mu2, is2 = self._bn_forward(blk.bn2, bsum2, B, sq2, rows, C, count, train, dev, st)
            out = new_act(C)
            pool_out = torch.empty(B, 4 * C, device=dev)
            Hse = blk.se_fc1.weight.shape[0]
            if (se_in_tail and blk.se_fc1.weight.is_contiguous() and blk.se_fc2.weight.is_contiguous()
                    and blk.se_fc1.bias is not None and blk.se_fc2.bias is not None
                    and _lib.query("ka_block_tail_fwd_se_supported", C, Hse, code)):
                sqz = torch.empty(B, C, device=dev) if keep else None
                se1 = torch.empty(B, Hse, device=dev) if keep else None
                se = torch.empty(B, 2 * C, device=dev)
                _call("ka_block_tail_fwd_se", y2, sc2, sh2, bsum2, blk.se_fc1.weight, blk.se_fc1.bias, blk.se_fc2.weight,
                      blk.se_fc2.bias, x, out, pool_out, sqz, se1, se, B, C, Hse, code, st)
            else:
                sqz, se1, se = self._fc_chain(bsum2, blk.se_fc1, blk.se_fc2, st, keep, affine=(sc2, sh2, 1.0 / 81.0))
                _call("ka_block_tail_fwd", y2, sc2, sh2, se, x, out, pool_out, B, C, code, st)
            if keep:
                sv.blocks.append((x, pool, y1, sc1, sh1, mu1, is1, g1, g, y2, sc2, sh2, mu2, is2, sqz, se1, se, out, x2))
            x, pool = out, pool_out

        P = p.policy_channels
        M = B * 81
        p1 = torch.empty(M, P, device=dev)
        wp1 = m.policy_conv1.weight
        self._gemm(x, wp1, p1, None, M, P, C, C, C, P, 0, 1, st, abf=int(T == torch.bfloat16))
        nsp = max(1, min(256, (M + 2047) // 2048))
        if train:
            part = torch.empty(nsp, P, device=dev); part2 = torch.empty(nsp, P, device=dev)
            _call("ka_rows_sq_sums", p1, part, part2, M, P, nsp, st)
        else:
            part = part2 = None
        scp, shp, mup, isp = self._bn_forward(m.policy_bn1, part, nsp, part2, nsp, P, M, train, dev, st)
        p1r = torch.empty(M, P, device=dev)
        _call("ka_rows_affine_relu", p1, scp, shp, p1r, M, P, st)
        A = m.SPATIAL_MOVE_TYPES
        logits = torch.empty(B, 9, 9, A, device=dev)
        wp2 = m.policy_conv2.weight
        self._gemm(p1r, wp2, logits, m.policy_conv2.bias, M, A, P, P, P, A, 0, 1, st)
        _, v1, v = self._fc_chain(pool, m.value_fc1, m.value_fc2, st, keep)
        _, s1, s = self._fc_chain(pool, m.score_fc1, m.score_fc2, st, keep)
        if keep:
            sv.heads = (x, pool, p1, scp, shp, mup, isp, p1r, v1, s1)
        self._in_forward = False
        self._evalc_live = None
        return logits, v, s, (sv if keep else None)

    def _bn_backward_begin(self, bn, s1p, s2p, rows, C, count, train, dev, st):
        ws = self._red_ws(C, dev)
        if train and self._sync_group(bn):
            sums = torch.empty(2 * C + 1, dtype=torch.float64, device=dev)
            gsums = torch.empty(2 * C + 1, dtype=torch.float64, device=dev)
            _call("ka_sync_reduce", s1p, rows, s2p, rows, C, float(count), gsums, sums, ws, st)
            return (sums, gsums, self._allreduce_async(gsums), ws)
        if self.bn_one_launch and C <= 64 * 64:
            return (None, None, None, (ws, s1p, s2p, rows))
        _call("ka_pair_reduce", s1p, s2p, rows, C, None, ws, st)
        return (None, None, None, ws)

    def _bn_backward_end(self, ctx, bn, C, count, mu, istd, train, grads, prefix, dev, st):
        sums, gsums, work, ws = ctx
        dgam = torch.empty(C, device=dev); dbet = torch.empty(C, device=dev)
        k = torch.empty(3 * C, device=dev)
        if gsums is not None:
            self._allreduce_wait(work)
            _call("ka_bn_bwd_coeffs", sums, gsums, float(count), gsums[2 * C:], bn.weight, mu, istd, dgam, dbet, k, C,
                  1 if train else 0, st)
        elif isinstance(ws, tuple):
            ws, s1p, s2p, rows = ws
            _call("ka_pair_reduce_bwd_coeffs", s1p, s2p, rows, C, ws, self._red_counters(dev), float(count), bn.weight, mu, istd,
                  dgam, dbet, k, 1 if train else 0, st)
        else:
            _call("ka_bn_bwd_coeffs_parts", ws, float(count), bn.weight, mu, istd, dgam, dbet, k, C, 1 if train else 0, st)
        grads[prefix + ".weight"], grads[prefix + ".bias"] = dgam, dbet
        return k

    def _bn_backward(self, bn, s1p, s2p, rows, C, count, mu, istd, train, grads, prefix, dev, st):
        ctx = self._bn_backward_begin(bn, s1p, s2p, rows, C, count, train, dev, st)
        return self._bn_backward_end(ctx, bn, C, count, mu, istd, train, grads, prefix, dev, st)

    def backward(self, sv: _Saved, dlogits, dv, ds) -> Dict[str, torch.Tensor]:
        m = self.model
        p = m.params
        B, T, train = sv.B, sv.T, sv.train
        code = _lib.dtype_code(T)
        bf = int(T == torch.bfloat16)
        C, P, A = p.channels, p.policy_channels, m.SPATIAL_MOVE_TYPES
        x, pool, p1, scp, shp, mup, isp, p1r, v1, s1 = sv.heads
        dev = x.device
        st = _lib.stream_ptr(dev)
        packs = self._get_packs(T, dev)
        grads: Dict[str, torch.Tensor] = {}
        M = B * 81
        count = M
        self._fc_jobs = [] if os.environ.get("KA_FC_WGRAD_GROUPED", "1") != "0" else None
        fc_tr = None
        if len(m.blocks) > 0 and os.environ.get("KA_FC_CHAIN_BWD", "1") != "0":
            l1, l2 = m.blocks[0].global_fc[0], m.blocks[0].global_fc[2]
            if (_lib.query("ka_fc_chain_supported", l2.out_features, l2.out_features, l1.out_features, l1.in_features)
                    and all(b.global_fc[0].weight.is_contiguous() and b.global_fc[2].weight.is_contiguous() for b in m.blocks)):
                fc_tr = self._fc_transposed(dev, st)

        def new_act(ch=C):
            return torch.empty(B, 81, ch, dtype=T, device=dev)

        def eval_stats(bn):
            return bn.running_mean, torch.rsqrt(bn.running_var + bn.eps)

        dpool = torch.zeros(B, 3 * C, device=dev)
        for d_out, hid, fc1, fc2, n1, n2 in ((dv, v1, m.value_fc1, m.value_fc2, "value_fc1", "value_fc2"),
                                              (ds, s1, m.score_fc1, m.score_fc2, "score_fc1", "score_fc2")):
            if d_out is None:
                grads[n2 + ".weight"] = torch.zeros_like(fc2.weight); grads[n2 + ".bias"] = torch.zeros_like(fc2.bias)
                grads[n1 + ".weight"] = torch.zeros_like(fc1.weight); grads[n1 + ".bias"] = torch.zeros_like(fc1.bias)
                continue
            d_out = d_out.float().contiguous()
            dh = self._linear_bwd(d_out, hid, fc2, grads, n2 + ".weight", n2 + ".bias", st)
            _call("ka_relu_mask", dh, hid, dh.numel(), st)
            self._linear_bwd(dh, pool, fc1, grads, n1 + ".weight", n1 + ".bias", st, dx_out=dpool, acc_dx=1)

        dxc = None
        if dlogits is not None:
            dl = dlogits.float().contiguous().view(M, A)
            w2 = _FakeLinear(m.policy_conv2.weight.view(A, P), m.policy_conv2.bias)
            dp = self._linear_bwd(dl, p1r, w2, grads, "policy_conv2.weight", "policy_conv2.bias", st, defer=False)
            grads["policy_conv2.weight"] = grads["policy_conv2.weight"].view_as(m.policy_conv2.weight)
            _call("ka_rows_bn_bwd", dp, p1, scp, shp, M, P, 0, st)
            nsp = max(1, min(256, (M + 2047) // 2048))
            part = torch.empty(nsp, P, device=dev); part2 = torch.empty(nsp, P, device=dev)
            mu_p, is_p = (mup, isp) if train else eval_stats(m.policy_bn1)
            _call("ka_rows_bn_sums", dp, p1, mu_p, is_p, part, part2, M, P, nsp, st)
            k = self._bn_backward(m.policy_bn1, part, part2, nsp, P, M, mu_p, is_p, train, grads, "policy_bn1", dev, st)
            _call("ka_rows_bn_bwd", dp, p1, k, None, M, P, 1, st)
            w1 = _FakeLinear(m.policy_conv1.weight.view(P, C), None)
            dxc = new_act()
            self._linear_bwd_act(dp, x, w1, grads, "policy_conv1.weight", dxc, bf, st)
            grads["policy_conv1.weight"] = grads["policy_conv1.weight"].view_as(m.policy_conv1.weight)
        else:
            for n, t in (("policy_conv2.weight", m.policy_conv2.weight), ("policy_conv2.bias", m.policy_conv2.bias),
                         ("policy_bn1.weight", m.policy_bn1.weight), ("policy_bn1.bias", m.policy_bn1.bias),
                         ("policy_conv1.weight", m.policy_conv1.weight)):
                grads[n] = torch.zeros_like(t)
        Hse = m.blocks[0].se_fc1.weight.shape[0] if len(m.blocks) > 0 else 0
        fuse_dx = (len(m.blocks) > 0 and os.environ.get("KA_DX_TAIL", "1") != "0"
                   and bool(_lib.query("ka_block_dx_tail_bwd_supported", C, Hse, code)))
        gate_dz = (fuse_dx and T == torch.bfloat16 and os.environ.get("KA_TAIL_GATE", "1") != "0"
                   and bool(_lib.query("ka_conv3x3_dgrad_gated_supported", B, C, C, code, 1)))
        pend = (dxc, None, None, x, pool, dpool, new_act())
        dout = pend[6]
        if not fuse_dx:
            _call("ka_block_dx", *pend, B, C, code, st)
            pend = None

        s1p = torch.empty(B, C, device=dev); s2p = torch.empty(B, C, device=dev)
        twg = 192 if self.overlap_wgrad else 0
        nsplit = _lib.query("ka_wgrad_splits", B, C, C, twg)
        nslab = max(nsplit * 9 * C * C, _lib.query("ka_wgrad_splits", B, 64, C, 0) * 9 * C * 64)
        main = torch.cuda.current_stream(dev)
        side, slab = self._wgrad_side(nslab, dev)
        if not self.overlap_wgrad:
            side = None

        red = self.grad_reducer
        per_block = 2 * 9 * C * C
        blocks_per_bucket = max(1, red.bucket_bytes // (4 * per_block)) if red is not None else 0
        bucket, bucket_off, bucket_left = None, 0, 0

        def conv_grad(like, i, last):
            nonlocal bucket, bucket_off, bucket_left
            if red is None:
                return torch.empty_like(like)
            if bucket is None:
                bucket_left = min(blocks_per_bucket, i + 1)
                bucket = torch.empty(bucket_left * per_block, device=dev)
                bucket_off = 0
            n = like.numel()
            view = bucket[bucket_off:bucket_off + n].view_as(like)
            bucket_off += n
            return view

        def conv_grads_done(i):
            nonlocal bucket, bucket_left
            if red is None:
                return
            bucket_left -= 1
            if bucket_left == 0:
                ev = torch.cuda.Event()
                ev.record(side if side is not None else main)
                red.launch(bucket, f"conv[{i}:{i + bucket.numel() // per_block}]", ev)
                bucket = None

        fc_bwd_side = None
        if os.environ.get("KA_FC_BWD_SIDE", "0") == "1" and fc_tr is not None and not self.overlap_wgrad:
            if self._fc_side is None or self._fc_side.device != dev:
                self._fc_side = torch.cuda.Stream(dev)
            fc_bwd_side = self._fc_side
        self._gpool_done = None

        def gpool_join():
            if self._gpool_done is not None:
                main.wait_event(self._gpool_done)
                self._gpool_done = None

        for i in range(len(sv.blocks) - 1, -1, -1):
            blk = m.blocks[i]
            (bx, bpool, y1, sc1, sh1, mu1, is1, g1, g, y2, sc2, sh2, mu2, is2, sqz, se1, se, out, x2) = sv.blocks[i]
            pre = f"blocks.{i}."
            if not train:
                mu1, is1 = eval_stats(blk.bn1); mu2, is2 = eval_stats(blk.bn2)
            dse = torch.empty(B, 2 * C, device=dev)
            H = blk.se_fc1.weight.shape[0]
            gpool_join()
            gate_add = None
            if pend is not None and gate_dz:
                dse1 = torch.empty(B, H, device=dev)
                gate_add = torch.empty(2, B, C, device=dev)
                dz = pend[6]
                _call("ka_block_dx_tail_bwd_du_gate", pend[0], pend[1], *pend[3:], y2, sc2, sh2, se, se1, blk.se_fc2.weight,
                      blk.se_fc1.weight, mu2, is2, gate_add[0], gate_add[1], dse, dse1, s1p, s2p, B, C, H, code, st)
                self._linear_bwd(dse, se1, blk.se_fc2, grads, pre + "se_fc2.weight", pre + "se_fc2.bias", st, need_dx=False)
                self._linear_bwd(dse1, sqz, blk.se_fc1, grads, pre + "se_fc1.weight", pre + "se_fc1.bias", st, need_dx=False)
            elif pend is not None:
                dse1 = torch.empty(B, H, device=dev)
                dz = new_act()
                _call("ka_block_dx_tail_bwd_du", pend[0], pend[1], *pend[3:], y2, sc2, sh2, se, se1, blk.se_fc2.weight,
                      blk.se_fc1.weight, mu2, is2, dz, dse, dse1, s1p, s2p, B, C, H, code, st)
                self._linear_bwd(dse, se1, blk.se_fc2, grads, pre + "se_fc2.weight", pre + "se_fc2.bias", st, need_dx=False)
                self._linear_bwd(dse1, sqz, blk.se_fc1, grads, pre + "se_fc1.weight", pre + "se_fc1.bias", st, need_dx=False)
            elif _lib.query("ka_tail_bwd_fused_supported", C, H, code):
                dse1 = torch.empty(B, H, device=dev)
                dz = new_act()
                _call("ka_tail_bwd_fused", dout, out, y2, sc2, sh2, se, se1, blk.se_fc2.weight, blk.se_fc1.weight, mu2, is2,
                      dz, dse, dse1, s1p, s2p, B, C, H, code, st)
                self._linear_bwd(dse, se1, blk.se_fc2, grads, pre + "se_fc2.weight", pre + "se_fc2.bias", st, need_dx=False)
                self._linear_bwd(dse1, sqz, blk.se_fc1, grads, pre + "se_fc1.weight", pre + "se_fc1.bias", st, need_dx=False)
            else:
                dz = new_act()
                _call("ka_tail_bwd_reduce", dout, out, y2, sc2, sh2, se, dse, B, C, code, st)
                dse1 = self._linear_bwd(dse, se1, blk.se_fc2, grads, pre + "se_fc2.weight", pre + "se_fc2.bias", st)
                _call("ka_relu_mask", dse1, se1, dse1.numel(), st)
                dsq = self._linear_bwd(dse1, sqz, blk.se_fc1, grads, pre + "se_fc1.weight", pre + "se_fc1.bias", st)
                _call("ka_tail_bwd_dz", dout, out, y2, se, dsq, mu2, is2, dz, s1p, s2p, B, C, code, st)
            k2 = self._bn_backward(blk.bn2, s1p, s2p, B, C, count, mu2, is2, train, grads, pre + "bn2", dev, st)
            dg = torch.empty(B, C, device=dev)
            if T == torch.bfloat16:
                rows = _lib.query("ka_conv3x3_sqpart_rows", B)
                dy2, dh = new_act(), new_act()
                ep1 = torch.empty(rows, C, device=dev); ep2 = torch.empty(rows, C, device=dev)
                if gate_add is not None:
                    self._timed("conv3x3", "ka_conv3x3_dgrad_fused_gated", dz, gate_add, y2, k2, dy2, packs[pre + "conv2"][1], dh, dg,
                                y1, sc1, sh1, mu1, is1, ep1, ep2, B, C, C, code, st)
                else:
                    self._timed("conv3x3", "ka_conv3x3_dgrad_fused", dz, y2, k2, dy2, packs[pre + "conv2"][1], dh, dg,
                                y1, sc1, sh1, mu1, is1, ep1, ep2, B, C, C, code, st)
                dW2 = conv_grad(blk.conv2.weight, i, False)
                if x2 is not None:
                    self._wgrad_launch(side, main, (dy2, dW2), dy2, x2, None, None, None, 0, slab, dW2, B, C, C, C, 0, twg, code)
                else:
                    self._wgrad_launch(side, main, (dy2, dW2), dy2, y1, sc1, sh1, g, 1, slab, dW2, B, C, C, C, 0, twg, code)
                grads[pre + "conv2.weight"] = dW2
                gside = None
                if fc_bwd_side is not None:
                    gev = torch.cuda.Event(); gev.record(main)
                    gside = (fc_bwd_side, gev)
                bn1_ctx = self._bn_backward_begin(blk.bn1, ep1, ep2, rows, C, count, train, dev, st)
                dpool_x = self._gpool_bwd(i, blk, dg, g1, bpool, grads, pre, st, fc_tr, gside)
                k1 = self._bn_backward_end(bn1_ctx, blk.bn1, C, count, mu1, is1, train, grads, pre + "bn1", dev, st)
                dy1, dxc = new_act(), new_act()
                self._timed("conv3x3", "ka_conv3x3_dgrad_fused", dh, y1, k1, dy1, packs[pre + "conv1"][1], dxc, None,
                            None, None, None, None, None, None, None, B, C, C, code, st)
                dW1 = conv_grad(blk.conv1.weight, i, True)
                self._wgrad_launch(side, main, (dy1, dW1), dy1, bx, None, None, None, 0, slab, dW1, B, C, C, C, 0, twg, code)
                grads[pre + "conv1.weight"] = dW1
                conv_grads_done(i)
                dx = new_act()
            else:
                _call("ka_bn_bwd_apply", dz, y2, k2, dz, B, C, code, st)
                dh = new_act()
                self._timed("conv3x3", "ka_conv3x3_fwd", dz, packs[pre + "conv2"][1], dh, None, None, None, 0, dg, None, B, C, C, code, st)
                dW2 = conv_grad(blk.conv2.weight, i, False)
                self._wgrad_launch(side, main, (dz, dW2), dz, y1, sc1, sh1, g, 1, slab, dW2, B, C, C, C, 0, twg, code)
                grads[pre + "conv2.weight"] = dW2
                dpool_x = self._gpool_bwd(i, blk, dg, g1, bpool, grads, pre, st, fc_tr)
                _call("ka_relu_bn_bwd_reduce", dh, y1, sc1, sh1, mu1, is1, dh, s1p, s2p, B, C, code, st)
                k1 = self._bn_backward(blk.bn1, s1p, s2p, B, C, count, mu1, is1, train, grads, pre + "bn1", dev, st)
                _call("ka_bn_bwd_apply", dh, y1, k1, dh, B, C, code, st)
                dxc = new_act() if side is not None else dz
                self._timed("conv3x3", "ka_conv3x3_fwd", dh, packs[pre + "conv1"][1], dxc, None, None, None, 0, None, None, B, C, C, code, st)
                dW1 = conv_grad(blk.conv1.weight, i, True)
                self._wgrad_launch(side, main, (dh, dW1), dh, bx, None, None, None, 0, slab, dW1, B, C, C, C, 0, twg, code)
                grads[pre + "conv1.weight"] = dW1
                conv_grads_done(i)
                dx = new_act() if side is not None else dh
            if fuse_dx and i > 0:
                pend = (dxc, dout, out, bx, bpool, dpool_x, dx)
            else:
                gpool_join()
                _call("ka_block_dx", dxc, dout, out, bx, bpool, dpool_x, dx, B, C, code, st)
                pend = None
            dout = dx

        y0, sc0, sh0, mu0, is0 = sv.stem
        if not train:
            mu0, is0 = eval_stats(m.input_bn)
        _call("ka_relu_bn_bwd_reduce", dout, y0, sc0, sh0, mu0, is0, dout, s1p, s2p, B, C, code, st)
        k0 = self._bn_backward(m.input_bn, s1p, s2p, B, C, count, mu0, is0, train, grads, "input_bn", dev, st)
        _call("ka_bn_bwd_apply", dout, y0, k0, dout, B, C, code, st)
        dW0 = torch.empty_like(m.input_conv.weight)
        cin_pad = sv.xin.shape[2]
        self._wgrad_launch(side, main, (dout, dW0), dout, sv.xin, None, None, None, 0, slab, dW0, B, cin_pad,
                           p.obs_channels, C, 0, 0, code)
        grads["input_conv.weight"] = dW0
        fc_flat = self._flush_fc_jobs(grads, dev, st)
        if side is not None:
            main.wait_stream(side)
        if red is not None:
            in_flat = set()
            if fc_flat is not None:
                lo, hi = fc_flat.data_ptr(), fc_flat.data_ptr() + 4 * fc_flat.numel()
                in_flat = {n for n, t in grads.items() if lo <= t.data_ptr() < hi}
# ... 72 lines not shown
```

Baseline: 42690 samples/s.

## Fuse SE block-output tail into next block's conv1 input staging

```diff
diff --git a/include/keisei_amd.h b/include/keisei_amd.h
--- a/include/keisei_amd.h
+++ b/include/keisei_amd.h
@@ -24,6 +24,9 @@
 int ka_conv3x3_fwd_keep(const void* in, const void* wpack, void* out, const float* in_scale, const float* in_shift,
                         const float* in_bias, int relu, float* bsum, float* sqpart, void* x_out, int B, int Cin, int Cout, int dtype,
                         void* stream);
+int ka_conv3x3_fwd_tail_supported(int B, int Cin, int Cout, int dtype);
+int ka_conv3x3_fwd_tail(const void* y2, const void* x, const float* ca_cb, void* out, const void* wpack, void* y, float* bsum,
+                        float* sqpart, int B, int Cin, int Cout, int dtype, void* stream);
 int ka_conv3x3_sqpart_rows(int B);
 int ka_conv_route_counts(long long* out, int n);
 int ka_conv3x3_dgrad_fused(const void* in, const void* in2, const float* k, void* dy_out, const void* wpack, void* out,
@@ -117,6 +120,9 @@
 int ka_fc_chain(const float* x, const float* in_scale, const float* in_shift, float in_alpha, const float* W1,
                 const float* b1, const float* W2, const float* b2, float* x_out, float* hidden_out, float* y, int M, int K1,
                 int ldx, int H, int N2, void* stream);
+int ka_fc_chain_coef(const float* x, const float* in_scale, const float* in_shift, float in_alpha, const float* W1,
+                     const float* b1, const float* W2, const float* b2, float* x_out, float* hidden_out, float* y, float* coef,
+                     int M, int K1, int ldx, int H, int N2, void* stream);
 int ka_fc_chain_bwd(const float* dy, const float* hidden, const float* W2T, const float* W1T, float* dhidden_out, float* dx,
                     int M, int N2, int H, int K1, void* stream);
 int ka_transpose_multi(const void* table, int n, int max_tiles, void* stream);
diff --git a/keisei_amd/_lib.py b/keisei_amd/_lib.py
--- a/keisei_amd/_lib.py
+++ b/keisei_amd/_lib.py
@@ -13,6 +13,8 @@
     "ka_conv3x3_fwd": "pppppp i pp iii i p",
     "ka_conv3x3_fwd_keep_supported": "iiii",
     "ka_conv3x3_fwd_keep": "pppppp i pp p iii i p",
+    "ka_conv3x3_fwd_tail_supported": "iiii",
+    "ka_conv3x3_fwd_tail": "pppppp pp iii i p",
     "ka_conv3x3_dgrad_fused": "ppppp pp ppppp pp iii i p",
     "ka_conv3x3_dgrad_gated_supported": "iiiii",
     "ka_conv3x3_dgrad_fused_gated": "pppppp pp ppppp pp iii i p",
@@ -76,6 +78,7 @@
     "ka_gemm_grouped_wgrad": "p ii p",
     "ka_fc_chain_supported": "iiii",
     "ka_fc_chain": "ppp f pppp ppp iiiii p",
+    "ka_fc_chain_coef": "ppp f pppp pppp iiiii p",
     "ka_fc_chain_bwd": "pppppp iiii p",
     "ka_transpose_multi": "p ii p",
     "ka_mask_words": "i",
diff --git a/keisei_amd/csrc/common.h b/keisei_amd/csrc/common.h
--- a/keisei_amd/csrc/common.h
+++ b/keisei_amd/csrc/common.h
@@ -51,7 +51,7 @@
 #define KA_OPTIONS(X)                                                                                                      \
     X(CONV_P) X(CONV_MT) X(CONV_PC2) X(CONV_PC2_SKIP) X(CONV_PC2_STAG) X(CONV_CORNER_IN) X(CONV_P_STAG) X(CONV_P_PRIO) X(CONV_P_WGS) X(CONV_P_NPW) X(CONV_WM) X(CONV_KC)       \
     X(CONV_NTW) X(CONV_STAGGER) X(CONV_PRIO) X(WGRAD_TN) X(WGRAD_WGS) X(WGRAD_STAG) X(WGRAD_LEAN) X(BOARD_PAIRS) X(TF_LDS_EPI) X(TF_K256) X(TF_BIG)    \
-    X(TF_MAP2D) X(TF_ATTN_LDS) X(TF_ATTN_ONE) X(TAIL_FWD_KB) X(TAIL_GATE_P4)
+    X(TF_MAP2D) X(TF_ATTN_LDS) X(TF_ATTN_ONE) X(TAIL_FWD_KB) X(TAIL_GATE_P4) X(FWD_TAIL_IN_CONV)
 enum KaOpt {
 #define KA_OPT_ENUM(n) KA_OPT_##n,
     KA_OPTIONS(KA_OPT_ENUM)
@@ -74,6 +74,7 @@
     KA_RT_CORNER,
     KA_RT_WGRAD_LEAN,
     KA_RT_WGRAD_TILED,
+    KA_RT_PC2_TAIL,
     KA_RT_COUNT
 };
 void ka_conv_route(int r);
diff --git a/keisei_amd/csrc/conv3x3.hip b/keisei_amd/csrc/conv3x3.hip
--- a/keisei_amd/csrc/conv3x3.hip
+++ b/keisei_amd/csrc/conv3x3.hip
@@ -1074,9 +1074,10 @@
     }
 }
 
-template <int C, int MT, bool TWO, bool MASKED, int NPW, bool SKIP = false, bool STAG = false, bool GATED = false>
+template <int C, int MT, bool TWO, bool MASKED, int NPW, bool SKIP = false, bool STAG = false, bool GATED = false, bool TAIL = false>
 __global__ __launch_bounds__((C / 32 + NPW) * 64) void conv3x3_pc2_kernel(ConvArgs a) {
     static_assert(!GATED || (TWO && MASKED && !SKIP && !STAG), "the gated input is conv2's data gradient: two-tensor, masked");
+    static_assert(!TAIL || (C == 256 && TWO && !MASKED && !SKIP && !STAG && !GATED), "the block-output input is a forward form: two-tensor, plain epilogue");
     static_assert(!(SKIP && MASKED), "the border-tile layout is built for the register-only epilogue");
     static_assert((C == 256 && MT == 5) || (C == 128 && MT == 6 && !SKIP), "shapes this kernel is built for");
     constexpr int NMW = C / 32, NCH = C / 64, NTILE = C / 16, KSG = C / 32, ROWB = C * 2, NTL = 2 * MT;
@@ -1094,7 +1095,7 @@
 
     if (wave >= NMW) {
         const int pt = tid - NMW * 64, pc = pt & 7, swave = __builtin_amdgcn_readfirstlane(wave) - NMW;
-        const bool has_aff = GATED || a.in_scale != nullptr;
+        const bool has_aff = !TAIL && (GATED || a.in_scale != nullptr);
         auto pair_rsrc = [&](const void* p, int b0, bool sized) {
             const unsigned nb = sized ? (unsigned)min(2, a.B - b0) * (KA_BOARD * ROWB) : 0u;
             return __builtin_amdgcn_make_buffer_rsrc(const_cast<char*>(static_cast<const char*>(p)) + (size_t)b0 * (KA_BOARD * ROWB), 0, nb,
@@ -1144,7 +1145,7 @@
                 const float* k3p = GATED ? a.in_scale + 2 * C : a.in_k3;
                 const f32x4 s0 = has_aff ? *reinterpret_cast<const f32x4*>(a.in_scale + ch0) : o, s1 = has_aff ? *reinterpret_cast<const f32x4*>(a.in_scale + ch0 + 4) : o;
                 const f32x4 t0 = has_aff ? *reinterpret_cast<const f32x4*>(shp + ch0) : z, t1 = has_aff ? *reinterpret_cast<const f32x4*>(shp + ch0 + 4) : z;
-                const f32x4 u0 = TWO ? *reinterpret_cast<const f32x4*>(k3p + ch0) : z, u1 = TWO ? *reinterpret_cast<const f32x4*>(k3p + ch0 + 4) : z;
+                const f32x4 u0 = (TWO && !TAIL) ? *reinterpret_cast<const f32x4*>(k3p + ch0) : z, u1 = (TWO && !TAIL) ? *reinterpret_cast<const f32x4*>(k3p + ch0 + 4) : z;
                 const bool bias = !TWO && a.in_bias;
                 const f32x4 p00 = bias ? *reinterpret_cast<const f32x4*>(a.in_bias + (size_t)b0 * C + ch0) : z;
                 const f32x4 p01 = bias ? *reinterpret_cast<const f32x4*>(a.in_bias + (size_t)b0 * C + ch0 + 4) : z;
@@ -1158,7 +1159,7 @@
                 }
             }
             float gsc0[8], gsh0[8], gsc1[8], gsh1[8];
-            if constexpr (GATED) {
+            if constexpr (GATED || TAIL) {
                 const f32x4 z = {0.f, 0.f, 0.f, 0.f};
                 const float* gp = a.in_bias + (size_t)b0 * C + ch0;
                 const float* ap = gp + (size_t)a.B * C;
@@ -1169,6 +1170,11 @@
                 const f32x4 a10 = b1 ? *reinterpret_cast<const f32x4*>(ap + C) : z, a11 = b1 ? *reinterpret_cast<const f32x4*>(ap + C + 4) : z;
 #pragma unroll
                 for (int e = 0; e < 4; ++e) {
+                    if constexpr (TAIL) {
+                        gsc0[e] = g00[e]; gsc0[4 + e] = g01[e]; gsh0[e] = a00[e]; gsh0[4 + e] = a01[e];
+                        gsc1[e] = g10[e]; gsc1[4 + e] = g11[e]; gsh1[e] = a10[e]; gsh1[4 + e] = a11[e];
+                        continue;
+                    }
                     gsc0[e] = g00[e] * sc[e]; gsc0[4 + e] = g01[e] * sc[4 + e];
                     gsh0[e] = fmaf(a00[e], sc[e], sh[e]); gsh0[4 + e] = fmaf(a01[e], sc[4 + e], sh[4 + e]);
                     gsc1[e] = g10[e] * sc[e]; gsc1[4 + e] = g11[e] * sc[4 + e];
@@ -1187,10 +1193,16 @@
 #pragma unroll
                     for (int e = 0; e < 8; ++e) {
                         float se_ = sc[e], he_ = sh[e];
-                        if constexpr (GATED) {
+                        if constexpr (GATED || TAIL) {
                             const float c0 = gsc0[e], c1 = gsc1[e], h0 = gsh0[e], h1 = gsh1[e];
                             se_ = jlo ? c0 : jhi ? c1 : (j ? c1 : c0);
                             he_ = jlo ? h0 : jhi ? h1 : (j ? h1 : h0);
+                        }
+                        if constexpr (TAIL) {
+                            float t = fmaf((float)v[e], se_, he_);
+                            t += (float)pw[TWO ? k : 0][e];
+                            v[e] = (__bf16)fmaxf(t, 0.f);
+                            continue;
                         }
                         v[e] = (__bf16)fmaf((float)pw[TWO ? k : 0][e], k3[e], fmaf((float)v[e], se_, he_));
                     }
@@ -1371,12 +1383,12 @@
     }
 }
 
-template <int C, int MT, bool TWO, bool MASKED, int NPW, bool SKIP = false, bool STAG = false, bool GATED = false>
+template <int C, int MT, bool TWO, bool MASKED, int NPW, bool SKIP = false, bool STAG = false, bool GATED = false, bool TAIL = false>
 static int launch_conv_pc2_form(const ConvArgs& a, hipStream_t st, const char* what) {
     static std::atomic<unsigned long long> done{0};
-    if (int rc = ka_big_lds_once(reinterpret_cast<const void*>(&conv3x3_pc2_kernel<C, MT, TWO, MASKED, NPW, SKIP, STAG, GATED>), done, what)) return rc;
+    if (int rc = ka_big_lds_once(reinterpret_cast<const void*>(&conv3x3_pc2_kernel<C, MT, TWO, MASKED, NPW, SKIP, STAG, GATED, TAIL>), done, what)) return rc;
     const int pairs = (a.B + 1) / 2, grid = pairs < 256 ? pairs : 256;
-    hipLaunchKernelGGL((conv3x3_pc2_kernel<C, MT, TWO, MASKED, NPW, SKIP, STAG, GATED>), dim3(grid), dim3((C / 32 + NPW) * 64),
+    hipLaunchKernelGGL((conv3x3_pc2_kernel<C, MT, TWO, MASKED, NPW, SKIP, STAG, GATED, TAIL>), dim3(grid), dim3((C / 32 + NPW) * 64),
                        C == 256 ? kP2LdsCorner : kP2Lds, st, a);
     return ka_check_launch(what);
 }
@@ -1659,6 +1671,31 @@
     return KA_ERR_ARG;
 }
 
+extern "C" int ka_conv3x3_fwd_tail_supported(int B, int Cin, int Cout, int dtype) {
+    if (ka_opt(KA_OPT_FWD_TAIL_IN_CONV, 1) == 0) return 0;
+    if (ka_opt(KA_OPT_CONV_PC2_SKIP, 0) != 0 || ka_opt(KA_OPT_CONV_PC2_STAG, 0) != 0) return 0;
+    return ka_conv3x3_fwd_keep_supported(B, Cin, Cout, dtype);
+}
+extern "C" int ka_conv3x3_fwd_tail(const void* y2, const void* x, const float* ca_cb, void* out, const void* wpack, void* y,
+                                   float* bsum, float* sqpart, int B, int Cin, int Cout, int dtype, void* stream) {
+    KA_REQUIRE(y2 && x && ca_cb && out && wpack && y, "conv3x3_fwd_tail: null tensor");
+    KA_REQUIRE(B > 0 && ka_conv3x3_fwd_tail_supported(B, Cin, Cout, dtype),
+               "conv3x3_fwd_tail: shape B=%d C=%d/%d dtype %d is not taken by the two-board kernel (or KA_FWD_TAIL_IN_CONV=0)", B, Cin, Cout, dtype);
+    hipStream_t st = static_cast<hipStream_t>(stream);
+    ConvArgs a{y2, wpack, y, nullptr, nullptr, ca_cb, bsum, sqpart, B, Cin, Cout, 0, 0,
+               x, nullptr, out, nullptr, nullptr, nullptr, nullptr, nullptr, nullptr, nullptr, 0, 0, g_stamps.load()};
+    const bool corner_in = ka_opt(KA_OPT_CONV_CORNER_IN, 1) != 0;
+    a.mt5 = corner_in ? 2 : 1;
+    ka_conv_route(KA_RT_PC2_TAIL);
+    ka_conv_route(corner_in ? KA_RT_PC2_CORNER_IN : KA_RT_PC2_CORNER_OUT);
+    if (int rc = launch_conv_pc2_form<256, 5, true, false, 4, false, false, false, true>(a, st, "conv3x3 (two boards per unit, block output built in)")) return rc;
+    if (corner_in) return KA_OK;
+    ConvArgs c{out, wpack, y, nullptr, nullptr, nullptr, bsum, sqpart, B, Cin, Cout, 0, 0,
+               nullptr, nullptr, nullptr, nullptr, nullptr, nullptr, nullptr, nullptr, nullptr, nullptr, 0, 0, g_stamps.load()};
+    c.mt5 = 1;
+    return launch_conv_corner(c, st);
+}
+
 extern "C" int ka_conv3x3_dgrad_fused(const void* in, const void* in2, const float* k, void* dy_out, const void* wpack,
                                       void* out, float* bsum, const void* ep_y, const float* ep_scale,
                                       const float* ep_shift, const float* ep_mean, const float* ep_invstd, float* ep_s1,
diff --git a/keisei_amd/csrc/gemm.hip b/keisei_amd/csrc/gemm.hip
--- a/keisei_amd/csrc/gemm.hip
+++ b/keisei_amd/csrc/gemm.hip
@@ -172,6 +172,7 @@
     int M, K1, ldx, H, N2;
     const float* hmask;
     unsigned long long* stamps;
+    float* coef;
 };
 
 constexpr int kFcBatch = 12;
@@ -181,6 +182,7 @@
     float* xs = lds;
     float* hs = xs + 16 * xs_ld;
     float* part = hs + 16 * hs_ld;
+    float* ys = part + (a.H < 128 ? (128 / a.H) * 16 * a.H : 0);
     const int tid = threadIdx.x, lane = tid & 63, wave = tid >> 6, r = lane & 15, q = lane >> 4;
     const int m0 = blockIdx.x * 16;
 #ifdef KA_DIAG_FC_TL
@@ -293,7 +295,19 @@
             for (int i = 0; i < 4; ++i) {
                 const int m = m0 + 4 * q + i;
                 if (m < a.M) a.y[(size_t)m * a.N2 + n] = acc[i] + bias;
-            }
+                if (a.coef) ys[(4 * q + i) * a.N2 + n] = acc[i] + bias;
+            }
+        }
+    }
+    if (a.coef) {
+        __syncthreads();
+        const int Cc = a.K1;
+        for (int i = tid; i < 16 * Cc; i += 512) {
+            const int row = i / Cc, c = i - row * Cc, m = m0 + row;
+            if (m >= a.M) continue;
+            const float gt = sigmoidf_(ys[row * a.N2 + c]);
+            a.coef[(size_t)m * Cc + c] = a.in_scale[c] * gt;
+            a.coef[((size_t)a.M + m) * Cc + c] = a.in_shift[c] * gt + ys[row * a.N2 + Cc + c];
         }
     }
     KA_FTL(6);
@@ -475,8 +489,8 @@
            (T1 >= 8 || T1 == 1 || T1 == 2 || T1 == 4) && (K1 / ksplit) % 16 == 0 && N2 >= 1;
 }
 
-extern "C" int ka_fc_chain(const float* x, const float* in_scale, const float* in_shift, float in_alpha, const float* W1,
-                           const float* b1, const float* W2, const float* b2, float* x_out, float* hidden_out, float* y,
+static int fc_chain_launch(const float* x, const float* in_scale, const float* in_shift, float in_alpha, const float* W1,
+                           const float* b1, const float* W2, const float* b2, float* x_out, float* hidden_out, float* y, float* coef,
                            int M, int K1, int ldx, int H, int N2, void* stream) {
     KA_REQUIRE(x && W1 && W2 && y && M > 0, "fc_chain: null tensor");
     KA_REQUIRE(ka_fc_chain_supported(K1, ldx, H, N2), "fc_chain: unsupported shape (K1=%d ldx=%d H=%d N2=%d)", K1, ldx, H, N2);
@@ -485,13 +499,24 @@
     KA_REQUIRE((reinterpret_cast<uintptr_t>(x) & 15) == 0 && (reinterpret_cast<uintptr_t>(W1) & 15) == 0 &&
                (reinterpret_cast<uintptr_t>(W2) & 15) == 0, "fc_chain: operands must be 16-byte aligned");
     const int T1 = H / 16, ksplit = T1 >= 8 ? 1 : 8 / T1;
-    const size_t lds = (size_t)(16 * (K1 + 4) + 16 * (H + 4) + (ksplit > 1 ? ksplit * 16 * H : 0)) * sizeof(float);
+    const size_t lds = (size_t)(16 * (K1 + 4) + 16 * (H + 4) + (ksplit > 1 ? ksplit * 16 * H : 0) + (coef ? 16 * N2 : 0)) * sizeof(float);
     KA_REQUIRE(lds <= 160 * 1024, "fc_chain: LDS %zu B", lds);
     static std::atomic<unsigned long long> attr_done{0};
     if (int rc = ka_big_lds_once(reinterpret_cast<const void*>(&fc_chain_kernel), attr_done, "fc_chain")) return rc;
-    ChainArgs a{x, in_scale, in_shift, in_alpha, W1, b1, W2, b2, x_out, hidden_out, y, M, K1, ldx, H, N2, nullptr, ka_debug_stamps().load()};
+    ChainArgs a{x, in_scale, in_shift, in_alpha, W1, b1, W2, b2, x_out, hidden_out, y, M, K1, ldx, H, N2, nullptr, ka_debug_stamps().load(), coef};
     hipLaunchKernelGGL(fc_chain_kernel, dim3((M + 15) / 16), dim3(512), lds, static_cast<hipStream_t>(stream), a);
     return ka_check_launch("fc_chain");
+}
+extern "C" int ka_fc_chain(const float* x, const float* in_scale, const float* in_shift, float in_alpha, const float* W1,
+                           const float* b1, const float* W2, const float* b2, float* x_out, float* hidden_out, float* y,
+                           int M, int K1, int ldx, int H, int N2, void* stream) {
+    return fc_chain_launch(x, in_scale, in_shift, in_alpha, W1, b1, W2, b2, x_out, hidden_out, y, nullptr, M, K1, ldx, H, N2, stream);
+}
+extern "C" int ka_fc_chain_coef(const float* x, const float* in_scale, const float* in_shift, float in_alpha, const float* W1,
+                                const float* b1, const float* W2, const float* b2, float* x_out, float* hidden_out, float* y,
+                                float* coef, int M, int K1, int ldx, int H, int N2, void* stream) {
+    KA_REQUIRE(coef && in_scale && in_shift && N2 == 2 * K1, "fc_chain_coef: needs coef, the BatchNorm coefficients and N2 == 2 K1 (got K1=%d N2=%d)", K1, N2);
+    return fc_chain_launch(x, in_scale, in_shift, in_alpha, W1, b1, W2, b2, x_out, hidden_out, y, coef, M, K1, ldx, H, N2, stream);
 }
 
 extern "C" int ka_fc_chain_bwd(const float* dy, const float* hidden, const float* W2T, const float* W1T, float* dhidden_out,
@@ -505,7 +530,7 @@
     KA_REQUIRE(lds <= 160 * 1024, "fc_chain_bwd: LDS %zu B", lds);
     static std::atomic<unsigned long long> attr_done{0};
     if (int rc = ka_big_lds_once(reinterpret_cast<const void*>(&fc_chain_kernel), attr_done, "fc_chain_bwd")) return rc;
-    ChainArgs a{dy, nullptr, nullptr, 1.f, W2T, nullptr, W1T, nullptr, nullptr, dhidden_out, dx, M, N2, N2, H, K1, hidden, ka_debug_stamps().load()};
+    ChainArgs a{dy, nullptr, nullptr, 1.f, W2T, nullptr, W1T, nullptr, nullptr, dhidden_out, dx, M, N2, N2, H, K1, hidden, ka_debug_stamps().load(), nullptr};
     hipLaunchKernelGGL(fc_chain_kernel, dim3((M + 15) / 16), dim3(512), lds, static_cast<hipStream_t>(stream), a);
     return ka_check_launch("fc_chain_bwd");
 }
diff --git a/keisei_amd/hip/seresnet.py b/keisei_amd/hip/seresnet.py
--- a/keisei_amd/hip/seresnet.py
+++ b/keisei_amd/hip/seresnet.py
@@ -67,7 +67,8 @@
         _call(name, *args)
         b.record(stream)
         ev[kind].append((a, b))
-        if kind == "conv3x3" and name == "ka_conv3x3_fwd" and "conv3x3_fwd" in ev and self._in_forward:
+        if (kind == "conv3x3" and name in ("ka_conv3x3_fwd", "ka_conv3x3_fwd_keep", "ka_conv3x3_fwd_tail") and "conv3x3_fwd" in ev
+                and self._in_forward):
             ev["conv3x3_fwd"].append((a, b))
 
     def notify_weights_updated(self) -> None:
@@ -289,7 +290,7 @@
         self._gemm(x, lin.weight, y, lin.bias, M, N, K, lda, K, N, 0, 1, st, relu=relu)
         return y
 
-    def _fc_chain(self, x, lin1: nn.Linear, lin2: nn.Linear, st, keep: bool, affine=None):
+    def _fc_chain(self, x, lin1: nn.Linear, lin2: nn.Linear, st, keep: bool, affine=None, want_coef: bool = False):
         M, ldx = x.shape
         H, K1 = lin1.weight.shape
         N2 = lin2.weight.shape[0]
@@ -302,14 +303,20 @@
                 xp = torch.empty(M, K1, device=dev)
                 _call("ka_affine_rows", x, affine[0], affine[1], float(affine[2]), xp, M, K1, st)
             hidden = self._linear(xp, lin1, 1, st)
-            return (xp if affine is not None else None), hidden, self._linear(hidden, lin2, 0, st)
+            res = (xp if affine is not None else None), hidden, self._linear(hidden, lin2, 0, st)
+            return res + (None,) if want_coef else res
         y = torch.empty(M, N2, device=dev)
         hidden = torch.empty(M, H, device=dev) if keep else None
         xp = torch.empty(M, K1, device=dev) if (keep and affine is not None) else None
         sc, sh, alpha = affine if affine is not None else (None, None, 1.0)
+        if want_coef and affine is not None and N2 == 2 * K1:
+            coef = torch.empty(2, M, K1, device=dev)
+            _call("ka_fc_chain_coef", x, sc, sh, float(alpha), lin1.weight, lin1.bias, lin2.weight, lin2.bias, xp, hidden, y,
+                  coef, M, K1, ldx, H, N2, st)
+            return xp, hidden, y, coef
         _call("ka_fc_chain", x, sc, sh, float(alpha), lin1.weight, lin1.bias, lin2.weight, lin2.bias, xp, hidden, y,
               M, K1, ldx, H, N2, st)
-        return xp, hidden, y
+        return (xp, hidden, y, None) if want_coef else (xp, hidden, y)
 
     def _fc_transposed(self, device, st):
         blocks = self.model.blocks
@@ -509,7 +516,16 @@
         sc0, sh0, mu0, is0 = self._bn_forward(m.input_bn, bsum, B, sq, rows, C, count, train, dev, st)
         x = new_act(C)
         pool = torch.empty(B, 4 * C, device=dev)
-        _call("ka_block_tail_fwd", y0, sc0, sh0, None, None, x, pool, B, C, code, st)
+        fc_side = os.environ.get("KA_FC_SIDE")
+        tail_in = (len(m.blocks) > 0 and (train or keep) and T == torch.bfloat16
+                   and not (self.fork_fc and (fc_side == "1" or (fc_side is None and B < 512))) and fc_side != "2"
+                   and os.environ.get("KA_SE_IN_TAIL", "0") != "1"
+                   and bool(_lib.query("ka_conv3x3_fwd_tail_supported", B, C, C, code)))
+        pend = None
+        if tail_in:
+            pend = ("stem", y0, sc0, sh0)
+        else:
+            _call("ka_block_tail_fwd", y0, sc0, sh0, None, None, x, pool, B, C, code, st)
         sv.xin = xin
         sv.stem = (y0, sc0, sh0, mu0, is0)
         sv.blocks = []
@@ -522,7 +538,6 @@
             _call("ka_tower_eval", x, pool, out, pool_out, tower_tab, len(m.blocks), B, C, blk0.global_fc[0].out_features,
                   blk0.se_fc1.out_features, code, st)
             x, pool = out, pool_out
-        fc_side = os.environ.get("KA_FC_SIDE")
         fside = self._wgrad_side(1, dev)[0] if (self.fork_fc and (fc_side == "1" or (fc_side is None and B < 512))) else None
         flate = self._wgrad_side(1, dev)[0] if (fc_side == "2" and fside is None) else None
         main_f = torch.cuda.current_stream(dev)
@@ -542,8 +557,18 @@
                     g1.record_stream(main_f)
             y1 = new_act(C)
             bsum1 = torch.empty(B, C, device=dev); sq1 = torch.empty(rows, C, device=dev)
-            self._timed("conv3x3", "ka_conv3x3_fwd", x, packs[f"blocks.{i}.conv1"][0], y1, None, None, None, 0,
-                  bsum1 if train else None, sq1 if train else None, B, C, C, code, st)
+            if pend is None:
+                self._timed("conv3x3", "ka_conv3x3_fwd", x, packs[f"blocks.{i}.conv1"][0], y1, None, None, None, 0,
+                      bsum1 if train else None, sq1 if train else None, B, C, C, code, st)
+            else:
+                if pend[0] == "stem":
+                    self._timed("conv3x3", "ka_conv3x3_fwd_keep", pend[1], packs[f"blocks.{i}.conv1"][0], y1, pend[2], pend[3], None, 1,
+                                bsum1 if train else None, sq1 if train else None, x, B, C, C, code, st)
+                else:
+                    self._timed("conv3x3", "ka_conv3x3_fwd_tail", pend[1], pend[2], pend[3], x, packs[f"blocks.{i}.conv1"][0], y1,
+                                bsum1 if train else None, sq1 if train else None, B, C, C, code, st)
+                _call("ka_pool_fwd", x, pool, B, C, code, st)
+                pend = None
             if flate is not None:
                 ev = torch.cuda.Event(); ev.record(main_f)
                 with torch.cuda.stream(flate):
@@ -583,8 +608,13 @@
                 _call("ka_block_tail_fwd_se", y2, sc2, sh2, bsum2, blk.se_fc1.weight, blk.se_fc1.bias, blk.se_fc2.weight,
                       blk.se_fc2.bias, x, out, pool_out, sqz, se1, se, B, C, Hse, code, st)
             else:
-                sqz, se1, se = self._fc_chain(bsum2, blk.se_fc1, blk.se_fc2, st, keep, affine=(sc2, sh2, 1.0 / 81.0))
-                _call("ka_block_tail_fwd", y2, sc2, sh2, se, x, out, pool_out, B, C, code, st)
+                want = tail_in and i + 1 < len(m.blocks)
+                sqz, se1, se, coef = self._fc_chain(bsum2, blk.se_fc1, blk.se_fc2, st, keep, affine=(sc2, sh2, 1.0 / 81.0), want_coef=True) \
+                    if want else self._fc_chain(bsum2, blk.se_fc1, blk.se_fc2, st, keep, affine=(sc2, sh2, 1.0 / 81.0)) + (None,)
+                if coef is not None:
+                    pend = ("block", y2, x, coef)
+                else:
+                    _call("ka_block_tail_fwd", y2, sc2, sh2, se, x, out, pool_out, B, C, code, st)
             if keep:
                 sv.blocks.append((x, pool, y1, sc1, sh1, mu1, is1, g1, g, y2, sc2, sh2, mu2, is2, sqz, se1, se, out, x2))
             x, pool = out, pool_out
```

Result: no change. 42760 samples/s (median of 6 runs) (+0.2%).
